# pwrliang/RayJoin

Measured on AMD Instinct MI355X. Metric: LSI+PIP query throughput, USCounty |><| BlockGroup, higher is better.
Workload: dtype int128+f64; 1 GPU; USCounty(base, 7112768 segs) |><| BlockGroup(query, 28793160 segs, 29665680 points), -query=lsi then -query=pip, -mode=lbvh (software LBVH); kernel_schedule=k_lsi and the PIP kernels share the chip (512 + 1536 blocks), schedule_settled_before_timing=True

## Files before the change

### rayjoin_amd/csrc/rj_api.hip

```cpp
#include <hip/hip_runtime.h>
#include <rccl/rccl.h>

#include <cmath>
#include <cstdarg>
#include <cstdio>
#include <cstring>
#include <functional>
#include <new>
#include <string>
#include <thread>
#include <vector>

#include "../../include/rayjoin_amd.h"
#include "rj_crossings.h"
#include "rj_dissolve.h"
#include "rj_eliminate.h"
#include "rj_faces.h"
#include "rj_node.h"
#include "rj_kernels.h"
#include "rj_face_points.h"
#include "rj_nearest.h"
#include "rj_within.h"
#include "rj_neighbours.h"
#include "rj_overlay_dev.h"
#include "rj_overlay_ops.h"
#include "rj_pipeline.h"
#include "rj_polygons.h"
#include "rj_ringmap.h"
#include "rj_rings.h"
#include "rj_simplify.h"
#include "rj_snap.h"

using namespace rj;

namespace {

struct MapState {
  bool present = false;
  uint64_t np = 0, ne = 0, nc = 0;
  int64_t* pts = nullptr;
  Seg* seg = nullptr;
  uint32_t* edge_chain = nullptr;
  uint32_t* ccode = nullptr;
  uint32_t* left = nullptr;
  uint32_t* right = nullptr;
  uint32_t* edge_begin = nullptr;
  int4* qext = nullptr;
  int2* qpts = nullptr;
  bool runs_cut = false;
  uint32_t run_cap = 0;
  uint64_t closed_chains = 0;
  uint32_t *run_len = nullptr, *leaf_first = nullptr, *pack_tmp = nullptr;
  QBox* run_box = nullptr;
  uint64_t packed_leaves = 0;
  uint32_t packed_solo = 0;
  uint64_t nruns = 0, npieces = 0;
  uint32_t *piece_begin = nullptr, *piece_len = nullptr, *run_first = nullptr;
};

struct BvhState {
  bool built = false;
  int leaf_order = 0;
  uint64_t n0 = 0, n0p = 0;
  char* pool = nullptr;
  Seg* sseg = nullptr;
  uint32_t* seid = nullptr;
  int32_t* sface = nullptr;
  QBox* box0 = nullptr;
  int32_t* pmx1 = nullptr;
  uint2* xtab = nullptr;
  uint2* ytab2 = nullptr;
  uint32_t* occ = nullptr;
  uint32_t* sky = nullptr;
  bool use_sky = false;
  uint32_t* strip_ytab = nullptr;
  uint4* strip_info = nullptr;
  uint2* strip_tall = nullptr;
  int strip_shift = 0;
  uint32_t occ_permille = 0;
  bool ysort = false;
  const char* columns_why = "";
  int strip_tab_shift = 0;
  QBox* strip_box = nullptr;
  uint64_t strip_entries = 0, strip_cap = 0;
  bool strips_built = false;
  QBox* lvl[kMaxLevels] = {nullptr};
  uint64_t nlvl[kMaxLevels] = {0};
  uint64_t alloc[kMaxLevels] = {0};
  int top = 0;
};

struct GridState {
  bool built = false;
  int g = 0;
  double scale = 0;
  uint32_t* begin = nullptr;
  uint32_t* eids = nullptr;
  uint64_t total = 0;
};

constexpr int kNumTimers = 12;
constexpr unsigned long long kIncoherentExtent = 1ull << 28;
constexpr uint64_t kExchHead = RJ_EXCHANGE_HEAD_WORDS;
constexpr int kCoTrials = 4;

}

struct rj_handle_s {
  int device = 0;
  hipStream_t own_stream = nullptr;
  hipStream_t aux_stream = nullptr;
  int pip_concurrent = 0;
  int cus = 256;
  bool lsi_inflight = false;
  bool lsi_shared = false;
  int co_trials = 0;
  float co_best[3] = {1e30f, 1e30f, 1e30f};
  int co_choice = -1;
  int co_mode = 0;
  bool co_measure = false;
  bool co_points = false;
  uint64_t co_n = 0;
  uint64_t co_np = 0;
  uint64_t co_np_other = 0;
  float co_ratio = 0.46f;
  int co_wpc = 8;
  int lsi_share_set = 0, pip_share_set = 0;
  int co_L = 0, co_best_L = 0;
  float co_best_imb = 0;
  int lsi_share_blocks() const {
    if (lsi_share_set) return lsi_share_set;
    if (co_L) return co_L;
    const int half = cus / 2 > 0 ? cus / 2 : 1;
    const int b = ((int) ((512.0f + 128.0f * (float) (8 - co_wpc) + 200.0f * (co_ratio - 0.6f)) * (float) cus / 256.0f) + half / 2) / half * half;
    return b < cus ? cus : (b > cus * 4 ? cus * 4 : b);
  }
  int last_pip_share = 0;
  int pip_share_blocks() const { return pip_share_set ? pip_share_set : cus * 5; }
  bool aux_pending = false;
  hipEvent_t ev_order = nullptr;
  hipStream_t stream = nullptr;
  MapState map[2];
  BvhState bvh[2];
  unsigned long long* d_counter = nullptr;
  int flip_lsi = 0, flip_pip[2] = {0, 0};
  int pip_walk = 1;
  int last_walk_points = 1;
  int last_prepared = 0;
  int last_passes = 0;
  int flip_walk[2] = {0, 0};
  uint32_t* rest[3] = {nullptr, nullptr, nullptr};
  uint64_t rest_cap[3] = {0, 0, 0};
  uint32_t* todo[3] = {nullptr, nullptr, nullptr};
  unsigned long long* todo_mask[3] = {nullptr, nullptr, nullptr};
  int exact_own_stream = 0;
  hipStream_t exact_stream = nullptr;
  hipEvent_t ev_walk_done = nullptr, ev_exact_done[2] = {nullptr, nullptr};
  bool exact_recorded[2] = {false, false};
  int exact_buf = 0, exact_last = -1;
  int exact_rot = 0;
  bool exact_pending = false;
  const void *exact_out_closest = nullptr, *exact_out_face = nullptr;
  unsigned long long* h_rest = nullptr;
  unsigned long long* d_rest = nullptr;
  uint64_t walk_n[2] = {0, 0};
  size_t count_word = 0;
  uint32_t* slow_list = nullptr;
  uint64_t slow_cap = 0;
  int flip_slow = 0;
  int last_lsi_segments = 1;
  int lsi_segments = 2;
  int walk_points = 2;
  int timers = 1;
  int points_split = -1;
  int last_points_split = 0;
  unsigned long long* d_stats = nullptr;
  unsigned long long* d_occ_part = nullptr;
  unsigned long long* h_pinned = nullptr;
  uint32_t* h_fault = nullptr;
  uint32_t* d_fault = nullptr;
  int debug_stack_cap = 1 << 30;
  int debug_walk_stack = 0;
  int debug_strip_shift = 0;
  int debug_lazy_columns_min = 0;
  bool lazy_columns_ok = false;
  bool lazy_columns_want = false;
  hipEvent_t ev[kNumTimers][2];
  bool ev_valid[kNumTimers] = {false};
  int stats_on = 0;
  GridState grid[2];
  int query_order = 1;
  bool last_ordered = false;
  bool order_fresh = false;
  struct CohCache { bool valid = false; uint64_t begin = 0, n = 0; bool incoherent = false; } coh[2][2];
  struct OrdCache { uint32_t* perm = nullptr; uint64_t cap = 0, begin = 0, n = 0; bool valid = false; } ordc[2][2];
  struct CallerSet {
    const void* p = nullptr;
    uint64_t n = 0;
    bool valid = false, has_perm = false, fresh_perm = false;
    uint32_t* perm = nullptr;
    uint64_t perm_cap = 0;
    unsigned long long sorted_extent = 0;
    uint64_t queries = 0, stamp = 0;
  };
  static constexpr int kCallerSets = 4;
  CallerSet caller[kCallerSets];
  unsigned long long* h_est = nullptr;
  unsigned long long* d_est = nullptr;
  uint64_t caller_clock = 0;
  int cur_caller = -1;
  const uint32_t* cur_order = nullptr;
  uint64_t ord_cap = 0;
  MortonKey *ord_kin = nullptr, *ord_kout = nullptr;
  uint32_t *ord_vin = nullptr, *ord_vout = nullptr;
  char* ord_temp = nullptr;
  size_t ord_temp_bytes = 0;
  int leaf_order = 1;
  int debug_run_cap = 0;
  int debug_pack_solo = 0;
  int debug_pack_spread = 0;
  int debug_cross_shift = 0, debug_cross_pair_budget = 0, debug_cross_extent_factor = 0, debug_cross_reg_factor = 0;
  CrossingsReport cross_report = {};
  NodeReport node_report;
  SnapReport snap_report;
  int debug_simplify_all_points = 0;
  SimplifyReport simplify_report;
  int debug_faces_shift = 0;
  FacesReport faces_report;
  int debug_elim_point_blocks = 0;
  EliminateReport eliminate_report;
  int debug_dissolve_point_blocks = 0;
  DissolveReport dissolve_report;
  int debug_neighbours_point_blocks = 0;
  NeighboursReport neighbours_report;
  int debug_face_points_blocks = 0;
  FacePointsReport face_points_report;
  int debug_nearest_blocks = 0;
  int debug_nearest_order_nomem = 0;
  StageMs nearest_report;
  struct NearestUnordered { const void* p = nullptr; uint64_t n = 0; bool valid = false; };
  static constexpr int kNearestUnordered = 4;
  NearestUnordered nearest_unordered[kNearestUnordered];
  int nearest_unordered_next = 0;
  int debug_within_blocks = 0;
  StageMs within_report;
  uint32_t stitch_stats[4] = {0, 0, 0, 0};
  char* strip_scratch = nullptr;
  size_t strip_scratch_bytes = 0;
  int pip_columns = -1;
  int last_columns = 0;
  int leaf_ysort = 1;
  int skyline = -1;
  int max_blocks = 1 << 20;
  int chunk_groups = 0;
  int group_lanes = 0;
  uint64_t last_stats[16] = {0};
  char* arena = nullptr;
  size_t arena_bytes = 0;
  ncclComm_t comm = nullptr;
  ncclComm_t comm2 = nullptr;
  hipStream_t comm_stream = nullptr, comm_stream2 = nullptr;
  hipEvent_t ev_comm = nullptr, ev_comm2 = nullptr, ev_comm2_aux = nullptr;
  struct Exch {
    uint32_t* send = nullptr;
    uint32_t* recv = nullptr;
    uint64_t recv_words = 0, slot = 0;
    bool pending = false;
  } ex[2];
  uint64_t ex_capacity = 0, ex_slot = 0;
  int ex_last_begin = -1;
  hipEvent_t ev_count[2] = {nullptr, nullptr};
  bool count_pending[2] = {false, false};
  unsigned long long* h_heads = nullptr;
  uint32_t* ag_send = nullptr;
  uint32_t* ag_recv = nullptr;
  uint64_t ag_send_words = 0, ag_recv_words = 0;
  int nranks = 1, rank = 0;
  unsigned long long* d_counts = nullptr;
  struct PlanRec {
    uint64_t epoch = 1;
    uint64_t sched_epoch = 0;
    struct Lsi { bool ran = false; uint64_t epoch = 0, n = 0; LaunchNote k = {"", 0, 0}; int order = 0, co_mode = 0; bool paired = false, shared = false; } lsi;
    struct Rec { bool ran = false; uint64_t epoch = 0; bool two_kernels = false, count_on_device = false; uint64_t seen = ~0ull; } rec;
    struct Pip {
      bool ran = false, aux = false, caller = false, shared = false;
      uint64_t epoch = 0, n = 0, rest_hint = ~0ull;
      LaunchNote first = {"", 0, 0};
      int passes = 0, order = 0, exact_blocks = 0, locate_blocks = 0;
      int prepared = 0;
      const char* why = "";
    } pip;
  } plan;
  std::string err;
};

namespace {

int fail(rj_handle h, int code, const char* fmt, ...) {
  char buf[512];
  va_list ap;
  va_start(ap, fmt);
  vsnprintf(buf, sizeof(buf), fmt, ap);
  va_end(ap);
  if (h) h->err = buf;
  return code;
}

#define RJ_HIP(h, expr)                                                                        \
  do {                                                                                         \
    hipError_t _e = (expr);                                                                    \
    if (_e != hipSuccess)                                                                      \
      return fail(h, _e == hipErrorOutOfMemory ? RJ_E_NOMEM : RJ_E_HIP, "%s failed: %s (%s:%d)", \
                  #expr, hipGetErrorString(_e), __FILE__, __LINE__);                           \
  } while (0)

#define RJ_CHECK_H(h) \
  if (!(h)) return RJ_E_INVALID

template <typename T>
int dev_alloc(rj_handle h, T** p, uint64_t count) {
  *p = nullptr;
  RJ_HIP(h, hipMalloc((void**) p, (count ? count : 1) * sizeof(T)));
  return RJ_OK;
}

void free_map(MapState& m) {
  (void) hipFree(m.pts); (void) hipFree(m.seg); (void) hipFree(m.edge_chain); (void) hipFree(m.ccode); (void) hipFree(m.left); (void) hipFree(m.right); (void) hipFree(m.edge_begin);
  (void) hipFree(m.qext);
  (void) hipFree(m.piece_begin); (void) hipFree(m.piece_len); (void) hipFree(m.run_first);
  (void) hipFree(m.run_len); (void) hipFree(m.leaf_first); (void) hipFree(m.pack_tmp); (void) hipFree(m.run_box);
  m = MapState();
}

void free_grid(GridState& g) {
  (void) hipFree(g.begin); (void) hipFree(g.eids);
  g = GridState();
}

void free_bvh(BvhState& b) {
  if (b.pool) {
    (void) hipFree(b.pool);
  } else {
    (void) hipFree(b.sseg); (void) hipFree(b.seid); (void) hipFree(b.sface); (void) hipFree(b.box0); (void) hipFree(b.pmx1); (void) hipFree(b.xtab); (void) hipFree(b.ytab2); (void) hipFree(b.occ); (void) hipFree(b.sky);
    for (int l = 0; l < kMaxLevels; l++) (void) hipFree(b.lvl[l]);
  }
  (void) hipFree(b.strip_ytab); (void) hipFree(b.strip_info); (void) hipFree(b.strip_tall); (void) hipFree(b.strip_box);
  b = BvhState();
}

DeviceBvh bvh_view(const BvhState& b) {
  DeviceBvh d;
  d.sseg = b.sseg; d.seid = b.seid; d.sface = b.sface; d.box0 = b.box0; d.pmx1 = b.pmx1; d.xtab = b.xtab; d.ytab2 = b.ysort ? b.ytab2 : nullptr; d.occ = b.occ; d.sky = b.use_sky ? b.sky : nullptr;
  for (int l = 0; l < kMaxLevels; l++) {
    d.lvl[l] = b.lvl[l]; d.nlvl[l] = (uint32_t) b.nlvl[l];
    d.ord[l] = b.lvl[l] ? reinterpret_cast<const uint64_t*>(b.lvl[l] + b.alloc[l]) : nullptr;
  }
  d.top = b.top; d.n0 = b.n0; d.occ_permille = b.occ_permille;
  d.lsi_root = b.top >= 2 && b.nlvl[b.top] <= 4 && b.nlvl[b.top - 1] <= 128 ? b.top - 1 : b.top;
  d.strips.ytab = b.strips_built ? b.strip_ytab : nullptr;
  d.strips.ebox = b.strip_box; d.strips.einfo = b.strip_info; d.strips.tall = b.strip_tall; d.strips.shift = b.strip_shift;
  return d;
}

DeviceMap map_view(const MapState& m) {
  DeviceMap d;
  d.pts = m.pts; d.seg = m.seg; d.edge_chain = m.edge_chain; d.left = m.left; d.right = m.right;
  d.np = m.np; d.ne = m.ne; d.nc = m.nc;
  return d;
}

int set_device(rj_handle h) {
  RJ_HIP(h, hipSetDevice(h->device));
  return RJ_OK;
}

static inline bool timers_off(rj_handle h) { return !h->timers && !(h->pip_concurrent == 2 && h->co_choice < 0); }
void tic(rj_handle h, int t, hipStream_t st = nullptr) { if (timers_off(h)) return; (void) hipEventRecord(h->ev[t][0], st ? st : h->stream); }
void toc(rj_handle h, int t, hipStream_t st = nullptr) { if (timers_off(h)) return; (void) hipEventRecord(h->ev[t][1], st ? st : h->stream); h->ev_valid[t] = true; }
hipError_t join_aux(rj_handle h) {
  if (!h->aux_pending) return hipSuccess;
  h->aux_pending = false;
  hipError_t e = hipStreamSynchronize(h->aux_stream);
  if (h->exact_pending) {
    h->exact_pending = false;
    const hipError_t e2 = hipStreamSynchronize(h->exact_stream);
    if (e == hipSuccess) e = e2;
  }
  return e;
}

static void co_reset(rj_handle h) {
  h->plan.epoch++;
  h->co_trials = 0; h->co_best[0] = h->co_best[1] = h->co_best[2] = 1e30f; h->co_choice = -1; h->co_measure = false; h->co_n = 0; h->co_np = 0; h->co_np_other = 0;
  h->co_ratio = 0.46f;
  h->co_L = h->co_best_L = 0;
  h->co_best_imb = 0;
}
static void co_collect(rj_handle h) {
  if (!h->co_measure) return;
  h->co_measure = false;
  if (h->co_choice >= 0) return;
  if (hipEventQuery(h->ev[RJ_T_LSI_KERNEL][1]) != hipSuccess || hipEventQuery(h->ev[RJ_T_PIP_KERNEL][1]) != hipSuccess) return;
  float a = 0, b = 0;
  if (hipEventElapsedTime(&a, h->ev[RJ_T_LSI_KERNEL][0], h->ev[RJ_T_LSI_KERNEL][1]) != hipSuccess) return;
  if (hipEventElapsedTime(&b, h->ev[RJ_T_LSI_KERNEL][0], h->ev[RJ_T_PIP_KERNEL][1]) != hipSuccess) return;
  float span = a > b ? a : b, c = 0;
  if (h->co_points && hipEventQuery(h->ev[RJ_T_LSI_POINTS][1]) == hipSuccess &&
      hipEventElapsedTime(&c, h->ev[RJ_T_LSI_KERNEL][0], h->ev[RJ_T_LSI_POINTS][1]) == hipSuccess && c > span) span = c;
  if (h->co_mode == 0) {
    float pip = 0, pts = 0;
    if (hipEventElapsedTime(&pip, h->ev[RJ_T_PIP_KERNEL][0], h->ev[RJ_T_PIP_KERNEL][1]) == hipSuccess && pip > 0) {
      if (h->co_points && c > 0) (void) hipEventElapsedTime(&pts, h->ev[RJ_T_LSI_POINTS][0], h->ev[RJ_T_LSI_POINTS][1]);
      h->co_ratio = (a + pts) / pip;
    }
  }
  if (h->co_mode == 1 && h->co_choice < 0 && !h->lsi_share_set) {
    const int used = h->lsi_share_blocks();
    const float lsi_side = a > c ? a : c;
    const float imb = (lsi_side - b) / (span > 0 ? span : 1.0f);
    const float aimb = imb < 0 ? -imb : imb;
    if (h->co_best_L == 0 || span < h->co_best[1] * 0.97f || (span < h->co_best[1] * 0.99f && aimb < h->co_best_imb)) {
      h->co_best_L = used;
      h->co_best_imb = aimb;
    }
    int next = used + (imb > 0 ? 1 : -1) * (h->cus / 2 > 0 ? h->cus / 2 : 1);
    next = next < h->cus ? h->cus : (next > h->cus * 4 ? h->cus * 4 : next);
    h->co_L = next;
  }
  if (span < h->co_best[h->co_mode]) h->co_best[h->co_mode] = span;
  if (++h->co_trials >= kCoTrials && h->co_choice < 0) {
    h->co_choice = 0;
    for (int m = 1; m < 3; m++) if (h->co_best[m] < h->co_best[h->co_choice]) h->co_choice = m;
    if (h->co_choice != 1 && h->co_best[1] <= h->co_best[h->co_choice] * 1.03f) h->co_choice = 1;
    if (h->co_best_L) h->co_L = h->co_best_L;
    h->plan.sched_epoch = h->plan.epoch;
  }
}
static int co_pick(rj_handle h, uint64_t n) {
  co_collect(h);
  if (h->co_n && (n > h->co_n + h->co_n / 4 || n + n / 4 < h->co_n)) co_reset(h);
  h->co_n = n;
  if (h->co_choice >= 0) return h->co_choice;
// ... 10 lines not shown
constexpr size_t kSlowCountWord = 12;
constexpr size_t kRestCountWord = 8;
constexpr size_t kExactRestWord[3] = {10, 11, 14};
constexpr size_t kGridLsiCountWord = 6;

int check_fault(rj_handle h) {
  const uint32_t l = h->h_fault[0], p = h->h_fault[1];
  if (!l && !p) return RJ_OK;
  h->h_fault[0] = h->h_fault[1] = 0;
  return fail(h, RJ_E_INTERNAL, "traversal stack overflow in %s%s%s: results are incomplete", l ? "k_lsi" : "",
              l && p ? " and " : "", p ? "k_pip" : "");
}

int switch_stream(rj_handle h, hipStream_t s) {
  if (s == h->stream) return RJ_OK;
  if (int r = set_device(h)) return r;
  RJ_HIP(h, hipStreamSynchronize(h->stream));
  RJ_HIP(h, join_aux(h));
  h->lsi_shared = h->lsi_inflight = false;
  h->co_measure = false;
  h->stream = s;
  return RJ_OK;
}

int set_stats(rj_handle h, int64_t v) { h->stats_on = v != 0; return RJ_OK; }
int set_own_stream(rj_handle h, int64_t) { return switch_stream(h, h->own_stream); }
int set_pip_concurrent(rj_handle h, int64_t v) {
  if (join_aux(h) != hipSuccess) return fail(h, RJ_E_HIP, "pip_concurrent: stream sync failed");
  h->pip_concurrent = (int) v;
  co_reset(h);
  return RJ_OK;
}
int set_pip_exact_stream(rj_handle h, int64_t v) {
  if ((int) v == h->exact_own_stream) return RJ_OK;
  if (int r = set_device(h)) return r;
  RJ_HIP(h, hipStreamSynchronize(h->stream));
  h->aux_pending = true;
  RJ_HIP(h, join_aux(h));
  RJ_HIP(h, hipStreamSynchronize(h->exact_stream));
  for (size_t wd : kExactRestWord) RJ_HIP(h, hipMemsetAsync(h->d_counter + wd, 0, 8, h->stream));
  RJ_HIP(h, hipStreamSynchronize(h->stream));
  h->exact_rot = 0; h->exact_buf = 0; h->exact_last = -1; h->exact_out_closest = h->exact_out_face = nullptr;
  h->exact_recorded[0] = h->exact_recorded[1] = false;
  h->exact_own_stream = (int) v;
  return RJ_OK;
}

constexpr int64_t kAnyLo = INT64_MIN, kAnyHi = INT64_MAX;
struct Option {
  const char* name;
  bool debug;
  int rj_handle_s::*field;
  int64_t lo, hi;
  const char* hint;
  const char* env;
  int (*set)(rj_handle h, int64_t v);
  int nalso;
  int64_t also[5];
  bool accepts(int64_t v) const {
    if (v >= lo && v <= hi) return true;
    for (int i = 0; i < nalso; i++) if (v == also[i]) return true;
    return false;
  }
};
const Option kOptions[] = {
    {"leaf_order", false, &rj_handle_s::leaf_order, 0, 1, "leaf_order: 0 Hilbert neighbours, 1 chain runs", "RJ_LEAF_ORDER"},
    {"skyline", false, &rj_handle_s::skyline, -1, 1, "skyline: -1 auto (maps of isolated rings), 0 never, 1 always"},
    {"leaf_ysort", false, &rj_handle_s::leaf_ysort, 0, 1, "leaf_ysort: 1 blocks taller than wide get a second order by y (LSI), 0 x order only", "RJ_LEAF_YSORT"},
    {"pip_columns", false, &rj_handle_s::pip_columns, -1, 1, "pip_columns: -1 auto (maps of closed rings or of short chains), 0 never, 1 always",
     "RJ_PIP_COLUMNS"},
    {"lsi_segments", false, &rj_handle_s::lsi_segments, 1, 2, "lsi_segments: 1 or 2", "RJ_LSI_SEGMENTS"},
    {"pip_walk_points", false, &rj_handle_s::walk_points, 1, 2, "pip_walk_points: 1 or 2", "RJ_WALK_POINTS"},
    {"pip_walk", false, &rj_handle_s::pip_walk, 0, 2, "pip_walk: 0 k_pip alone, 1 auto, 2 always two passes"},
    {"lsi_points_split", false, &rj_handle_s::points_split, -1, 1, "lsi_points_split: -1 by the last count, 0 never, 1 always", "RJ_POINTS_SPLIT"},
    {"query_order", false, &rj_handle_s::query_order, 0, 2, "query_order: 0 never, 1 auto, 2 always"},
    {"timers", false, &rj_handle_s::timers, 0, 1, "timers: 0 or 1"},
    {"pip_concurrent", false, &rj_handle_s::pip_concurrent, 0, 2,
     "pip_concurrent: 0 never, 1 LSI and PIP queries come in pairs and share the chip, 2 the same if it measures faster", nullptr, set_pip_concurrent},
    {"pip_exact_stream", false, &rj_handle_s::exact_own_stream, 0, 1, "pip_exact_stream: 0 or 1", nullptr, set_pip_exact_stream},
    {"stats", false, &rj_handle_s::stats_on, kAnyLo, kAnyHi, nullptr, nullptr, set_stats},
    {"own_stream", false, nullptr, kAnyLo, kAnyHi, nullptr, nullptr, set_own_stream},
    {"chunk_groups", true, &rj_handle_s::chunk_groups, 0, 4096},
    {"group_lanes", true, &rj_handle_s::group_lanes, 0, 0, "group_lanes: 0 (auto), 4, 8, 16, 32 or 64", nullptr, nullptr, 5, {4, 8, 16, 32, 64}},
    {"max_blocks", true, &rj_handle_s::max_blocks, 1, 1 << 20},
    {"lsi_share_blocks", true, &rj_handle_s::lsi_share_set, 0, 1 << 20},
    {"pip_share_blocks", true, &rj_handle_s::pip_share_set, 0, 1 << 20},
    {"stack_cap", true, &rj_handle_s::debug_stack_cap, 1, 1 << 30},
    {"walk_stack", true, &rj_handle_s::debug_walk_stack, 0, 1 << 30},
    {"strip_shift", true, &rj_handle_s::debug_strip_shift, 15, 20, "strip_shift: 0 or 15..20 (the sort key holds 16 bits of strip)", nullptr, nullptr, 1, {0}},
    {"lazy_columns_min", true, &rj_handle_s::debug_lazy_columns_min, 0, 1 << 30},
    {"run_cap", true, &rj_handle_s::debug_run_cap, 2, 64, "run_cap: 0 or 2..64", nullptr, nullptr, 1, {0}},
    {"pack_solo", true, &rj_handle_s::debug_pack_solo, 0, 64},
    {"pack_spread", true, &rj_handle_s::debug_pack_spread, 0, 1000000},
    {"cross_shift", true, &rj_handle_s::debug_cross_shift, 15, 47, "cross_shift: 0 (choose) or 15..47", nullptr, nullptr, 1, {0}},
    {"cross_pair_budget", true, &rj_handle_s::debug_cross_pair_budget, 0, 1 << 30},
    {"cross_extent_factor", true, &rj_handle_s::debug_cross_extent_factor, 0, 1 << 20},
    {"cross_reg_factor", true, &rj_handle_s::debug_cross_reg_factor, 0, 1 << 20},
    {"simplify_all_points", true, &rj_handle_s::debug_simplify_all_points, 0, 1},
    {"faces_shift", true, &rj_handle_s::debug_faces_shift, 15, 47, "faces_shift: 0 (choose) or 15..47", nullptr, nullptr, 1, {0}},
    {"elim_point_blocks", true, &rj_handle_s::debug_elim_point_blocks, 0, 1 << 20},
    {"dissolve_point_blocks", true, &rj_handle_s::debug_dissolve_point_blocks, 0, 1 << 20},
    {"neighbours_point_blocks", true, &rj_handle_s::debug_neighbours_point_blocks, 0, 1 << 20},
    {"face_points_blocks", true, &rj_handle_s::debug_face_points_blocks, 0, 1 << 20},
    {"nearest_blocks", true, &rj_handle_s::debug_nearest_blocks, 0, 1 << 20},
    {"nearest_order_nomem", true, &rj_handle_s::debug_nearest_order_nomem, 0, 1},
    {"within_blocks", true, &rj_handle_s::debug_within_blocks, 0, 1 << 20},
};

const Option* find_option(const char* name, bool debug) {
  for (const Option& o : kOptions)
    if (o.debug == debug && !strcmp(name, o.name)) return &o;
  return nullptr;
}

int set_option(rj_handle h, const char* name, int64_t value, bool debug) {
  RJ_CHECK_H(h);
  if (!name) return fail(h, RJ_E_INVALID, "null option name");
  const Option* o = find_option(name, debug);
  if (!o) return fail(h, RJ_E_INVALID, debug ? "unknown debug option '%s'" : "unknown option '%s'", name);
  if (!o->accepts(value))
    return o->hint ? fail(h, RJ_E_INVALID, "%s", o->hint) : fail(h, RJ_E_INVALID, "%s: %lld..%lld", name, (long long) o->lo, (long long) o->hi);
  if (o->set) return o->set(h, value);
  h->*o->field = (int) value;
  return RJ_OK;
}

int read_gcd_pairs(rj_handle h, int, int64_t* v) {
  if (int r = set_device(h)) return r;
  unsigned long long c = 0;
  RJ_HIP(h, hipStreamSynchronize(h->stream));
  RJ_HIP(h, hipMemcpy(&c, h->d_counter + kSlowCountWord + (1 - h->flip_slow), 8, hipMemcpyDeviceToHost));
  *v = h->last_points_split ? (int64_t) c : -1;
  return RJ_OK;
}
int read_comm_ranks(rj_handle h, int, int64_t* v) {
  int c = 0;
  if (h->comm && ncclCommCount(h->comm, &c) != ncclSuccess) return fail(h, RJ_E_HIP, "ncclCommCount failed");
  *v = c;
  return RJ_OK;
}
struct Report {
  const char* name;
  int per;
  int (*get)(rj_handle h, int k, int64_t* v);
};
#define RJ_READ(expr) [](rj_handle h, int k, int64_t* v) { *v = (int64_t) (expr); return (int) RJ_OK; }
const Report kReports[] = {
    {"query_last_ordered", 0, RJ_READ(h->last_ordered ? 1 : 0)},
    {"pip_schedule", 0, RJ_READ(h->pip_concurrent == 2 ? h->co_choice : (h->pip_concurrent == 1 ? 1 : 0))},
    {"pip_schedule_trials", 0, RJ_READ(h->co_trials)},
    {"pip_schedule_us", 3, RJ_READ(h->co_best[k] < 1e29f ? (int64_t) (h->co_best[k] * 1000.0f) : -1)},
    {"lsi_last_segments", 0, RJ_READ(h->last_lsi_segments)},
    {"pip_last_walk_points", 0, RJ_READ(h->last_walk_points)},
    {"pip_last_prepared", 0, RJ_READ(h->last_prepared)},
    {"lsi_points_last_split", 0, RJ_READ(h->last_points_split)},
    {"lsi_points_gcd_pairs", 0, read_gcd_pairs},
    {"pip_last_passes", 0, RJ_READ(h->last_passes)},
    {"pip_last_columns", 0, RJ_READ(h->last_columns)},
    {"pip_rest", 0, RJ_READ(h->h_rest[0])},
    {"pip_rest_aux", 0, RJ_READ(h->h_rest[1])},
    {"leaf_order_used", 2, RJ_READ(h->bvh[k].leaf_order)},
    {"leaf_slots", 2, RJ_READ(h->bvh[k].n0p)},
    {"leaf_runs", 2, RJ_READ(h->map[k].runs_cut ? (int64_t) h->map[k].nruns : -1)},
    {"occ_permille", 2, RJ_READ(h->bvh[k].occ_permille)},
    {"leaf_ysort_used", 2, RJ_READ(h->bvh[k].ysort ? 1 : 0)},
    {"pip_columns_used", 2, RJ_READ(h->bvh[k].strips_built ? 1 : 0)},
    {"pip_column_entries", 2, RJ_READ(h->bvh[k].strip_entries)},
    {"pip_column_shift", 2, RJ_READ(h->bvh[k].strips_built ? h->bvh[k].strip_shift : 0)},
    {"skyline_used", 2, RJ_READ(h->bvh[k].use_sky ? 1 : 0)},
    {"closed_chains", 2, RJ_READ(h->map[k].closed_chains)},
    {"stitch_rounds", 0, RJ_READ(h->stitch_stats[0])},
    {"stitch_loop_ends", 0, RJ_READ(h->stitch_stats[1])},
    {"cross_last_shift", 0, RJ_READ(h->cross_report.shift)},
    {"cross_last_registrations", 0, RJ_READ(h->cross_report.registrations)},
    {"cross_last_largest_cell", 0, RJ_READ(h->cross_report.largest_run)},
    {"cross_last_pair_tests", 0, RJ_READ(h->cross_report.pair_tests)},
    {"cross_last_items", 0, RJ_READ(h->cross_report.n_items)},
    {"cross_last_us", 6, RJ_READ(h->cross_report.ms[k] < 0 ? -1 : (int64_t) (h->cross_report.ms[k] * 1000.0f))},
    {"node_last_us", 6, RJ_READ(h->node_report.ms[k] < 0 ? -1 : (int64_t) (h->node_report.ms[k] * 1000.0f))},
    {"snap_last_us", 6, RJ_READ(h->snap_report.ms[k] < 0 ? -1 : (int64_t) (h->snap_report.ms[k] * 1000.0f))},
    {"simplify_last_us", 6, RJ_READ(h->simplify_report.ms[k] < 0 ? -1 : (int64_t) (h->simplify_report.ms[k] * 1000.0f))},
    {"simplify_last_syncs", 0, RJ_READ(h->simplify_report.n_syncs)},
    {"simplify_last_list_sum", 0, RJ_READ(h->simplify_report.list_sum)},
    {"simplify_last_list_max", 0, RJ_READ(h->simplify_report.list_max)},
    {"simplify_round_list", 10, RJ_READ(h->simplify_report.round_list[k])},
    {"simplify_round_us", 10, RJ_READ((int64_t) (h->simplify_report.round_ms[k] * 1000.0f))},
    {"simplify_late_rounds", 0, RJ_READ(h->simplify_report.late_rounds)},
    {"simplify_late_list", 0, RJ_READ(h->simplify_report.late_list)},
    {"simplify_late_us", 0, RJ_READ((int64_t) (h->simplify_report.late_ms * 1000.0f))},
    {"faces_last_shift", 0, RJ_READ(h->faces_report.shift)},
    {"faces_last_registrations", 0, RJ_READ(h->faces_report.registrations)},
    {"faces_last_ray_tests", 0, RJ_READ(h->faces_report.ray_tests)},
    {"faces_last_cells", 0, RJ_READ(h->faces_report.cells)},
    {"faces_last_us", 6, RJ_READ(h->faces_report.ms[k] < 0 ? -1 : (int64_t) (h->faces_report.ms[k] * 1000.0f))},
    {"elim_last_us", 6, RJ_READ(h->eliminate_report.ms[k] < 0 ? -1 : (int64_t) (h->eliminate_report.ms[k] * 1000.0f))},
    {"dissolve_last_us", 6, RJ_READ(h->dissolve_report.ms[k] < 0 ? -1 : (int64_t) (h->dissolve_report.ms[k] * 1000.0f))},
    {"neighbours_last_us", 6, RJ_READ(h->neighbours_report.ms[k] < 0 ? -1 : (int64_t) (h->neighbours_report.ms[k] * 1000.0f))},
    {"face_points_last_us", 5, RJ_READ(h->face_points_report.ms[k == 4 ? 5 : k] < 0 ? -1 : (int64_t) (h->face_points_report.ms[k == 4 ? 5 : k] * 1000.0f))},
    {"nearest_last_us", 3, RJ_READ(h->nearest_report.ms[k == 2 ? 5 : k] < 0 ? -1 : (int64_t) (h->nearest_report.ms[k == 2 ? 5 : k] * 1000.0f))},
    {"within_last_us", 4, RJ_READ(h->within_report.ms[k == 3 ? 5 : k] < 0 ? -1 : (int64_t) (h->within_report.ms[k == 3 ? 5 : k] * 1000.0f))},
    {"comm_ranks", 0, read_comm_ranks},
    {"lsi_share_blocks", 0, RJ_READ(h->lsi_share_blocks())},
    {"pip_share_blocks", 0, RJ_READ(h->last_pip_share ? h->last_pip_share : h->pip_share_blocks())},
};
#undef RJ_READ

const Report* find_report(const char* name, int* k) {
  for (const Report& r : kReports) {
    const size_t len = strlen(r.name);
    if (strncmp(name, r.name, len)) continue;
    const char* tail = name + len;
    if (!r.per && !tail[0]) { *k = 0; return &r; }
    if (r.per && tail[0] >= '0' && tail[0] < '0' + r.per && !tail[1]) { *k = tail[0] - '0'; return &r; }
  }
  return nullptr;
}

int fail_map_check(rj_handle h, const char* name, uint32_t bad) {
  if (bad == rings::kBadStart) return fail(h, RJ_E_INVALID, "%s: row_index must start at 0", name);
  if (bad == rings::kBadEnd) return fail(h, RJ_E_INVALID, "%s: row_index must end at np", name);
  if (bad == rings::kBadEmptyChain) return fail(h, RJ_E_INVALID, "%s: row_index must ascend (a chain has no point)", name);
  return fail(h, RJ_E_INVALID, "%s: a coordinate lies outside the scaled range [-2^46, 2^46)", name);
}
int write_empty_row(rj_handle h, uint32_t* row_index_dev) {
  if (row_index_dev) {
    RJ_HIP(h, hipMemsetAsync(row_index_dev, 0, 4, h->stream));
    RJ_HIP(h, hipStreamSynchronize(h->stream));
  }
  return RJ_OK;
}
template <class Meta, class Device, class Report, class Counts>
int map_cuts_call(rj_handle h, const char* name, const char* drop_last, Device device, Report rj_handle_s::*report, const int64_t* xy_dev, uint64_t np,
                  const uint32_t* row_index_dev, uint64_t nc, const rj_crossing* cross_dev, uint64_t n_cross, uint32_t flags, uint64_t point_capacity,
                  int64_t* out_xy_dev, uint32_t* out_row_index_dev, uint32_t* edge_origin_dev, Counts* counts) {
  RJ_CHECK_H(h);
  if (!counts) return fail(h, RJ_E_INVALID, "%s: counts is null", name);
  memset(counts, 0, sizeof(*counts));
  if (flags & ~node::kDropLast) return fail(h, RJ_E_INVALID, "%s: unknown flags 0x%x", name, flags);
  if ((np && !xy_dev) || (nc && !row_index_dev) || (n_cross && !cross_dev)) return fail(h, RJ_E_INVALID, "%s: null input array", name);
  if (np >= (1ull << 32) || nc > np || np - nc >= 0xFFFFFFFFull) return fail(h, RJ_E_INVALID, "%s: nc <= np < 2^32 and np - nc < 2^32 - 1", name);
  if (nc == 0 && np != 0) return fail(h, RJ_E_INVALID, "%s: points without chains", name);
  if (n_cross >= (1ull << 31)) return fail(h, RJ_E_INVALID, "%s: n_cross < 2^31", name);
  if (nc == 0 && n_cross) return fail(h, RJ_E_INVALID, "%s: a record names an edge that the map does not have", name);
  if (point_capacity && (!out_xy_dev || !out_row_index_dev)) return fail(h, RJ_E_INVALID, "%s: null output", name);
  if (int r = set_device(h)) return r;
  h->*report = Report{};
  if (nc == 0) return write_empty_row(h, out_row_index_dev);
  Meta m;
  RJ_HIP(h, device(h->stream, xy_dev, np, row_index_dev, nc, cross_dev, n_cross, flags, point_capacity, out_xy_dev, out_row_index_dev, edge_origin_dev, &m,
                   &(h->*report)));
  if (m.bad && m.bad <= rings::kBadStart) return fail_map_check(h, name, m.bad);
  if (m.bad == node::kBadOpenChain)
    return fail(h, RJ_E_INVALID, "%s: %s needs chains of two points or more whose first point equals the last", name, drop_last);
  if (m.bad == node::kBadRecord) return fail(h, RJ_E_INVALID, "%s: a record needs eid[0] < eid[1] < ne and a kind in 1..4", name);
  if (m.bad == node::kBadZeroEdge) return fail(h, RJ_E_INVALID, "%s: a record names an edge of zero length", name);
  if (m.bad) return fail(h, RJ_E_INVALID, "%s: the records must strictly ascend by (eid[0], eid[1])", name);
  memcpy(counts, &m.counts, sizeof(*counts));
  if (np + counts->n_cuts >= (1ull << 32))
    return fail(h, RJ_E_INVALID, "%s: %llu points and %llu cuts: np + n_cuts < 2^32", name, (unsigned long long) np, (unsigned long long) counts->n_cuts);
  if (counts->n_points > point_capacity)
    return fail(h, RJ_E_OVERFLOW, "%s: %llu points; capacity %llu", name, (unsigned long long) counts->n_points, (unsigned long long) point_capacity);
  return RJ_OK;
}

}

extern "C" {

const char* rj_version(void) { return "rayjoin_amd 0.1.0 (gfx950)"; }

int rj_create(int device_id, rj_handle* out) {
  if (!out) return RJ_E_INVALID;
  *out = nullptr;
  int ndev = 0;
  if (hipGetDeviceCount(&ndev) != hipSuccess || device_id < 0 || device_id >= ndev) return RJ_E_HIP;
  rj_handle h = new (std::nothrow) rj_handle_s();
  if (!h) return RJ_E_NOMEM;
  h->device = device_id;
  for (const Option& o : kOptions)
    if (const char* e = o.env ? getenv(o.env) : nullptr)
      if (o.accepts(atoi(e))) h->*o.field = atoi(e);
  {
    hipDeviceProp_t prop;
    if (hipGetDeviceProperties(&prop, device_id) == hipSuccess && prop.multiProcessorCount > 0) h->cus = prop.multiProcessorCount;
  }
  if (hipSetDevice(device_id) != hipSuccess) { delete h; return RJ_E_HIP; }
  if (hipStreamCreateWithFlags(&h->own_stream, hipStreamNonBlocking) != hipSuccess) { delete h; return RJ_E_HIP; }
  h->stream = h->own_stream;
  if (hipStreamCreateWithFlags(&h->aux_stream, hipStreamNonBlocking) != hipSuccess) { (void) hipStreamDestroy(h->own_stream); delete h; return RJ_E_HIP; }
  int prio_least = 0, prio_greatest = 0;
  (void) hipDeviceGetStreamPriorityRange(&prio_least, &prio_greatest);
  if (hipStreamCreateWithPriority(&h->exact_stream, hipStreamNonBlocking, prio_greatest) != hipSuccess) {
    (void) hipStreamDestroy(h->own_stream); (void) hipStreamDestroy(h->aux_stream); delete h; return RJ_E_HIP;
  }
  bool ok = hipMalloc((void**) &h->d_counter, kCounterBytes) == hipSuccess &&
            hipMalloc((void**) &h->d_stats, 128) == hipSuccess &&
            hipMalloc((void**) &h->d_occ_part, 128) == hipSuccess &&
            hipHostMalloc((void**) &h->h_pinned, 256) == hipSuccess &&
            hipHostMalloc((void**) &h->h_fault, 64, hipHostMallocMapped) == hipSuccess &&
            hipHostGetDevicePointer((void**) &h->d_fault, h->h_fault, 0) == hipSuccess &&
            hipHostMalloc((void**) &h->h_rest, 64, hipHostMallocMapped) == hipSuccess &&
            hipHostGetDevicePointer((void**) &h->d_rest, h->h_rest, 0) == hipSuccess &&
            hipHostMalloc((void**) &h->h_est, 64, hipHostMallocMapped) == hipSuccess &&
            hipHostGetDevicePointer((void**) &h->d_est, h->h_est, 0) == hipSuccess;
  if (ok) {
    h->h_fault[0] = h->h_fault[1] = h->h_fault[kFaultNearestStack] = h->h_fault[kFaultWithinStack] = 0;
    h->h_rest[0] = h->h_rest[1] = ~0ull;
    h->h_rest[2] = ~0ull;
    for (int k = 0; k < rj_handle_s::kCallerSets; k++) h->h_est[k] = 0;
    ok = hipMemset(h->d_counter, 0, kCounterBytes) == hipSuccess;
    for (size_t blk : {kSchedLsi, kSchedLsi + kSchedBlockWords, kSchedPipMain, kSchedPipMain + kSchedBlockWords, kSchedPipAux,
                       kSchedPipAux + kSchedBlockWords, kSchedWalkMain, kSchedWalkMain + kSchedBlockWords, kSchedWalkAux,
                       kSchedWalkAux + kSchedBlockWords})
      ok = ok && hipMemcpy((char*) (h->d_counter + blk) + kSchedFaultPtrWord * 4, &h->d_fault, sizeof(h->d_fault), hipMemcpyHostToDevice) == hipSuccess;
  }
  for (int t = 0; ok && t < kNumTimers; t++)
    ok = hipEventCreate(&h->ev[t][0]) == hipSuccess && hipEventCreate(&h->ev[t][1]) == hipSuccess;
  ok = ok && hipEventCreateWithFlags(&h->ev_count[0], hipEventDisableTiming) == hipSuccess &&
       hipEventCreateWithFlags(&h->ev_count[1], hipEventDisableTiming) == hipSuccess;
  ok = ok && hipEventCreateWithFlags(&h->ev_order, hipEventDisableTiming) == hipSuccess;
  ok = ok && hipEventCreateWithFlags(&h->ev_walk_done, hipEventDisableTiming) == hipSuccess &&
       hipEventCreateWithFlags(&h->ev_exact_done[0], hipEventDisableTiming) == hipSuccess &&
       hipEventCreateWithFlags(&h->ev_exact_done[1], hipEventDisableTiming) == hipSuccess;
  ok = ok && warm_query_kernels(h->stream) == hipSuccess && warm_grid_kernels(h->stream) == hipSuccess &&
       warm_stitch_kernels(h->stream) == hipSuccess && warm_strip_kernels(h->stream) == hipSuccess &&
       warm_overlay_kernels(h->stream) == hipSuccess && warm_crossings_kernels(h->stream) == hipSuccess &&
       hipStreamSynchronize(h->stream) == hipSuccess;
  if (!ok) { delete h; return RJ_E_HIP; }
  *out = h;
  return RJ_OK;
}

int rj_destroy(rj_handle h) {
  RJ_CHECK_H(h);
  (void) hipSetDevice(h->device);
  (void) hipStreamSynchronize(h->stream);
  (void) hipStreamSynchronize(h->aux_stream);
  (void) hipStreamSynchronize(h->exact_stream);
  for (int i = 0; i < 2; i++) { free_map(h->map[i]); free_bvh(h->bvh[i]); free_grid(h->grid[i]); }
  for (int k = 0; k < 2; k++) for (int i = 0; i < 2; i++) (void) hipFree(h->ordc[k][i].perm);
  (void) hipFree(h->d_counter); (void) hipFree(h->d_stats); (void) hipFree(h->d_occ_part); (void) hipHostFree(h->h_pinned); (void) hipHostFree(h->h_fault);
  (void) hipFree(h->slow_list);
  (void) hipHostFree(h->h_est);
  for (int k = 0; k < rj_handle_s::kCallerSets; k++) (void) hipFree(h->caller[k].perm);
  (void) hipHostFree(h->h_rest); for (int k = 0; k < 3; k++) { (void) hipFree(h->rest[k]); (void) hipFree(h->todo[k]); (void) hipFree(h->todo_mask[k]); }
  (void) hipFree(h->ord_kin); (void) hipFree(h->ord_kout); (void) hipFree(h->ord_vin); (void) hipFree(h->ord_vout); (void) hipFree(h->ord_temp);
  for (int t = 0; t < kNumTimers; t++) { (void) hipEventDestroy(h->ev[t][0]); (void) hipEventDestroy(h->ev[t][1]); }
  for (int k = 0; k < 2; k++) if (h->ev_count[k]) (void) hipEventDestroy(h->ev_count[k]);
  if (h->ev_order) (void) hipEventDestroy(h->ev_order);
  if (h->ev_walk_done) (void) hipEventDestroy(h->ev_walk_done);
  for (int k = 0; k < 2; k++) if (h->ev_exact_done[k]) (void) hipEventDestroy(h->ev_exact_done[k]);
  (void) hipFree(h->arena);
  (void) hipFree(h->strip_scratch);
  if (h->comm) (void) rj_comm_destroy(h);
  (void) hipStreamDestroy(h->own_stream);
  (void) hipStreamDestroy(h->aux_stream);
  (void) hipStreamDestroy(h->exact_stream);
  delete h;
  return RJ_OK;
}

int rj_set_stream(rj_handle h, void* s) {
  RJ_CHECK_H(h);
  return switch_stream(h, (hipStream_t) s);
}

int rj_sync(rj_handle h) {
  RJ_CHECK_H(h);
  if (int r = set_device(h)) return r;
  RJ_HIP(h, hipStreamSynchronize(h->stream));
  h->lsi_shared = h->lsi_inflight = false;
  RJ_HIP(h, join_aux(h));
  return check_fault(h);
}

const char* rj_last_error_string(rj_handle h) { return h ? h->err.c_str() : "null handle"; }

int rj_invalidate(rj_handle h) {
  RJ_CHECK_H(h);
  if (int r = set_device(h)) return r;
  RJ_HIP(h, hipStreamSynchronize(h->stream));
  RJ_HIP(h, join_aux(h));
  for (int k = 0; k < rj_handle_s::kCallerSets; k++) {
    h->caller[k].valid = h->caller[k].has_perm = false;
    h->h_est[k] = 0;
  }
  for (auto& u : h->nearest_unordered) u.valid = false;
  return RJ_OK;
}

int rj_get_option(rj_handle h, const char* name, int64_t* value) {
  RJ_CHECK_H(h);
  if (!name || !value) return fail(h, RJ_E_INVALID, "rj_get_option: null argument");
  const Option* o = find_option(name, false);
  if (o && o->field) { *value = h->*o->field; return RJ_OK; }
  int k = 0;
  if (const Report* r = find_report(name, &k)) return r->get(h, k, value);
  return fail(h, RJ_E_INVALID, "unknown option '%s'", name);
}

int rj_get_plan(rj_handle h, char* buf, size_t cap, size_t* need) {
  RJ_CHECK_H(h);
  const rj_handle_s::PlanRec& P = h->plan;
  char t[1024];
  std::string o = "{";
  auto add = [&](const char* fmt, ...) {
    va_list ap;
    va_start(ap, fmt);
    vsnprintf(t, sizeof(t), fmt, ap);
    va_end(ap);
    o += t;
  };
  static const char* const kOrder[3] = {"as given", "through a cached Morton permutation", "through a Morton permutation sorted in this call (runs alone)"};
  static const char* const kSched[3] = {"turns", "shared", "full grids"};
  add("\"epoch\": %llu", (unsigned long long) P.epoch);
  add(", \"index\": [");
  for (int m = 0; m < 2; m++) {
    const BvhState& b = h->bvh[m];
    add("%s{\"map\": %d, \"built\": %s, \"levels\": %d, \"slots\": %llu, \"leaves\": \"%s\", \"skyline\": %s, \"columns\": %s, \"column_shift\": %d, "
        "\"steep_blocks_sorted_by_y\": %s, \"occupancy_permille\": %u, \"mean_chain_edges\": %.1f, \"slots_per_segment\": %.3f, \"columns_why\": \"",
        m ? ", " : "", m, b.built ? "true" : "false", b.top, (unsigned long long) b.n0p, b.leaf_order == 1 ? "polyline runs" : "Hilbert neighbours",
        b.use_sky ? "true" : "false", b.strips_built ? "true" : "false", b.strips_built ? b.strip_shift : 0, b.ysort ? "true" : "false", b.occ_permille,
        h->map[m].nc ? (double) h->map[m].ne / (double) h->map[m].nc : 0.0, b.n0 ? (double) b.n0p / (double) b.n0 : 0.0);
    for (const char* c = b.built ? b.columns_why : ""; *c; c++) { if (*c == '"') o += '\\'; o += *c; }
    o += "\"}";
  }
  add("]");
  add(", \"schedule\": {\"pip_concurrent\": %d, \"trials\": %d, \"of\": %d", h->pip_concurrent, h->co_trials, kCoTrials);
  if (h->pip_concurrent == 2) {
    add(", \"choice\": \"%s\", \"settled\": %s, \"settled_in_epoch\": %llu, \"in_force\": %s, \"for_query_size\": %llu", h->co_choice >= 0 ? kSched[h->co_choice] : "undecided",
        h->co_choice >= 0 ? "true" : "false", (unsigned long long) P.sched_epoch, h->co_choice >= 0 && P.sched_epoch == P.epoch ? "true" : "false",
        (unsigned long long) h->co_n);
    add(", \"best_span_us\": {");
    for (int m = 0; m < 3; m++) add("%s\"%s\": %d", m ? ", " : "", kSched[m], h->co_best[m] < 1e29f ? (int) (h->co_best[m] * 1000.0f) : -1);
    add("}, \"turns_ratio_lsi_over_pip\": %.3f", (double) h->co_ratio);
  } else {
    add(", \"choice\": \"%s\", \"settled\": true", h->pip_concurrent == 1 ? "shared" : "turns");
  }
  add(", \"shared_grids\": {\"lsi_blocks\": %d, \"pip_blocks\": %d, \"fixed_by_debug_option\": %s}}", h->lsi_share_blocks(),
      h->last_pip_share ? h->last_pip_share : h->pip_share_blocks(), h->lsi_share_set || h->pip_share_set ? "true" : "false");
  if (P.lsi.ran) {
    add(", \"lsi\": {\"epoch\": %llu, \"current\": %s, \"segments\": %llu, \"kernel\": \"%s\", \"blocks\": %d, \"segments_per_lane\": %d, \"order\": \"%s\", "
        "\"paired_with_pip\": %s, \"schedule\": \"%s\", \"on_shared_grid\": %s}",
        (unsigned long long) P.lsi.epoch, P.lsi.epoch == P.epoch ? "true" : "false", (unsigned long long) P.lsi.n, P.lsi.k.kernel, P.lsi.k.grid, P.lsi.k.per_lane,
        kOrder[P.lsi.order], P.lsi.paired ? "true" : "false", P.lsi.paired ? kSched[P.lsi.co_mode] : "alone (a synchronous or unpaired query: full grid)",
        P.lsi.shared ? "true" : "false");
  } else {
    add(", \"lsi\": null");
  }
  if (P.rec.ran) {
    add(", \"records\": {\"epoch\": %llu, \"kernels\": \"%s\", \"count\": \"%s\", \"pairs_expected\": %lld, \"rule\": \"%s\"}", (unsigned long long) P.rec.epoch,
        P.rec.two_kernels ? "k_lsi_points + k_lsi_points_gcd over what it declines" : "k_lsi_points_gcd alone",
        P.rec.count_on_device ? "read on the device" : "given by the caller", P.rec.seen == ~0ull ? -1ll : (long long) P.rec.seen,
        h->points_split >= 0 ? "fixed by the lsi_points_split option" : "two kernels from 393216 pairs on (the count of the last query; unknown yet: two)");
  } else {
    add(", \"records\": null");
  }
  if (P.pip.ran) {
    add(", \"pip\": {\"epoch\": %llu, \"current\": %s, \"points\": %llu, \"points_from\": \"%s\", \"stream\": \"%s\", \"on_shared_grid\": %s, \"order\": \"%s\", "
        "\"passes\": %d, \"first_pass\": {\"kernel\": \"%s\", \"blocks\": %d, \"points_per_lane\": %d}, \"prepared_points\": %d",
        (unsigned long long) P.pip.epoch, P.pip.epoch == P.epoch ? "true" : "false", (unsigned long long) P.pip.n, P.pip.caller ? "a caller-owned array" : "the query map's vertices",
        P.pip.aux ? "second (beside the LSI query)" : "main", P.pip.shared ? "true" : "false", kOrder[P.pip.order], P.pip.passes, P.pip.first.kernel, P.pip.first.grid,
        P.pip.first.per_lane, P.pip.prepared);
    if (P.pip.passes == 3)
      add(", \"second_pass\": {\"kernel\": \"k_pip_exact\", \"blocks\": %d, \"locate_blocks\": %d}, \"left_over_by_last_query_of_this_size\": %lld", P.pip.exact_blocks,
          P.pip.locate_blocks, P.pip.rest_hint == ~0ull ? -1ll : (long long) P.pip.rest_hint);
    add(", \"why\": \"");
    for (const char* c = P.pip.why; *c; c++) { if (*c == '"' || *c == '\\') o += '\\'; o += *c; }
    add("\"}");
  } else {
    add(", \"pip\": null");
  }
  o += "}";
  if (need) *need = o.size();
  if (buf && cap) {
    const size_t k = o.size() < cap - 1 ? o.size() : cap - 1;
    memcpy(buf, o.data(), k);
    buf[k] = 0;
  }
  return RJ_OK;
}

int rj_set_option(rj_handle h, const char* name, int64_t value) { return set_option(h, name, value, false); }

int rj_set_debug_option(rj_handle h, const char* name, int64_t value) { return set_option(h, name, value, true); }

int rj_get_debug_option(rj_handle h, const char* name, int64_t* value) {
  RJ_CHECK_H(h);
  if (!name || !value) return fail(h, RJ_E_INVALID, "rj_get_debug_option: null argument");
  const Option* o = find_option(name, true);
  if (!o) return fail(h, RJ_E_INVALID, "unknown debug option '%s'", name);
  *value = h->*o->field;
  return RJ_OK;
}

static int begin_upload(rj_handle h, int map_id) {
  if (map_id < 0 || map_id > 1) return fail(h, RJ_E_INVALID, "map_id must be 0 or 1");
  RJ_HIP(h, join_aux(h));
  co_reset(h);
  h->h_rest[0] = h->h_rest[1] = ~0ull;
  h->walk_n[0] = h->walk_n[1] = 0;
  return RJ_OK;
}

static int install_map(rj_handle h, int map_id, uint64_t np, uint64_t nc, const std::function<hipError_t(MapState&)>& fill) {
  if (int r = set_device(h)) return r;
  MapState& m = h->map[map_id];
  free_map(m);
  free_bvh(h->bvh[map_id]);
  free_grid(h->grid[map_id]);
  h->coh[0][map_id].valid = h->coh[1][map_id].valid = false;
  h->ordc[0][map_id].valid = h->ordc[1][map_id].valid = false;
  for (auto& u : h->nearest_unordered) u.valid = false;
  m.np = np; m.nc = nc; m.ne = np - nc;
  int rc = RJ_OK;
  if (!rc) rc = dev_alloc(h, &m.pts, 2 * np + 2);
  if (!rc) rc = dev_alloc(h, &m.seg, m.ne);
  if (!rc) rc = dev_alloc(h, &m.edge_chain, m.ne);
  if (!rc) rc = dev_alloc(h, &m.ccode, m.ne);
  if (!rc) rc = dev_alloc(h, &m.left, nc);
  if (!rc) rc = dev_alloc(h, &m.right, nc);
  if (!rc) rc = dev_alloc(h, &m.edge_begin, nc + 1);
  hipError_t e = hipSuccess;
  if (!rc) {
    e = fill(m);
    if (e == hipSuccess) e = launch_build_segs(h->stream, m.pts, m.edge_begin, (uint32_t) nc, m.ne, m.seg, m.edge_chain, m.ccode);
    if (e == hipSuccess && np) {
      const uint64_t nblocks = (np + 63) / 64;
      if (hipMalloc((void**) &m.qext, 16 * nblocks + 8 * np) != hipSuccess) {
        (void) hipGetLastError();
        m.qext = nullptr;
      } else {
        m.qpts = reinterpret_cast<int2*>(m.qext + nblocks);
        e = launch_prepare_points(h->stream, m.pts, np, m.qpts, m.qext);
      }
    }
    const hipError_t es = hipStreamSynchronize(h->stream);
    if (e == hipSuccess) e = es;
  }
  if (rc || e != hipSuccess) free_map(m);
  if (rc) return rc;
  RJ_HIP(h, e);
  m.present = true;
  return RJ_OK;
}

int rj_upload_map(rj_handle h, int map_id, const int64_t* xy, uint64_t np, const uint32_t* row_index,
                  const int64_t* left, const int64_t* right, uint64_t nc) {
  RJ_CHECK_H(h);
  if (int r = begin_upload(h, map_id)) return r;
  if ((np && !xy) || (nc && (!row_index || !left || !right))) return fail(h, RJ_E_INVALID, "null input array");
  if (np >= (1ull << 32) || nc > np) return fail(h, RJ_E_INVALID, "index_t is 32-bit: np < 2^32, nc <= np");
  if (nc && (row_index[0] != 0 || row_index[nc] != np)) return fail(h, RJ_E_INVALID, "row_index must start at 0 and end at np");
  for (uint64_t c = 0; c < nc; c++)
    if (row_index[c + 1] < row_index[c] + 2)
      return fail(h, RJ_E_INVALID, "chain %llu has fewer than 2 points (planar_graph.h:71)", (unsigned long long) c);
  if (nc == 0 && np != 0) return fail(h, RJ_E_INVALID, "points without chains");
  for (uint64_t i = 0; i < 2 * np; i++)
    if (xy[i] < -((int64_t) 1 << 46) || xy[i] >= ((int64_t) 1 << 46))
      return fail(h, RJ_E_INVALID, "coordinate %llu outside the scaled range [-2^46, 2^46)", (unsigned long long) i);
  std::vector<uint32_t> eb(nc + 1), l32(nc), r32(nc);
  for (uint64_t c = 0; c <= nc; c++) eb[c] = nc ? (uint32_t) (row_index[c] - c) : 0;
  for (uint64_t c = 0; c < nc; c++) { l32[c] = (uint32_t) left[c]; r32[c] = (uint32_t) right[c]; }
  return install_map(h, map_id, np, nc, [&](MapState& m) {
    hipError_t e = hipSuccess;
    if (np) e = hipMemcpyAsync(m.pts, xy, 16 * np, hipMemcpyHostToDevice, h->stream);
    if (e == hipSuccess && nc) e = hipMemcpyAsync(m.edge_begin, eb.data(), 4 * (nc + 1), hipMemcpyHostToDevice, h->stream);
    if (e == hipSuccess && nc) e = hipMemcpyAsync(m.left, l32.data(), 4 * nc, hipMemcpyHostToDevice, h->stream);
    if (e == hipSuccess && nc) e = hipMemcpyAsync(m.right, r32.data(), 4 * nc, hipMemcpyHostToDevice, h->stream);
    return e;
  });
}

int rj_upload_map_dev(rj_handle h, int map_id, const int64_t* xy_dev, uint64_t np, const uint32_t* row_index_dev,
                      const int32_t* left_dev, const int32_t* right_dev, uint64_t nc) {
  RJ_CHECK_H(h);
  if (int r = begin_upload(h, map_id)) return r;
  if ((np && !xy_dev) || (nc && (!row_index_dev || !left_dev || !right_dev))) return fail(h, RJ_E_INVALID, "null input array");
  if (np >= (1ull << 32) || nc > np) return fail(h, RJ_E_INVALID, "index_t is 32-bit: np < 2^32, nc <= np");
  if (nc == 0 && np != 0) return fail(h, RJ_E_INVALID, "points without chains");
  if (int r = set_device(h)) return r;
  uint32_t* eb = nullptr;
  if (nc) {
    uint32_t status = 0;
    if (int r = dev_alloc(h, &eb, nc + 2)) return r;
    const hipError_t e = map_check_device(h->stream, xy_dev, np, row_index_dev, nc, eb, eb + nc + 1, &status);
    if (e != hipSuccess || status) (void) hipFree(eb);
    RJ_HIP(h, e);
    if (status == kMapBadStart) return fail(h, RJ_E_INVALID, "row_index must start at 0");
    if (status == kMapBadEnd) return fail(h, RJ_E_INVALID, "row_index must end at np");
    if (status == kMapBadShortChain) return fail(h, RJ_E_INVALID, "a chain has fewer than 2 points (planar_graph.h:71)");
    if (status) return fail(h, RJ_E_INVALID, "a coordinate lies outside the scaled range [-2^46, 2^46)");
  }
  const int rc = install_map(h, map_id, np, nc, [&](MapState& m) {
    hipError_t e = hipSuccess;
    if (np) e = hipMemcpyAsync(m.pts, xy_dev, 16 * np, hipMemcpyDeviceToDevice, h->stream);
    if (e == hipSuccess && nc) e = hipMemcpyAsync(m.edge_begin, eb, 4 * (nc + 1), hipMemcpyDeviceToDevice, h->stream);
    if (e == hipSuccess && nc) e = hipMemcpyAsync(m.left, left_dev, 4 * nc, hipMemcpyDeviceToDevice, h->stream);
    if (e == hipSuccess && nc) e = hipMemcpyAsync(m.right, right_dev, 4 * nc, hipMemcpyDeviceToDevice, h->stream);
    return e;
  });
  (void) hipFree(eb);
  return rc;
}

int rj_scale_points(const double bb[4], const double* xy, uint64_t n, int64_t* out_xy, int fused) {
  if (!bb || (n && (!xy || !out_xy))) return RJ_E_INVALID;
  const int64_t imax = INT64_MAX >> 17, imin = INT64_MIN >> 17;
  const double range = (double) (imax - imin);
  const double max_x = bb[2] + 1, min_x = bb[0] - 1, max_y = bb[3] + 1, min_y = bb[1] - 1;
  const double rx = range / (max_x - min_x), ry = range / (max_y - min_y);
  const double dx = 0.5 * ((imax + imin) - (max_x + min_x) * rx), dy = 0.5 * ((imax + imin) - (max_y + min_y) * ry);
  for (uint64_t i = 0; i < n; i++) {
    const double x = xy[2 * i], y = xy[2 * i + 1];
    double sx, sy;
    if (fused) {
      sx = std::fma(x, rx, dx);
      sy = std::fma(y, ry, dy);
    } else {
      const double tx = x * rx, ty = y * ry;
      sx = tx + dx;
      sy = ty + dy;
    }
    out_xy[2 * i] = (int64_t) sx;
    out_xy[2 * i + 1] = (int64_t) sy;
  }
  return RJ_OK;
}

int rj_map_num_edges(rj_handle h, int map_id, uint64_t* ne) {
  RJ_CHECK_H(h);
  if (map_id < 0 || map_id > 1 || !ne || !h->map[map_id].present) return fail(h, RJ_E_INVALID, "map not uploaded");
  *ne = h->map[map_id].ne;
  return RJ_OK;
}

int rj_map_num_points(rj_handle h, int map_id, uint64_t* np) {
  RJ_CHECK_H(h);
  if (map_id < 0 || map_id > 1 || !np || !h->map[map_id].present) return fail(h, RJ_E_INVALID, "map not uploaded");
  *np = h->map[map_id].np;
  return RJ_OK;
}

int rj_map_points_dev(rj_handle h, int map_id, const int64_t** pts_dev) {
  RJ_CHECK_H(h);
  if (map_id < 0 || map_id > 1 || !pts_dev || !h->map[map_id].present) return fail(h, RJ_E_INVALID, "map not uploaded");
  *pts_dev = h->map[map_id].pts;
  return RJ_OK;
}

int rj_map_prepared_dev(rj_handle h, int map_id, const int32_t** qpts_dev, const int32_t** qext_dev) {
  RJ_CHECK_H(h);
  if (map_id < 0 || map_id > 1 || !h->map[map_id].present) return fail(h, RJ_E_INVALID, "map not uploaded");
  if (qpts_dev) *qpts_dev = reinterpret_cast<const int32_t*>(h->map[map_id].qpts);
// ... 174 lines not shown
  uint64_t nruns = (h->leaf_order == 1 && m.ne && m.runs_cut) ? m.nruns : 0;
  uint64_t nleaves_runs = 0;
  if (nruns) {
    MapState& mm = h->map[base_map_id];
    if (int r = ensure_sort_scratch(h, nruns)) return r;
    k_in = h->ord_kin; k_out = h->ord_kout; v_in = h->ord_vin; v_out = h->ord_vout;
    const uint64_t nchunks = pack_runs_chunks(nruns);
    if (!mm.run_len) {
      int rc = dev_alloc(h, &mm.run_len, nruns);
      if (!rc) rc = dev_alloc(h, &mm.leaf_first, nruns + 1);
      if (!rc) rc = dev_alloc(h, &mm.run_box, nruns);
      if (!rc) rc = dev_alloc(h, &mm.pack_tmp, 2 * (nchunks + 1));
      if (rc) return rc;
    }
    const bool short_rings = mm.nc && mm.ne / mm.nc < 16 && 2 * mm.closed_chains >= mm.nc;
    const uint32_t solo_above = h->debug_pack_solo ? (uint32_t) h->debug_pack_solo : (short_rings ? 24u : (mm.run_cap ? mm.run_cap : 64u) * 3 / 4);
    const uint32_t spread = h->debug_pack_spread ? (uint32_t) h->debug_pack_spread : 8;
    hipError_t e = hipSuccess;
    tic(h, RJ_T_BUILD_KEYS);
    e = launch_run_keys(h->stream, m.seg, m.piece_begin, m.piece_len, m.run_first, nruns, k_in, v_in, mm.run_len, mm.run_box, solo_above);
    toc(h, RJ_T_BUILD_KEYS);
    tic(h, RJ_T_BUILD_SORT);
    size_t tb = h->ord_temp_bytes;
    if (e == hipSuccess) e = sort_morton_pairs(h->stream, h->ord_temp, tb, k_in, k_out, v_in, v_out, nruns);
    if (e == hipSuccess) e = launch_pack_runs(h->stream, v_out, mm.run_len, mm.run_box, nruns, solo_above, spread, mm.pack_tmp, mm.pack_tmp + nchunks + 1, mm.leaf_first, h->d_rest + 3);
    toc(h, RJ_T_BUILD_SORT);
    RJ_HIP(h, e);
    if (!mm.packed_leaves || mm.packed_solo != solo_above + 1000 * spread) {
      RJ_HIP(h, hipStreamSynchronize(h->stream));
      mm.packed_leaves = h->h_rest[3];
      mm.packed_solo = solo_above + 1000 * spread;
    }
    nleaves_runs = mm.packed_leaves;
    if (nleaves_runs * 64 > m.ne * 5 / 2) nruns = 0;
  }
  const uint64_t n0p_new = nruns ? nleaves_runs * 64 : pad64(m.ne ? m.ne : 1);
  if (n0p_new >= (1ull << 32)) return fail(h, RJ_E_INVALID, "rj_build_lbvh: %llu leaf slots do not fit 32-bit slot ids", (unsigned long long) n0p_new);
  const bool reuse = b.sseg && b.n0p == n0p_new;
  if (!reuse) free_bvh(b);
  b.built = false;
  b.leaf_order = nruns ? 1 : 0;
  b.n0 = m.ne;
  b.n0p = n0p_new;
  b.nlvl[0] = b.n0;
  b.alloc[0] = b.n0p;
  int top = 0;
  uint64_t n = b.n0p / 64;
  for (int l = 1; l < kMaxLevels; l++) {
    b.nlvl[l] = n;
    b.alloc[l] = pad64(n);
    top = l;
    if (n <= 64) break;
    n = (n + 63) / 64;
  }
  if (b.nlvl[top] > 64) return fail(h, RJ_E_INVALID, "too many segments for %d levels", kMaxLevels);
  b.top = top;
  if (!reuse) {
    size_t used = 0;
    auto take = [&](size_t bytes) { const size_t at = used; used = (used + bytes + 255) & ~(size_t) 255; return at; };
    const size_t o_sseg = take(sizeof(Seg) * b.n0p), o_seid = take(4 * b.n0p), o_sface = take(4 * b.n0p), o_box0 = take(sizeof(QBox) * b.n0p),
                 o_pmx1 = take(4 * b.n0p), o_xtab = take(sizeof(uint2) * b.n0p), o_ytab2 = take(sizeof(uint2) * b.n0p), o_occ = take(4 * ((size_t) kOccDim * kOccRowWords + 1)),
                 o_sky = take(4 * ((size_t) kSkyBuckets + 1));
    size_t o_lvl[kMaxLevels] = {0};
    for (int l = 1; l <= top; l++) o_lvl[l] = take(sizeof(QBox) * (b.alloc[l] + b.alloc[l] / 2));
    if (used <= ((size_t) 5 << 29)) {
      const hipError_t pe = hipMalloc((void**) &b.pool, used ? used : 1);
      if (pe != hipSuccess) {
        free_bvh(b);
        return fail(h, pe == hipErrorOutOfMemory ? RJ_E_NOMEM : RJ_E_HIP, "rj_build_lbvh: hipMalloc of %zu bytes for the index failed: %s", used, hipGetErrorString(pe));
      }
      b.sseg = (Seg*) (b.pool + o_sseg); b.seid = (uint32_t*) (b.pool + o_seid); b.sface = (int32_t*) (b.pool + o_sface);
      b.box0 = (QBox*) (b.pool + o_box0); b.pmx1 = (int32_t*) (b.pool + o_pmx1); b.xtab = (uint2*) (b.pool + o_xtab); b.ytab2 = (uint2*) (b.pool + o_ytab2);
      b.occ = (uint32_t*) (b.pool + o_occ); b.sky = (uint32_t*) (b.pool + o_sky);
      for (int l = 1; l <= top; l++) b.lvl[l] = (QBox*) (b.pool + o_lvl[l]);
    } else {
      int r = 0;
      if (!r) r = dev_alloc(h, &b.sseg, b.n0p);
      if (!r) r = dev_alloc(h, &b.seid, b.n0p);
      if (!r) r = dev_alloc(h, &b.sface, b.n0p);
      if (!r) r = dev_alloc(h, &b.box0, b.n0p);
      if (!r) r = dev_alloc(h, &b.pmx1, b.n0p);
      if (!r) r = dev_alloc(h, &b.xtab, b.n0p);
      if (!r) r = dev_alloc(h, &b.ytab2, b.n0p);
      if (!r) r = dev_alloc(h, &b.occ, (uint64_t) kOccDim * kOccRowWords + 1);
      if (!r) r = dev_alloc(h, &b.sky, (uint64_t) kSkyBuckets + 1);
      for (int l = 1; l <= top && !r; l++) r = dev_alloc(h, &b.lvl[l], b.alloc[l] + b.alloc[l] / 2);
      if (r) { free_bvh(b); return r; }
    }
  }
  if (!nruns && m.ne) {
    if (int r = ensure_sort_scratch(h, m.ne)) return r;
    k_in = h->ord_kin; k_out = h->ord_kout; v_in = h->ord_vin; v_out = h->ord_vout;
  }
  hipError_t e = hipSuccess;
  do {
    if (!nruns) {
      tic(h, RJ_T_BUILD_KEYS);
      if ((e = launch_morton(h->stream, m.seg, m.ne, k_in, v_in)) != hipSuccess) break;
      toc(h, RJ_T_BUILD_KEYS);
      tic(h, RJ_T_BUILD_SORT);
      if (m.ne) {
        size_t tb = h->ord_temp_bytes;
        if ((e = sort_morton_pairs(h->stream, h->ord_temp, tb, k_in, k_out, v_in, v_out, m.ne)) != hipSuccess) break;
      }
      toc(h, RJ_T_BUILD_SORT);
    }
    tic(h, RJ_T_BUILD_LEAVES);
    if ((e = hipMemsetAsync(b.occ, 0, ((size_t) kOccDim * kOccRowWords + 1) * 4, h->stream)) != hipSuccess) break;
    b.use_sky = false;
    b.ysort = h->leaf_ysort != 0 && !(m.runs_cut && m.nc && 2 * m.closed_chains >= m.nc);
    if ((e = launch_build_leaves(h->stream, m.seg, v_out, m.edge_chain, m.left, m.right, m.ne, nruns ? m.piece_begin : nullptr,
                                 m.piece_len, m.run_first, m.run_len, m.leaf_first, b.n0p / 64, b.alloc[1],
                                 b.sseg, b.seid, b.sface, b.box0, b.pmx1, b.xtab, b.lvl[1], b.occ, b.ysort ? b.ytab2 : nullptr)) != hipSuccess) break;
    toc(h, RJ_T_BUILD_LEAVES);
    tic(h, RJ_T_BUILD_LEVELS);
    const QBox* child = b.lvl[1];
    uint64_t child_alloc = b.alloc[1];
    for (int l = 2; l <= top; l++) {
      if ((e = launch_reduce_level(h->stream, child, child_alloc, b.lvl[l], b.alloc[l])) != hipSuccess) break;
      child = b.lvl[l];
      child_alloc = b.alloc[l];
    }
    if (e != hipSuccess) break;
    for (int l = 1; l <= top; l++)
      if ((e = launch_sibling_order(h->stream, b.lvl[l], b.alloc[l], (uint64_t*) (b.lvl[l] + b.alloc[l]))) != hipSuccess) break;
    if (e != hipSuccess) break;
    toc(h, RJ_T_BUILD_LEVELS);
  } while (0);
  RJ_HIP(h, e);
  b.strips_built = false;
  const bool rings = m.runs_cut && m.nc && 2 * m.closed_chains >= m.nc;
  const bool short_chains = m.runs_cut && m.nc && m.ne / m.nc < 16;
  const bool want_sky = h->skyline == 1 || (h->skyline < 0 && rings);
  b.columns_why = h->pip_columns == 0 ? "off (\"pip_columns\" 0)" : "the map's chains are long open polylines: the tree walk is the faster first pass";
  if (h->pip_columns == 1 || (h->pip_columns < 0 && (rings || short_chains))) {
    if (int r = build_strips(h, b, want_sky)) return r;
    b.columns_why = !b.strips_built ? "wanted, not built (a segment spans too many strips, or no memory for it): the tree serves the map"
                    : h->pip_columns == 1 ? "forced (\"pip_columns\" 1)"
                    : rings ? "most chains are closed rings (the tree is at its worst for upward rays there)"
                            : "short chains (mean chain length below 16 edges: fat leaves, measured rule of round 6)";
  }
  if (want_sky && !b.use_sky) {
    RJ_HIP(h, hipMemsetAsync(b.sky, 0, ((size_t) kSkyBuckets + 1) * 4, h->stream));
    RJ_HIP(h, launch_build_sky(h->stream, b.box0, b.seid, b.n0p, b.sky));
    b.use_sky = true;
  }
  RJ_HIP(h, launch_occ_count(h->stream, b.occ, h->d_occ_part, h->d_rest + 4));
  toc(h, RJ_T_BUILD);
  RJ_HIP(h, hipStreamSynchronize(h->stream));
  b.occ_permille = (uint32_t) (h->h_rest[4] * 1000ull / ((unsigned long long) kOccDim * kOccDim));
  b.built = true;
  co_reset(h);
  h->h_rest[0] = h->h_rest[1] = ~0ull;
  h->walk_n[0] = h->walk_n[1] = 0;
  return RJ_OK;
}

static int sort_query_points(rj_handle h, const int64_t* pts, uint64_t n) {
  if (int r = ensure_sort_scratch(h, n)) return r;
  tic(h, RJ_T_ORDER);
  RJ_HIP(h, launch_query_keys(h->stream, true, pts, nullptr, 0, n, h->ord_kin, h->ord_vin));
  size_t tb = h->ord_temp_bytes;
  RJ_HIP(h, sort_morton_pairs(h->stream, h->ord_temp, tb, h->ord_kin, h->ord_kout, h->ord_vin, h->ord_vout, n));
  toc(h, RJ_T_ORDER);
  return RJ_OK;
}
static int order_caller_points(rj_handle h, const int64_t* pts, uint64_t n, const uint32_t** order_out) {
  rj_handle_s::CallerSet* e = nullptr;
  int slot = -1;
  for (int k = 0; k < rj_handle_s::kCallerSets; k++)
    if (h->caller[k].valid && h->caller[k].p == pts && h->caller[k].n == n) { e = &h->caller[k]; slot = k; }
  bool incoherent = false;
  if (!e) {
    slot = 0;
    for (int k = 0; k < rj_handle_s::kCallerSets; k++) {
      if (!h->caller[k].valid) { slot = k; break; }
      if (h->caller[k].stamp < h->caller[slot].stamp) slot = k;
    }
    e = &h->caller[slot];
    RJ_HIP(h, hipStreamSynchronize(h->stream));
    RJ_HIP(h, join_aux(h));
    uint32_t* keep = e->perm;
    const uint64_t keep_cap = e->perm_cap;
    *e = rj_handle_s::CallerSet();
    e->perm = keep; e->perm_cap = keep_cap;
    e->p = pts; e->n = n; e->valid = true;
    h->h_est[slot] = 0;
    RJ_HIP(h, launch_group_extent_tail(h->stream, pts, nullptr, n, h->d_est + slot));
    RJ_HIP(h, hipStreamSynchronize(h->stream));
    incoherent = h->h_est[slot] > kIncoherentExtent + 1;
  } else {
    const unsigned long long v = h->h_est[slot];
    if (v) {
      if (e->has_perm) {
        if (e->fresh_perm) { e->sorted_extent = v - 1; e->fresh_perm = false; }
        incoherent = v - 1 > kIncoherentExtent && v - 1 > 2 * e->sorted_extent;
      } else {
        incoherent = v - 1 > kIncoherentExtent;
      }
    }
  }
  e->stamp = ++h->caller_clock;
  e->queries++;
  if (incoherent && h->lazy_columns_ok) {
    h->lazy_columns_want = true;
    h->cur_caller = slot;
    return RJ_OK;
  }
  if (incoherent) {
    if (e->perm_cap < n) {
      RJ_HIP(h, hipStreamSynchronize(h->stream));
      RJ_HIP(h, join_aux(h));
      (void) hipFree(e->perm);
      e->perm = nullptr; e->perm_cap = 0; e->has_perm = false;
      RJ_HIP(h, hipMalloc((void**) &e->perm, n * sizeof(uint32_t)));
      e->perm_cap = n;
    }
    if (int r = sort_query_points(h, pts, n)) return r;
    h->order_fresh = true;
    RJ_HIP(h, hipMemcpyAsync(e->perm, h->ord_vout, n * sizeof(uint32_t), hipMemcpyDeviceToDevice, h->stream));
    e->has_perm = true;
    e->fresh_perm = true;
    h->h_est[slot] = 0;
    e->queries = 1;
  }
  if (e->has_perm) {
    *order_out = e->perm;
    h->last_ordered = true;
  }
  h->cur_caller = slot;
  h->cur_order = *order_out;
  return RJ_OK;
}

static int maybe_order_queries(rj_handle h, bool points, const int64_t* pts, const Seg* segs, uint64_t begin,
                               uint64_t n, const uint32_t** order_out, int owner_map ,
                               uint64_t key_begin) {
  *order_out = nullptr;
  h->last_ordered = false;
  h->order_fresh = false;
  h->cur_caller = -1;
  h->cur_order = nullptr;
  if (h->query_order == 0 || n <= 64) return RJ_OK;
  if (points && owner_map < 0 && h->query_order == 1) return order_caller_points(h, pts, n, order_out);
  if (h->query_order == 1) {
    rj_handle_s::CohCache* cc = owner_map >= 0 ? &h->coh[points ? 1 : 0][owner_map] : nullptr;
    bool incoherent;
    if (cc && cc->valid && cc->begin == key_begin && cc->n == n) {
      incoherent = cc->incoherent;
    } else {
      RJ_HIP(h, hipMemsetAsync(h->d_counter + 4, 0, 16, h->stream));
      RJ_HIP(h, launch_group_extent(h->stream, points, pts, segs, begin, n, h->d_counter + 4));
      RJ_HIP(h, hipMemcpyAsync(h->h_pinned + 20, h->d_counter + 4, 16, hipMemcpyDeviceToHost, h->stream));
      RJ_HIP(h, hipStreamSynchronize(h->stream));
      const unsigned long long sum = h->h_pinned[20], groups = h->h_pinned[21];
      incoherent = groups != 0 && sum / groups > kIncoherentExtent;
      if (cc) { cc->valid = true; cc->begin = key_begin; cc->n = n; cc->incoherent = incoherent; }
    }
    if (!incoherent) return RJ_OK;
    if (h->lazy_columns_ok) { h->lazy_columns_want = true; return RJ_OK; }
  }
  rj_handle_s::OrdCache* oc = owner_map >= 0 ? &h->ordc[points ? 1 : 0][owner_map] : nullptr;
  if (oc && oc->valid && oc->begin == key_begin && oc->n == n) {
    *order_out = oc->perm;
    h->last_ordered = true;
    return RJ_OK;
  }
  if (int r = ensure_sort_scratch(h, n)) return r;
  h->order_fresh = true;
  tic(h, RJ_T_ORDER);
  RJ_HIP(h, launch_query_keys(h->stream, points, pts, segs, begin, n, h->ord_kin, h->ord_vin));
  size_t tb = h->ord_temp_bytes;
  RJ_HIP(h, sort_morton_pairs(h->stream, h->ord_temp, tb, h->ord_kin, h->ord_kout, h->ord_vin, h->ord_vout, n));
  toc(h, RJ_T_ORDER);
  *order_out = h->ord_vout;
  h->last_ordered = true;
  if (oc) {
    oc->valid = false;
    if (oc->cap < n) {
      (void) hipFree(oc->perm);
      oc->perm = nullptr; oc->cap = 0;
      if (hipMalloc((void**) &oc->perm, n * sizeof(uint32_t)) != hipSuccess) { oc->perm = nullptr; return RJ_OK; }
      oc->cap = n;
    }
    RJ_HIP(h, hipMemcpyAsync(oc->perm, h->ord_vout, n * sizeof(uint32_t), hipMemcpyDeviceToDevice, h->stream));
    oc->begin = key_begin; oc->n = n; oc->valid = true;
    *order_out = oc->perm;
  }
  return RJ_OK;
}

static int lsi_launch(rj_handle h, int base_map_id, int query_map_id, uint64_t qb, uint64_t qe,
                      uint64_t capacity, uint32_t* pairs_dev, bool async_call = false) {
  if (base_map_id < 0 || base_map_id > 1 || query_map_id != 1 - base_map_id)
    return fail(h, RJ_E_INVALID, "rj_lsi_query: base/query map ids must be {0,1} and differ");
  if (!h->map[query_map_id].present) return fail(h, RJ_E_INVALID, "rj_lsi_query: query map not uploaded");
  if (!h->bvh[base_map_id].built) return fail(h, RJ_E_INVALID, "rj_lsi_query: call rj_build_lbvh(base map) first");
  if (qb > qe || qe > h->map[query_map_id].ne) return fail(h, RJ_E_INVALID, "rj_lsi_query: bad query eid range");
  if (capacity && !pairs_dev) return fail(h, RJ_E_INVALID, "rj_lsi_query: null output");
  if (int r = set_device(h)) return r;
  if (h->stats_on) RJ_HIP(h, hipMemsetAsync(h->d_stats, 0, 128, h->stream));
  const uint32_t* order = nullptr;
  if (int r = maybe_order_queries(h, false, nullptr, h->map[query_map_id].seg, qb, qe - qb, &order, query_map_id, qb)) return r;
  LsiArgs a;
  a.bvh = bvh_view(h->bvh[base_map_id]);
  a.qseg = h->map[query_map_id].seg;
  a.qcode = h->map[query_map_id].ccode;
// ... 62 lines not shown
  RJ_CHECK_H(h);
  if (slot < 0 || slot > 1) return fail(h, RJ_E_INVALID, "rj_lsi_count_async: slot is 0 or 1");
  if (int r = set_device(h)) return r;
  RJ_HIP(h, hipMemcpyAsync(h->h_pinned + 28 + slot, h->d_counter + h->count_word, 8, hipMemcpyDeviceToHost, h->stream));
  RJ_HIP(h, hipEventRecord(h->ev_count[slot], h->stream));
  h->count_pending[slot] = true;
  return RJ_OK;
}

int rj_lsi_count_wait(rj_handle h, int slot, uint64_t capacity, uint64_t* n_found) {
  RJ_CHECK_H(h);
  if (slot < 0 || slot > 1 || !h->count_pending[slot]) return fail(h, RJ_E_INVALID, "rj_lsi_count_wait: no count in flight in slot %d", slot);
  if (int r = set_device(h)) return r;
  RJ_HIP(h, hipEventSynchronize(h->ev_count[slot]));
  h->count_pending[slot] = false;
  const uint64_t n = h->h_pinned[28 + slot];
  h->h_rest[2] = n;
  if (n_found) *n_found = n;
  if (int r = check_fault(h)) return r;
  if (n > capacity)
    return fail(h, RJ_E_OVERFLOW, "intersection queue overflow: %llu found, capacity %llu", (unsigned long long) n, (unsigned long long) capacity);
  return RJ_OK;
}

int rj_lsi_count_to(rj_handle h, uint64_t* n_found_dev) {
  RJ_CHECK_H(h);
  if (!n_found_dev) return fail(h, RJ_E_INVALID, "rj_lsi_count_to: null destination");
  if (int r = set_device(h)) return r;
  RJ_HIP(h, hipMemcpyAsync(n_found_dev, h->d_counter + h->count_word, 8, hipMemcpyDeviceToDevice, h->stream));
  return RJ_OK;
}

int rj_lsi_query(rj_handle h, int base_map_id, int query_map_id, uint64_t qb, uint64_t qe,
                 uint64_t capacity, uint32_t* pairs_dev, uint64_t* n_found) {
  RJ_CHECK_H(h);
  if (int r = lsi_launch(h, base_map_id, query_map_id, qb, qe, capacity, pairs_dev)) return r;
  return rj_lsi_query_finish(h, capacity, n_found);
}

constexpr uint64_t kPointsSplitAbove = 384 * 1024;
static hipError_t lsi_points_on_stream(rj_handle h, const uint32_t* pairs_dev, uint64_t n, const unsigned long long* n_dev, XsectRec* out) {
  const uint64_t seen = n_dev ? (uint64_t) h->h_rest[2] : n;
  const bool split = n < (1ull << 32) && (h->points_split >= 0 ? h->points_split == 1 : (seen == ~0ull || seen >= kPointsSplitAbove));
  if (split && h->slow_cap < n) {
    hipError_t e = hipStreamSynchronize(h->stream);
    if (e != hipSuccess) return e;
    (void) hipFree(h->slow_list);
    h->slow_list = nullptr; h->slow_cap = 0;
    if (hipMalloc((void**) &h->slow_list, n * 4) == hipSuccess) {
      h->slow_cap = n;
      (void) hipMemsetAsync(h->slow_list, 0, n * 4, h->stream);
    } else {
      (void) hipGetLastError();
    }
  }
  uint32_t* list = split && h->slow_cap >= n ? h->slow_list : nullptr;
  const int f = h->flip_slow;
  hipError_t e = launch_lsi_points(h->stream, h->map[0].seg, h->map[1].seg, pairs_dev, n, n_dev, out, list,
                                   h->d_counter + kSlowCountWord + f, h->d_counter + kSlowCountWord + (1 - f), h->d_rest + 2);
  if (list) h->flip_slow = 1 - f;
  h->last_points_split = list ? 1 : 0;
  h->plan.rec.ran = true; h->plan.rec.epoch = h->plan.epoch; h->plan.rec.two_kernels = list != nullptr;
  h->plan.rec.count_on_device = n_dev != nullptr; h->plan.rec.seen = seen;
  return e;
}

int rj_lsi_points(rj_handle h, const uint32_t* pairs_dev, uint64_t n, rj_xsect* out_dev) {
  RJ_CHECK_H(h);
  if (!h->map[0].present || !h->map[1].present) return fail(h, RJ_E_INVALID, "rj_lsi_points: both maps must be uploaded");
  if (n && (!pairs_dev || !out_dev)) return fail(h, RJ_E_INVALID, "rj_lsi_points: null buffer");
  if (int r = set_device(h)) return r;
  h->co_measure = false;
  tic(h, RJ_T_LSI_POINTS);
  RJ_HIP(h, lsi_points_on_stream(h, pairs_dev, n, nullptr, (XsectRec*) out_dev));
  toc(h, RJ_T_LSI_POINTS);
  RJ_HIP(h, hipStreamSynchronize(h->stream));
  return RJ_OK;
}

int rj_lsi_points_async(rj_handle h, const uint32_t* pairs_dev, uint64_t capacity, rj_xsect* out_dev) {
  RJ_CHECK_H(h);
  if (!h->map[0].present || !h->map[1].present) return fail(h, RJ_E_INVALID, "rj_lsi_points_async: both maps must be uploaded");
  if (capacity && (!pairs_dev || !out_dev)) return fail(h, RJ_E_INVALID, "rj_lsi_points_async: null buffer");
  if (int r = set_device(h)) return r;
  if (h->lsi_inflight) h->co_points = true;
  tic(h, RJ_T_LSI_POINTS);
  RJ_HIP(h, lsi_points_on_stream(h, pairs_dev, capacity, h->d_counter + h->count_word, (XsectRec*) out_dev));
  toc(h, RJ_T_LSI_POINTS);
  return RJ_OK;
}

int rj_sort_pairs(rj_handle h, uint32_t* pairs_dev, uint64_t n) {
  RJ_CHECK_H(h);
  if (n == 0) return RJ_OK;
  if (!pairs_dev) return fail(h, RJ_E_INVALID, "rj_sort_pairs: null buffer");
  if (int r = set_device(h)) return r;
  uint64_t* keys = (uint64_t*) pairs_dev;
  uint64_t* tmp = nullptr;
  void* temp = nullptr;
  size_t temp_bytes = 0;
  if (int r = dev_alloc(h, &tmp, n)) return r;
  tic(h, RJ_T_SORT);
  hipError_t e = launch_swap_halves(h->stream, keys, n);
  if (e == hipSuccess) e = sort_keys_u64(h->stream, nullptr, temp_bytes, keys, tmp, n);
  if (e == hipSuccess) e = hipMalloc(&temp, temp_bytes ? temp_bytes : 1);
  if (e == hipSuccess) e = sort_keys_u64(h->stream, temp, temp_bytes, keys, tmp, n);
  if (e == hipSuccess) e = hipMemcpyAsync(keys, tmp, 8 * n, hipMemcpyDeviceToDevice, h->stream);
  if (e == hipSuccess) e = launch_swap_halves(h->stream, keys, n);
  toc(h, RJ_T_SORT);
  if (e == hipSuccess) e = hipStreamSynchronize(h->stream);
  (void) hipFree(tmp); (void) hipFree(temp);
  RJ_HIP(h, e);
  return RJ_OK;
}

int rj_pip_query_async(rj_handle h, int base_map_id, int query_map_id, const int64_t* pts_dev,
                       uint64_t pt_begin, uint64_t n, uint32_t* closest_eid_dev, int32_t* face_id_dev) {
  RJ_CHECK_H(h);
  if (base_map_id < 0 || base_map_id > 1 || query_map_id != 1 - base_map_id)
    return fail(h, RJ_E_INVALID, "rj_pip_query: base/query map ids must be {0,1} and differ");
  if (!h->bvh[base_map_id].built) return fail(h, RJ_E_INVALID, "rj_pip_query: call rj_build_lbvh(base map) first");
  if (n && !closest_eid_dev) return fail(h, RJ_E_INVALID, "rj_pip_query: null output");
  const int64_t* pts = pts_dev;
  uint64_t coh_begin = 0;
  if (!pts) {
    coh_begin = pt_begin;
    const MapState& q = h->map[query_map_id];
    if (!q.present || pt_begin + n > q.np) return fail(h, RJ_E_INVALID, "rj_pip_query: bad point range of the query map");
    pts = q.pts + 2 * pt_begin;
  }
  if (int r = set_device(h)) return r;
  if (h->stats_on) RJ_HIP(h, hipMemsetAsync(h->d_stats, 0, 128, h->stream));
  const uint32_t* order = nullptr;
  bool by_columns = h->bvh[base_map_id].strips_built && h->pip_walk != 0 && (!h->stats_on || h->pip_walk == 2);
  if (by_columns && h->query_order != 2) { h->last_ordered = false; h->order_fresh = false; h->cur_caller = -1; h->cur_order = nullptr; }
  else {
    const uint64_t lazy_min = h->debug_lazy_columns_min ? (uint64_t) h->debug_lazy_columns_min : (1ull << 22);
    h->lazy_columns_ok = !by_columns && !h->bvh[base_map_id].strips_built && h->pip_columns < 0 && h->query_order == 1 && h->pip_walk != 0 &&
                         !h->stats_on && n >= lazy_min;
    h->lazy_columns_want = false;
    if (int r = maybe_order_queries(h, true, pts, nullptr, 0, n, &order, pts_dev ? -1 : query_map_id, coh_begin)) { h->lazy_columns_ok = false; return r; }
    h->lazy_columns_ok = false;
    if (h->lazy_columns_want) {
      BvhState& bb = h->bvh[base_map_id];
      RJ_HIP(h, hipStreamSynchronize(h->stream));
      RJ_HIP(h, join_aux(h));
      if (int r = build_strips(h, bb, false)) return r;
      if (bb.strips_built) {
        bb.columns_why = "built at the first PIP query over a spatially incoherent point set (uniform random points: every point on its own)";
        by_columns = true;
        co_reset(h);
        h->plan.epoch++;
        h->h_rest[0] = h->h_rest[1] = ~0ull;
        h->walk_n[0] = h->walk_n[1] = 0;
        h->last_ordered = false; h->order_fresh = false; h->cur_caller = -1; h->cur_order = nullptr;
      } else if (int r = maybe_order_queries(h, true, pts, nullptr, 0, n, &order, pts_dev ? -1 : query_map_id, coh_begin)) {
        return r;
      }
    }
  }
  const bool aux = !(order && h->order_fresh) && !h->stats_on && (h->pip_concurrent == 1 || (h->pip_concurrent == 2 && h->lsi_inflight));
  if (aux && h->pip_concurrent == 2 && h->co_mode == 0) {
    RJ_HIP(h, hipEventRecord(h->ev_order, h->stream));
    RJ_HIP(h, hipStreamWaitEvent(h->aux_stream, h->ev_order, 0));
  }
  const int max_blocks = aux && h->lsi_shared && h->pip_share_blocks() < h->max_blocks ? h->pip_share_blocks() : h->max_blocks;
  const int walk_share_of_this_pair = h->lsi_share_blocks();
  h->co_measure = h->pip_concurrent == 2 && h->lsi_inflight && !(order && h->order_fresh) && !h->stats_on && n > 0;
  if (h->co_measure) {
    if (h->co_np && (n > h->co_np + h->co_np / 4 || n + n / 4 < h->co_np)) {
      h->co_measure = false;
      if (h->co_np_other && !(n > h->co_np_other + h->co_np_other / 4 || n + n / 4 < h->co_np_other)) {
        const int keep_mode = h->co_mode;
        co_reset(h);
        h->co_mode = keep_mode;
        h->co_np = n;
        h->co_np_other = 0;
      } else {
        h->co_np_other = n;
      }
    } else {
      h->co_np = n;
      h->co_np_other = 0;
    }
  }
  hipStream_t st = aux ? h->aux_stream : h->stream;
  const int pflip = h->flip_pip[aux ? 1 : 0];
  unsigned long long* sched = h->d_counter + (aux ? kSchedPipAux : kSchedPipMain) + pflip * kSchedBlockWords;
  PipArgs a;
  a.bvh = bvh_view(h->bvh[base_map_id]);
  a.base = map_view(h->map[base_map_id]);
  a.pts = pts; a.n = n;
  a.order = order;
  a.query_map_id = query_map_id;
  a.closest = closest_eid_dev; a.face = face_id_dev;
  a.work_counter = (unsigned int*) sched;
  a.next_work_counter = (unsigned int*) (h->d_counter + (aux ? kSchedPipAux : kSchedPipMain) + (1 - pflip) * kSchedBlockWords);
  a.chunk_groups = (uint32_t) h->chunk_groups;
  a.group_lanes = (uint32_t) h->group_lanes;
  a.stack_cap = h->debug_stack_cap;
  a.walk_stack = h->debug_walk_stack;
  a.stats = h->stats_on ? h->d_stats : nullptr;
  a.rest = nullptr; a.rest_count = nullptr; a.next_rest_count = nullptr; a.n_dev = nullptr;
  a.todo = nullptr; a.todo_mask = nullptr;
  a.qpts = nullptr; a.qext = nullptr;
  const int walk_full = h->cus * pip_walk_blocks_per_cu(h->bvh[base_map_id].top);
  int walk_blocks = h->max_blocks;
  if (aux && h->lsi_shared) {
    const int share = h->pip_share_set ? h->pip_share_set : walk_full - (walk_share_of_this_pair <= 2 * h->cus ? 2 : 1) * h->cus;
    walk_blocks = share < h->max_blocks ? share : h->max_blocks;
  }
  if (aux && h->lsi_shared) h->last_pip_share = max_blocks;
  const int si = aux ? 1 : 0;
  bool walk = h->pip_walk != 0 && (!h->stats_on || h->pip_walk == 2) && n > 0 && n < (1ull << 32);
  uint64_t seen = ~0ull;
  for (int k : {si, 1 - si})
    if (seen == ~0ull && h->walk_n[k] == n && h->h_rest[k] != ~0ull) {
      seen = h->h_rest[k];
    }
  const char* why = !h->pip_walk ? "\"pip_walk\" 0: the exact kernel alone" : (walk ? "" : "instrumented (\"stats\"), no points, or more than 2^32 of them: the exact kernel alone");
  if (walk && h->pip_walk == 1 && seen != ~0ull && (seen * 10 > n * 3 || seen > 16384)) {
    walk = false;
    why = "the last two-pass query of this size left too many points to the exact kernel (> 30 %, or > 16384): first pass dropped";
  }
  const bool own = aux && walk && h->exact_own_stream;
  const int li = own ? 1 + h->exact_buf : si;
  if (walk && (h->rest_cap[si] < n || h->rest_cap[li] < n)) {
    RJ_HIP(h, hipStreamSynchronize(h->stream));
    RJ_HIP(h, join_aux(h));
    for (int k = 0; k < (h->exact_own_stream ? 3 : 2); k++) {
      if (h->rest_cap[k] >= n) continue;
      (void) hipFree(h->rest[k]); (void) hipFree(h->todo[k]); (void) hipFree(h->todo_mask[k]);
      h->rest[k] = nullptr; h->rest_cap[k] = 0; h->todo[k] = nullptr; h->todo_mask[k] = nullptr;
      if (int r = dev_alloc(h, &h->rest[k], n)) return r;
      if (int r = dev_alloc(h, &h->todo[k], n * (uint64_t) pip_walk_list_slots())) return r;
      if (int r = dev_alloc(h, &h->todo_mask[k], n / 4 + 1)) return r;
      h->rest_cap[k] = n;
      RJ_HIP(h, hipMemsetAsync(h->todo[k], 0xFF, n * (uint64_t) pip_walk_list_slots() * 4, h->stream));
      RJ_HIP(h, hipMemsetAsync(h->todo_mask[k], 0, (n / 4 + 1) * 8, h->stream));
      RJ_HIP(h, hipMemsetAsync(h->rest[k], 0, n * 4, h->stream));
    }
    RJ_HIP(h, hipStreamSynchronize(h->stream));
  }
  h->last_passes = walk ? 3 : 1;
  h->last_walk_points = 1;
  h->last_prepared = 0;
  tic(h, RJ_T_PIP_KERNEL, st);
  if (n && walk) {
    const int wflip = h->flip_walk[si];
    PipArgs w = a;
    w.work_counter = (unsigned int*) (h->d_counter + (aux ? kSchedWalkAux : kSchedWalkMain) + wflip * kSchedBlockWords);
    w.next_work_counter = (unsigned int*) (h->d_counter + (aux ? kSchedWalkAux : kSchedWalkMain) + (1 - wflip) * kSchedBlockWords);
    w.rest = h->rest[li];
    w.rest_count = h->d_counter + kRestCountWord + 2 * si + wflip;
    w.next_rest_count = h->d_counter + kRestCountWord + 2 * si + (1 - wflip);
    if (own) {
      w.rest_count = h->d_counter + kExactRestWord[h->exact_rot];
      w.next_rest_count = h->d_counter + kExactRestWord[(h->exact_rot + 1) % 3];
      h->exact_rot = (h->exact_rot + 1) % 3;
      if (h->exact_recorded[h->exact_buf]) RJ_HIP(h, hipStreamWaitEvent(st, h->ev_exact_done[h->exact_buf], 0));
      if (h->exact_last >= 0 && h->exact_recorded[h->exact_last] &&
          (h->exact_out_closest == (const void*) closest_eid_dev || (face_id_dev && h->exact_out_face == (const void*) face_id_dev)))
        RJ_HIP(h, hipStreamWaitEvent(st, h->ev_exact_done[h->exact_last], 0));
    }
    w.todo = h->todo[li]; w.todo_mask = h->todo_mask[li];
    if (!w.group_lanes) w.group_lanes = pip_walk_group_lanes(n, w.bvh.top, h->cus);
    const bool two = h->walk_points >= 2 && w.group_lanes == 64 && !h->chunk_groups && pip_walk2_blocks_per_cu(w.bvh.top) >= 6 &&
                     n >= (uint64_t) 2 * 256 * 4 * h->cus * pip_walk2_blocks_per_cu(w.bvh.top);
    tic(h, RJ_T_PIP_WALK, st);
    const bool columns = w.bvh.strips.ytab != nullptr;
    h->last_columns = columns ? 1 : 0;
    if (columns) {
      w.group_lanes = 64;
      RJ_HIP(h, launch_pip_strip(st, w, walk_blocks, h->cus));
    } else if (two) {
      if (aux && h->lsi_shared && !h->pip_share_set)
        walk_blocks = h->cus * pip_walk2_blocks_beside(w.bvh.top, walk_share_of_this_pair / h->cus < 1 ? 1 : walk_share_of_this_pair / h->cus);
      const MapState& q = h->map[query_map_id];
      if (!pts_dev && !order && !h->stats_on && q.qpts) {
        w.qpts = q.qpts + pt_begin;
        h->last_prepared = 1;
        if (pt_begin % 64 == 0) { w.qext = q.qext + pt_begin / 64; h->last_prepared = 2; }
      }
      RJ_HIP(h, launch_pip_walk2(st, w, walk_blocks, h->cus, h->stats_on));
      h->last_walk_points = 2;
    } else {
      RJ_HIP(h, launch_pip_walk(st, w, h->stats_on, walk_blocks));
    }
    if (aux && h->lsi_shared) h->last_pip_share = walk_blocks;
    h->plan.pip.first = columns ? last_strip_launch() : last_launch();
    toc(h, RJ_T_PIP_WALK, st);
    h->flip_walk[si] = 1 - wflip;
    const uint64_t left = seen != ~0ull ? seen : 8192;
    PipRestArgs r;
    r.order = h->rest[li];
    r.n_dev = w.rest_count;
    r.rest_count = h->d_rest + si;
    r.work_counter = a.work_counter;
    r.next_work_counter = a.next_work_counter;
    r.group_lanes = left < 8192 ? 1 : (left * 100 < n ? 4 : (left * 10 < n ? 8 : 16));
    r.chunk_groups = 1;
    int rest_blocks = h->cus * 4;
    if (seen != ~0ull) {
      const uint64_t want = seen / (r.group_lanes * 4 * 2) + 1;
      const uint64_t lo = (uint64_t) h->cus / 4, hi = (uint64_t) h->cus * 4;
      rest_blocks = (int) (want < lo ? lo : (want > hi ? hi : want));
    }
    r.blocks = (uint32_t) rest_blocks;
    h->walk_n[si] = n;
    if (own) {
      RJ_HIP(h, hipEventRecord(h->ev_walk_done, st));
      RJ_HIP(h, hipStreamWaitEvent(h->exact_stream, h->ev_walk_done, 0));
      RJ_HIP(h, launch_pip_exact(h->exact_stream, w, h->cus * 8, r));
      RJ_HIP(h, hipEventRecord(h->ev_exact_done[h->exact_buf], h->exact_stream));
      h->exact_recorded[h->exact_buf] = true;
      h->exact_last = h->exact_buf;
      h->exact_out_closest = closest_eid_dev; h->exact_out_face = face_id_dev;
      h->exact_buf ^= 1;
      h->exact_pending = true;
    } else {
      RJ_HIP(h, launch_pip_exact(st, w, h->cus * 8, r));
    }
    h->flip_pip[si] = 1 - pflip;
    h->plan.pip.exact_blocks = h->cus * 8; h->plan.pip.locate_blocks = rest_blocks;
    if (columns) why = "the base map has a column index (closed rings or short chains: index[].columns_why): the first pass reads the point's strip";
    else if (!two && h->walk_points >= 2) why = "one point per lane: a query set too small for full groups on every resident wave (or a debug knob set)";
  } else if (n) {
    if (aux && h->exact_pending && h->exact_last >= 0) RJ_HIP(h, hipStreamWaitEvent(st, h->ev_exact_done[h->exact_last], 0));
    RJ_HIP(h, launch_pip(st, a, h->stats_on, max_blocks));
    h->flip_pip[aux ? 1 : 0] = 1 - pflip;
    h->plan.pip.first = last_launch();
    h->plan.pip.exact_blocks = h->plan.pip.locate_blocks = 0;
  }
  {
    rj_handle_s::PlanRec::Pip& pp = h->plan.pip;
    pp.ran = n > 0; pp.epoch = h->plan.epoch; pp.n = n; pp.aux = aux; pp.caller = pts_dev != nullptr;
    pp.shared = aux && h->lsi_shared; pp.passes = h->last_passes; pp.rest_hint = seen; pp.why = why;
    pp.order = order ? (h->order_fresh ? 2 : 1) : 0;
    pp.prepared = h->last_prepared;
  }
  toc(h, RJ_T_PIP_KERNEL, own ? h->exact_stream : st);
  if (h->cur_caller >= 0 && n) {
    const rj_handle_s::CallerSet& e = h->caller[h->cur_caller];
    if (e.queries <= 2 || e.queries % 4 == 0) RJ_HIP(h, launch_group_extent_tail(st, pts, h->cur_order, n, h->d_est + h->cur_caller));
  }
  if (aux) h->aux_pending = true;
  return RJ_OK;
}

int rj_pip_query(rj_handle h, int base_map_id, int query_map_id, const int64_t* pts_dev,
                 uint64_t pt_begin, uint64_t n, uint32_t* closest_eid_dev, int32_t* face_id_dev) {
  RJ_CHECK_H(h);
  if (int r = rj_pip_query_async(h, base_map_id, query_map_id, pts_dev, pt_begin, n, closest_eid_dev, face_id_dev)) return r;
  if (h->stats_on) RJ_HIP(h, hipMemcpyAsync(h->h_pinned + 1, h->d_stats, 128, hipMemcpyDeviceToHost, h->stream));
  RJ_HIP(h, hipStreamSynchronize(h->stream));
  RJ_HIP(h, join_aux(h));
  if (h->stats_on) for (int i = 0; i < 16; i++) h->last_stats[i] = h->h_pinned[1 + i];
  return check_fault(h);
}

static int order_distance_points(rj_handle h, const int64_t* pts, bool callers, int query_map_id, uint64_t coh_begin, uint64_t n, const uint32_t** order_out) {
  const uint32_t* order = nullptr;
  h->lazy_columns_ok = false;
  bool given_order = false;
  for (const auto& u : h->nearest_unordered) given_order = given_order || (u.valid && u.p == pts && u.n == n);
  if (!given_order) {
    const std::string err_before = h->err;
    const int r = h->debug_nearest_order_nomem ? RJ_E_NOMEM : maybe_order_queries(h, true, pts, nullptr, 0, n, &order, callers ? -1 : query_map_id, coh_begin);
    if (r == RJ_E_NOMEM) {
      (void) hipGetLastError();
      h->err = err_before;
      rj_handle_s::NearestUnordered& u = h->nearest_unordered[h->nearest_unordered_next];
      h->nearest_unordered_next = (h->nearest_unordered_next + 1) % rj_handle_s::kNearestUnordered;
      u.p = pts; u.n = n; u.valid = true;
      given_order = true;
    } else if (r != RJ_OK) {
      return r;
    }
  }
  if (given_order) {
    order = nullptr;
    h->last_ordered = false; h->order_fresh = false; h->cur_caller = -1; h->cur_order = nullptr;
  }
  *order_out = order;
  return RJ_OK;
}
static int estimate_distance_points(rj_handle h, const int64_t* pts, uint64_t n) {
  if (h->cur_caller >= 0) {
    const rj_handle_s::CallerSet& e = h->caller[h->cur_caller];
    if (e.queries <= 2 || e.queries % 4 == 0) RJ_HIP(h, launch_group_extent_tail(h->stream, pts, h->cur_order, n, h->d_est + h->cur_caller));
  }
  return RJ_OK;
}

int rj_nearest_query(rj_handle h, int base_map_id, int query_map_id, const int64_t* pts_dev, uint64_t pt_begin, uint64_t n, int64_t max_dist,
                     uint32_t* eid_dev, rj_near* rec_dev, double* dist_dev) {
  static_assert(sizeof(rj_near) == 40 && sizeof(nearest::Near) == 40, "layouts");
  static_assert(RJ_MISS_EID == nearest::kMissEid, "the miss value");
  RJ_CHECK_H(h);
  h->nearest_report = StageMs{};
  if (base_map_id < 0 || base_map_id > 1 || query_map_id != 1 - base_map_id)
    return fail(h, RJ_E_INVALID, "rj_nearest_query: base/query map ids must be {0,1} and differ");
  if (!h->bvh[base_map_id].built) return fail(h, RJ_E_INVALID, "rj_nearest_query: call rj_build_lbvh(base map) first");
  if (n && !eid_dev) return fail(h, RJ_E_INVALID, "rj_nearest_query: null output");
  if (max_dist > nearest::kMaxDist) return fail(h, RJ_E_INVALID, "rj_nearest_query: max_dist must not exceed 2^48 (negative: unlimited)");
  const int64_t* pts = pts_dev;
  uint64_t coh_begin = 0;
  if (!pts) {
    coh_begin = pt_begin;
    const MapState& q = h->map[query_map_id];
    if (!q.present || pt_begin + n > q.np || pt_begin + n < pt_begin) return fail(h, RJ_E_INVALID, "rj_nearest_query: bad point range of the query map");
    pts = q.pts + 2 * pt_begin;
  }
  if (n >= (1ull << 32)) return fail(h, RJ_E_INVALID, "rj_nearest_query: n < 2^32");
  if (n == 0) return RJ_OK;
  if (int r = set_device(h)) return r;
  StageEvents ev;
  RJ_HIP(h, ev.create());
  RJ_HIP(h, ev.mark(0, h->stream));
  const uint32_t* order = nullptr;
  if (int r = order_distance_points(h, pts, pts_dev != nullptr, query_map_id, coh_begin, n, &order)) return r;
  if (h->stats_on) RJ_HIP(h, hipMemsetAsync(h->d_stats, 0, 128, h->stream));
  NearestArgs a;
  a.bvh = bvh_view(h->bvh[base_map_id]);
  a.pts = pts; a.n = n; a.order = order;
  a.max_dist = max_dist;
  a.eid = eid_dev; a.rec = reinterpret_cast<nearest::Near*>(rec_dev); a.dist = dist_dev;
  a.fault = h->d_fault;
  a.stats = h->stats_on ? h->d_stats : nullptr;
  a.stack_cap = h->debug_stack_cap;
  RJ_HIP(h, ev.mark(1, h->stream));
  RJ_HIP(h, launch_nearest(h->stream, a, h->stats_on != 0, h->debug_nearest_blocks, h->cus));
  RJ_HIP(h, ev.mark(2, h->stream));
  if (int r = estimate_distance_points(h, pts, n)) return r;
  if (h->stats_on) RJ_HIP(h, hipMemcpyAsync(h->h_pinned + 1, h->d_stats, 128, hipMemcpyDeviceToHost, h->stream));
  RJ_HIP(h, hipStreamSynchronize(h->stream));
  ev.times(2, h->nearest_report.ms);
  if (h->stats_on) for (int i = 0; i < 16; i++) h->last_stats[i] = h->h_pinned[1 + i];
  if (h->h_fault[kFaultNearestStack]) {
    h->h_fault[kFaultNearestStack] = 0;
    return fail(h, RJ_E_INTERNAL, "traversal stack overflow in k_nearest: results are incomplete");
  }
  return RJ_OK;
}

int rj_within_query(rj_handle h, int base_map_id, int query_map_id, const int64_t* pts_dev, uint64_t pt_begin, uint64_t n, int64_t max_dist,
                    uint64_t pair_capacity, uint64_t* offsets_dev, uint32_t* eid_dev, rj_near* rec_dev, double* dist_dev, rj_within_counts* counts) {
  static_assert(sizeof(rj_within_counts) == sizeof(within::Counts), "layouts");
  RJ_CHECK_H(h);
  h->within_report = StageMs{};
  if (base_map_id < 0 || base_map_id > 1 || query_map_id != 1 - base_map_id)
    return fail(h, RJ_E_INVALID, "rj_within_query: base/query map ids must be {0,1} and differ");
  if (!h->bvh[base_map_id].built) return fail(h, RJ_E_INVALID, "rj_within_query: call rj_build_lbvh(base map) first");
  if (!counts) return fail(h, RJ_E_INVALID, "rj_within_query: counts is null");
  if (pair_capacity && !eid_dev) return fail(h, RJ_E_INVALID, "rj_within_query: pair_capacity without eid_dev");
  if (max_dist < 0 || max_dist > nearest::kMaxDist) return fail(h, RJ_E_INVALID, "rj_within_query: max_dist must lie in [0, 2^48]");
  const int64_t* pts = pts_dev;
  uint64_t coh_begin = 0;
  if (!pts) {
    coh_begin = pt_begin;
    const MapState& q = h->map[query_map_id];
    if (!q.present || pt_begin + n > q.np || pt_begin + n < pt_begin) return fail(h, RJ_E_INVALID, "rj_within_query: bad point range of the query map");
    pts = q.pts + 2 * pt_begin;
  }
  if (n >= within::kMaxPoints || pair_capacity >= within::kMaxPoints) return fail(h, RJ_E_INVALID, "rj_within_query: n < 2^32 and pair_capacity < 2^32");
  if (int r = set_device(h)) return r;
  memset(counts, 0, sizeof(*counts));
  if (n == 0) {
    if (offsets_dev) {
      RJ_HIP(h, hipMemsetAsync(offsets_dev, 0, sizeof(uint64_t), h->stream));
      RJ_HIP(h, hipStreamSynchronize(h->stream));
    }
    return RJ_OK;
  }
  StageEvents ev;
  RJ_HIP(h, ev.create());
  RJ_HIP(h, ev.mark(0, h->stream));
  const uint32_t* order = nullptr;
  if (int r = order_distance_points(h, pts, pts_dev != nullptr, query_map_id, coh_begin, n, &order)) return r;
  if (int r = estimate_distance_points(h, pts, n)) return r;
  if (h->stats_on) RJ_HIP(h, hipMemsetAsync(h->d_stats, 0, 128, h->stream));
  WithinArgs a;
  a.bvh = bvh_view(h->bvh[base_map_id]);
  a.seg = h->map[base_map_id].seg;
  a.pts = pts; a.n = n; a.order = order;
  a.max_dist = max_dist;
  a.capacity = pair_capacity;
  a.offsets = offsets_dev;
  a.eid = eid_dev; a.rec = reinterpret_cast<nearest::Near*>(rec_dev); a.dist = dist_dev;
  a.fault = h->d_fault;
  a.stats = h->stats_on ? h->d_stats : nullptr;
  a.stack_cap = h->debug_stack_cap;
// ... 1014 lines not shown
```

### rayjoin_amd/csrc/rj_kernels.h

```cpp
#pragma once
#include "../../include/rayjoin_amd.h"
#include "rj_device.h"

namespace rj {

struct XsectRec {
  int64_t x_num, x_den, y_num, y_den;
  uint32_t eid0, eid1;
  int32_t mid, pad;
};
static_assert(sizeof(XsectRec) == 48, "Intersection record must be 48 bytes");
static_assert(sizeof(Seg) == 32 && sizeof(QBox) == 16, "layout");

struct PipRestArgs {
  const uint32_t* order;
  const unsigned long long* n_dev;
  unsigned long long* rest_count;
  unsigned int* work_counter;
  unsigned int* next_work_counter;
  uint32_t group_lanes, chunk_groups;
  uint32_t blocks;
};

struct LsiArgs {
  DeviceBvh bvh;
  const Seg* qseg;
  const uint32_t* qcode;
  const uint32_t* order;
  uint64_t qbeg, qend;
  int base_is_map0;
  uint32_t* out;
  uint64_t cap;
  unsigned long long* counter;
  unsigned int* work_counter;
  unsigned long long* next_counter;
  unsigned int* next_work_counter;
  uint32_t chunk_groups;
  uint32_t group_lanes;
  int stack_cap;
  unsigned long long* stats;
};

struct PipArgs {
  DeviceBvh bvh;
  DeviceMap base;
  const int64_t* pts;
  const uint32_t* order;
  uint64_t n;
  int query_map_id;
  uint32_t* closest;
  int32_t* face;
  unsigned int* work_counter;
  unsigned int* next_work_counter;
  uint32_t chunk_groups;
  uint32_t group_lanes;
  int stack_cap;
  int walk_stack;
  unsigned long long* stats;
  uint32_t* todo;
  unsigned long long* todo_mask;
  uint32_t* rest;
  unsigned long long* rest_count;
  unsigned long long* next_rest_count;
  const unsigned long long* n_dev;
  const int2* qpts;
  const int4* qext;
};

struct GridLsiArgs {
  int g;
  double scale;
  const uint32_t *begin0, *eids0, *begin1, *eids1;
  const Seg *seg0, *seg1;
  uint32_t* out;
  uint64_t cap;
  unsigned long long* counter;
};
struct GridPipArgs {
  int g;
  double scale;
  const uint32_t *begin, *eids;
  DeviceMap base;
  const int64_t* pts;
  uint64_t n;
  int query_map_id;
  uint32_t* closest;
  int32_t* face;
};
hipError_t launch_grid_count(hipStream_t st, const Seg* seg, uint64_t ne, int g, double scale, uint32_t* counts,
                             unsigned long long* total);
hipError_t launch_grid_emit(hipStream_t st, const Seg* seg, uint64_t ne, int g, double scale, uint64_t* keys,
                            unsigned long long* cursor);
hipError_t launch_grid_unpack(hipStream_t st, const uint64_t* keys, uint64_t n, uint32_t* eids);
hipError_t scan_cell_counts(hipStream_t st, void* temp, size_t& temp_bytes, const uint32_t* counts, uint32_t* begin, uint64_t n);
hipError_t launch_lsi_grid(hipStream_t st, const GridLsiArgs& a);
hipError_t launch_pip_grid(hipStream_t st, const GridPipArgs& a);

hipError_t launch_build_segs(hipStream_t st, const int64_t* pts, const uint32_t* edge_begin,
                             uint32_t nc, uint64_t ne, Seg* seg, uint32_t* edge_chain, uint32_t* ccode);
hipError_t launch_prepare_points(hipStream_t st, const int64_t* pts, uint64_t np, int2* qpts, int4* qext);
hipError_t launch_morton(hipStream_t st, const Seg* seg, uint64_t ne, MortonKey* keys, uint32_t* vals);
hipError_t sort_morton_pairs(hipStream_t st, void* temp, size_t& temp_bytes, const MortonKey* kin, MortonKey* kout,
                             const uint32_t* vin, uint32_t* vout, uint64_t n);
hipError_t sort_pairs_u64_u32(hipStream_t st, void* temp, size_t& temp_bytes, const uint64_t* kin,
                              uint64_t* kout, const uint32_t* vin, uint32_t* vout, uint64_t n, unsigned begin_bit = 0,
                              unsigned end_bit = 64);
hipError_t sort_keys_u64(hipStream_t st, void* temp, size_t& temp_bytes, const uint64_t* kin,
                         uint64_t* kout, uint64_t n);
hipError_t launch_xsect_keys(hipStream_t st, const XsectRec* rec, uint64_t n, int im, uint64_t* keys, uint32_t* vals);
hipError_t launch_xsect_gather(hipStream_t st, const XsectRec* in, const uint32_t* order, uint64_t n, XsectRec* out);
hipError_t launch_xsect_order_runs(hipStream_t st, XsectRec* rec, uint64_t n, int im, const Seg* seg_im, int64_t* midpts);
hipError_t launch_xsect_set_mid(hipStream_t st, XsectRec* rec, uint64_t n, int im, const int32_t* face);
hipError_t launch_swap_halves(hipStream_t st, uint64_t* v, uint64_t n);
hipError_t warm_query_kernels(hipStream_t st);
hipError_t warm_grid_kernels(hipStream_t st);
hipError_t warm_stitch_kernels(hipStream_t st);
hipError_t warm_strip_kernels(hipStream_t st);
hipError_t warm_overlay_kernels(hipStream_t st);
hipError_t launch_strip_width(hipStream_t st, const QBox* box0, const uint32_t* seid, uint64_t n0p, unsigned long long* out2);
hipError_t launch_strip_count(hipStream_t st, const QBox* box0, const uint32_t* seid, uint64_t n0p, int shift, uint32_t* cnt, uint32_t* offs,
                              void* temp, size_t& temp_bytes, uint32_t* flag);
hipError_t launch_strip_fill(hipStream_t st, const QBox* box0, const uint32_t* seid, const int32_t* sface, const uint32_t* cnt,
                             const uint32_t* offs, uint64_t n0p, int shift, uint64_t entries, uint32_t* key, uint32_t* eslot, uint32_t* key_tmp,
                             uint32_t* slot_tmp, uint32_t* tall, uint32_t* ytab, QBox* ebox, uint4* einfo, uint2* tall_end, uint32_t* sky, void* temp,
                             size_t& temp_bytes);
hipError_t launch_pip_strip(hipStream_t st, const PipArgs& a, int max_blocks, int cus);
void stitch_output_bounds(uint64_t nc, uint64_t ne, uint32_t cap, uint64_t* max_pieces, uint64_t* max_runs);
hipError_t stitch_runs_device(hipStream_t st, const int64_t* pts, const uint32_t* edge_begin, uint64_t nc, uint64_t ne, uint32_t cap,
                              uint32_t* piece_begin, uint32_t* piece_len, uint32_t* run_first, uint64_t* nruns, uint64_t* npieces,
                              uint32_t* stats ,
                              char** scratch, size_t* scratch_bytes );
hipError_t launch_run_keys(hipStream_t st, const Seg* seg, const uint32_t* piece_begin, const uint32_t* piece_len, const uint32_t* run_first,
                           uint64_t nruns, MortonKey* keys, uint32_t* vals, uint32_t* run_len, QBox* run_box, uint32_t box_upto);
uint64_t pack_runs_chunks(uint64_t nruns);
hipError_t launch_pack_runs(hipStream_t st, const uint32_t* order, const uint32_t* run_len, const QBox* run_box, uint64_t nruns,
                            uint32_t solo_above, uint32_t spread, uint32_t* chunk_leaves, uint32_t* chunk_base, uint32_t* leaf_first,
                            unsigned long long* total_out);
hipError_t launch_build_leaves(hipStream_t st, const Seg* seg, const uint32_t* order, const uint32_t* edge_chain,
                               const uint32_t* left, const uint32_t* right, uint64_t ne, const uint32_t* piece_begin,
                               const uint32_t* piece_len, const uint32_t* run_first, const uint32_t* run_len, const uint32_t* leaf_first, uint64_t nblocks,
                               uint64_t n_parent_alloc, Seg* sseg, uint32_t* seid, int32_t* sface, QBox* box0,
                               int32_t* pmx1, uint2* xtab, QBox* lvl1, uint32_t* occ, uint2* ytab2 = nullptr);
hipError_t launch_occ_count(hipStream_t st, const uint32_t* occ, unsigned long long* part16, unsigned long long* out_mapped);
hipError_t launch_build_sky(hipStream_t st, const QBox* box0, const uint32_t* seid, uint64_t n0p, uint32_t* sky);
hipError_t launch_sibling_order(hipStream_t st, const QBox* box, uint64_t n_alloc, uint64_t* higher);
hipError_t launch_reduce_level(hipStream_t st, const QBox* child, uint64_t n_child_alloc, QBox* parent,
                               uint64_t n_parent_alloc);
struct LaunchNote { const char* kernel; int grid; int per_lane; };
LaunchNote last_launch();
LaunchNote last_strip_launch();
hipError_t launch_lsi(hipStream_t st, const LsiArgs& a, bool stats, int max_blocks, int segs_per_lane = 1, int* segs_used = nullptr);
hipError_t launch_group_extent(hipStream_t st, bool points, const int64_t* pts, const Seg* segs, uint64_t begin,
                               uint64_t n, unsigned long long* out2);
hipError_t launch_group_extent_tail(hipStream_t st, const int64_t* pts, const uint32_t* order, uint64_t n, unsigned long long* out_mapped);
hipError_t launch_query_keys(hipStream_t st, bool points, const int64_t* pts, const Seg* segs, uint64_t begin,
                             uint64_t n, MortonKey* keys, uint32_t* vals);
hipError_t launch_lsi_points(hipStream_t st, const Seg* seg0, const Seg* seg1, const uint32_t* pairs,
                             uint64_t n, const unsigned long long* n_dev, XsectRec* out, uint32_t* slow_list,
                             unsigned long long* slow_count, unsigned long long* next_slow_count,
                             unsigned long long* count_hint);
hipError_t launch_pip(hipStream_t st, const PipArgs& a, bool stats, int max_blocks);
hipError_t launch_pip_walk(hipStream_t st, const PipArgs& a, bool stats, int max_blocks);
hipError_t launch_pip_walk2(hipStream_t st, const PipArgs& a, int max_blocks, int cus, bool stats = false);
int pip_walk2_blocks_per_cu(int top);
int pip_walk2_blocks_beside(int top, int lsi_blocks_per_cu);
hipError_t launch_pip_exact(hipStream_t st, const PipArgs& a, int blocks, const PipRestArgs& r);
int pip_walk_list_slots();
uint32_t pip_walk_group_lanes(uint64_t n, int top, int cus);
int pip_walk_blocks_per_cu(int top);

struct OverlayFacesMap {
  const int64_t* pts;
  const uint32_t *edge_chain, *edge_begin, *left, *right;
  uint64_t ne, nc;
};
struct OverlayOp {
  uint32_t how, by;
};
hipError_t overlay_faces_device(hipStream_t st, const OverlayFacesMap maps[2], const rj_xsect* const xsects[2], uint64_t n,
                                const int32_t* const vertex_face[2], uint64_t capacity, rj_overlay_face* out, uint64_t* n_rows,
                                char** scratch, size_t* scratch_bytes, const OverlayOp* op = nullptr);

}
```

### rayjoin_amd/csrc/rj_kernels.hip

```cpp
#include "rj_kernels.h"

#include <cstring>
#include <rocprim/device/device_radix_sort.hpp>

namespace rj {

__device__ __forceinline__ uint32_t cell_code(const Seg& s) {
  const int cx0 = quant(s.x1 < s.x2 ? s.x1 : s.x2) >> kOccShift, cx1 = quant(s.x1 < s.x2 ? s.x2 : s.x1) >> kOccShift;
  const int cy0 = quant(s.y1 < s.y2 ? s.y1 : s.y2) >> kOccShift, cy1 = quant(s.y1 < s.y2 ? s.y2 : s.y1) >> kOccShift;
  const int dx = cx1 - cx0 > 1 ? 2 : cx1 - cx0, dy = cy1 - cy0 > 1 ? 2 : cy1 - cy0;
  return (uint32_t) cx0 | ((uint32_t) cy0 << 12) | ((uint32_t) dx << 24) | ((uint32_t) dy << 26);
}
__global__ __launch_bounds__(256) void k_build_segs(const int64_t* __restrict__ pts,
                                                    const uint32_t* __restrict__ edge_begin,
                                                    uint32_t nc, uint64_t ne, Seg* __restrict__ seg,
                                                    uint32_t* __restrict__ edge_chain, uint32_t* __restrict__ ccode) {
  for (uint64_t e = blockIdx.x * (uint64_t) blockDim.x + threadIdx.x; e < ne;
       e += (uint64_t) gridDim.x * blockDim.x) {
    uint32_t lo = 0, hi = nc;
    while (hi - lo > 1) {
      uint32_t mid = lo + ((hi - lo) >> 1);
      if (edge_begin[mid] <= e) lo = mid; else hi = mid;
    }
    uint64_t p = e + lo;
// ... 1540 lines not shown
    }
    if (STATS) tk_head += clock64() - tkg;
    while (sp > 0) {
      --sp;
      uint4 ent;
      asm volatile("ds_read_b128 %0, %1\n\ts_waitcnt lgkmcnt(0)" : "=v"(ent) : "v"(stack_lds + (uint32_t) sp * 16u) : "memory");
      const int32_t ey0 = (int32_t) ent.y, ex0 = (int32_t) ent.z, ex1 = (int32_t) ent.w;
      const bool want = ((uint32_t) (qx - ex0) <= (uint32_t) (ex1 - ex0)) & (qbest >= ey0);
      if (!__ballot(want)) {
        if (STATS) st_stale++;
        continue;
      }
      const uint32_t e = __builtin_amdgcn_readfirstlane(ent.x);
      const long long tk0 = STATS ? clock64() : 0;
      const int lvl = (int) (e >> 28);
      const uint32_t idx = e & 0x0FFFFFFFu;
      if (lvl > 1) {
        const QBox b = T.lvl[lvl - 1][(uint64_t) idx * 64 + lane];
        const uint64_t higher = sibling_order(T, lvl - 1)[(uint64_t) idx * 64 + lane];
        uint64_t m = refine_if_many(b, __ballot(b.x0 <= gx1 && gx0 <= b.x1 && b.y1 >= gy0 - 1 && b.y0 <= gbest));
        if (sp + __popcll(m) > stack_cap) { ovf = true; break; }
        if ((m >> lane) & 1)
          stack[sp + __popcll(m & higher)] =
              make_uint4(((uint32_t) (lvl - 1) << 28) | (idx * 64 + lane), (uint32_t) b.y0, (uint32_t) b.x0, (uint32_t) b.x1);
        sp += __popcll(m);
        wave_lds_fence();
        if (STATS) {
          sp_max = sp > sp_max ? sp : sp_max;
          st_nodes++;
          tk_node += clock64() - tk0;
        }
      } else {
        const uint32_t slot0 = idx * 64;
        const QBox bb = T.box0[(uint64_t) slot0 + lane];
        const uint2 tab = T.xtab[(uint64_t) slot0 + lane];
        const uint32_t sx0s = __builtin_amdgcn_readfirstlane((uint32_t) ex0);
        const int sh = leaf_bucket_shift(__builtin_amdgcn_readfirstlane((uint32_t) ex1) - sx0s);
        const uint32_t bk = want ? ((uint32_t) qx - sx0s) >> sh : 0u;
        const uint32_t bsh = (bk & 3u) * 8u;
        const uint32_t hi = ((uint32_t) __shfl((int) tab.x, (int) (bk >> 2), 64) >> bsh) & 0xFFu;
        const uint32_t lo = ((uint32_t) __shfl((int) tab.y, (int) (bk >> 2), 64) >> bsh) & 0xFFu;
        int j = (int) hi - 1, jlo = (int) lo;
        {
          const int32_t top_x0 = __builtin_amdgcn_ds_bpermute(j << 2, bb.x0);
          const int32_t low_x1 = __builtin_amdgcn_ds_bpermute(jlo << 2, bb.x1);
          j -= top_x0 > qx ? 1 : 0;
          jlo += low_x1 < qx ? 1 : 0;
        }
        j = want ? j : -1;
        jlo = want ? jlo : 0;
        const int32_t qbest_before = qbest;
        if (STATS) {
          st_leaf++;
          st_leaf_lanes += (unsigned long long) __popcll(__ballot(want));
        }
        while (__ballot(j >= jlo)) {
          const int jj = j & 63;
          const int ja = j << 2;
          const int32_t sx0 = __builtin_amdgcn_ds_bpermute(ja, bb.x0), sx1 = __builtin_amdgcn_ds_bpermute(ja, bb.x1);
          const int32_t sy0 = __builtin_amdgcn_ds_bpermute(ja, bb.y0), sy1 = __builtin_amdgcn_ds_bpermute(ja, bb.y1);
          if (STATS) st_box++;
          if ((sx0 <= qx) & (qx <= sx1) & (sy1 >= qym1) & (qbest >= sy0) & (j >= jlo)) {
            const bool certain = sx0 < qx && qx < sx1 && sy0 > qy;
            const bool replace = certain && sy1 < sure_y0;
            const bool first = cand_at == cand_base;
            const bool over = !replace && cand_at == cand_base + kWalkList * 64;
            cand[(replace || over) ? cand_base : cand_at] = slot0 + (uint32_t) jj;
            sure_y0 = (replace || (first && certain)) ? sy0 : INT32_MIN;
            cand_at += replace ? 0u : 64u;
            const int32_t top = certain ? sy1 + 1 : 0x7FFFFFFF;
            qbest = over ? -1 : (top < qbest ? top : qbest);
          }
          j--;
        }
        if (__ballot(qbest != qbest_before)) {
          const int32_t gbest_before = gbest;
          gbest = wave_max(qbest);
          if (gbest < gbest_before && sp > 1) {
            int kept = 0;
            for (int base = 0; base < sp; base += 64) {
              const int i = base + lane;
              const bool have = i < sp;
              uint4 en = make_uint4(0, 0, 0, 0);
              if (have) en = stack[i];
              const bool alive = have && (int32_t) en.y <= gbest;
              const uint64_t am = __ballot(alive);
              wave_lds_fence();
              if (alive) stack[kept + rank_below(am)] = en;
              kept += __popcll(am);
            }
            if (STATS) st_stale += (unsigned long long) (sp - kept);
            sp = kept;
            wave_lds_fence();
          }
        }
        if (STATS) tk_leaf += clock64() - tk0;
      }
    }
    const long long tkt = STATS ? clock64() : 0;
    const bool done = valid && !ovf && (cand_at == cand_base || sure_y0 != INT32_MIN);
    {
      const bool hit = done && cand_at != cand_base;
      const uint32_t slot = hit ? cand[lane] : 0u;
      const uint32_t e = T.seid[slot];
      const int32_t f = A.face ? T.sface[slot] : 0;
      if (done) {
        __builtin_nontemporal_store(hit ? e : 0xFFFFFFFFu, A.closest + ip);
        if (A.face) __builtin_nontemporal_store(hit ? f : 0, A.face + ip);
      }
    }
    const uint32_t fill = (cand_at - cand_base) >> 6;
    const bool listed = valid && !done && !ovf && fill <= (uint32_t) kWalkList;
    const bool rest = valid && !done && !listed;
    const uint64_t lm = __ballot(listed);
    if (listed) {
      const uint64_t rec = (uint64_t) g32 * GL + rank_below(lm);
#pragma unroll
      for (int k = 0; k < kWalkList; k++) A.todo[rec * kWalkList + k] = (uint32_t) k < fill ? cand[lane + 64 * k] : 0xFFFFFFFFu;
    }
    if (lane == 0) A.todo_mask[g32] = lm;
    const uint64_t rm = __ballot(rest);
    if (rm) {
      unsigned long long base = 0;
      if (lane == 0) base = atomicAdd(A.rest_count, (unsigned long long) __popcll(rm));
      base = ((unsigned long long) __builtin_amdgcn_readfirstlane((uint32_t) (base >> 32)) << 32) | __builtin_amdgcn_readfirstlane((uint32_t) base);
      if (rest) A.rest[base + rank_below(rm)] = ip;
    }
    wave_lds_fence();
    if (STATS) {
      if (lane == 0 && A.stats) atomicMax(&A.stats[8], (unsigned long long) sp_max);
      st_rest += (unsigned long long) __popcll(rm);
      tk_tail += clock64() - tkt;
    }
  }
  if (STATS && lane == 0 && A.stats) {
    const long long tk_total = clock64() - tk_begin;
    atomicAdd(&A.stats[0], st_leaf);
    atomicAdd(&A.stats[1], st_rest);
    atomicAdd(&A.stats[2], st_nodes);
    atomicAdd(&A.stats[3], st_box);
    atomicAdd(&A.stats[4], (unsigned long long) tk_total);
    atomicAdd(&A.stats[5], (unsigned long long) tk_node);
    atomicAdd(&A.stats[6], (unsigned long long) tk_leaf);
    atomicMax(&A.stats[9], (unsigned long long) tk_total);
    atomicAdd(&A.stats[10], (unsigned long long) tk_sched);
    atomicAdd(&A.stats[11], (unsigned long long) tk_head);
    atomicAdd(&A.stats[12], (unsigned long long) tk_tail);
    atomicAdd(&A.stats[13], st_stale);
    atomicAdd(&A.stats[15], st_leaf_lanes);
  }
}


__host__ __device__ __forceinline__ size_t walk2_wave_lds(int top, int P = 2) { return (size_t) 16 * walk_stack_entries(top) + (size_t) kWalkList * 256 * P; }

constexpr int kWalkCycleStamps = 7777;
template <bool STATS, int P, bool PREP = false>
__device__ __forceinline__ void pip_walk_many(const PipArgs& A) {
  extern __shared__ uint4 walk_smem[];
  const int lane = lane_id();
  const int wib = threadIdx.x >> 6;
  const DeviceBvh& T = A.bvh;
  const uint32_t* const sky = (T.sky && T.sky[kSkyBuckets] == 0u) ? T.sky : nullptr;
  const int stack_entries = walk_stack_entries(T.top);
  const int stack_cap = A.walk_stack > 0 && A.walk_stack < stack_entries ? A.walk_stack : stack_entries;
  uint4* const stack = walk_smem + (size_t) wib * (walk2_wave_lds(T.top, P) / 16);
  uint32_t* const cand = reinterpret_cast<uint32_t*>(stack + stack_entries);
  const uint32_t stack_lds = (uint32_t) (uintptr_t) stack;
  constexpr uint32_t GP = 64u * P;
  const uint64_t ngroups = (A.n + GP - 1) / GP;
  const uint32_t nchunks = (uint32_t) ((ngroups + A.chunk_groups - 1) / A.chunk_groups);
  int part = blockIdx.x & 7, tried = 0;
  __shared__ unsigned long long ranges[4];
  if (threadIdx.x < 4) ranges[threadIdx.x] = 0;
  if (blockIdx.x == 0 && threadIdx.x < 8) A.next_work_counter[threadIdx.x * 32] = 0;
  if (blockIdx.x == 0 && threadIdx.x == 8) *A.next_rest_count = 0;
  __syncthreads();
  unsigned long long st_pops = 0, st_stale = 0, st_nodes = 0, st_leaf = 0, st_setvisits = 0, st_steps = 0, st_pushed = 0, st_sweeps = 0, st_swept = 0,
                     st_groups = 0, st_want = 0, st_hits = 0, st_rest = 0;
  const bool cyc = STATS && A.stack_cap == kWalkCycleStamps;
  long long ck_sched = 0, ck_load = 0, ck_head = 0, ck_pop = 0, ck_node_wait = 0, ck_node = 0, ck_leaf_wait = 0, ck_leaf = 0, ck_bound = 0, ck_tail = 0;
  const long long ck_begin = STATS ? clock64() : 0;
#define RJ_CK(var, since) do { if (STATS && cyc) { const long long _n = clock64(); var += _n - since; since = _n; } } while (0)
  for (;;) {
    uint32_t g32 = 0;
    long long ck = STATS && cyc ? clock64() : 0;
    if (!next_group<4>(ranges, wib, A.work_counter, nchunks, A.chunk_groups, ngroups, part, tried, lane, g32)) break;
    RJ_CK(ck_sched, ck);
    typedef long long ll2_t __attribute__((ext_vector_type(2)));
    int32_t qx[P], qy[P], qbest[P], sure_y0[P];
    uint32_t cand_base[P], cand_at[P];
    bool valid[P];
    typedef int i2_t __attribute__((ext_vector_type(2)));
    typedef int i4_t __attribute__((ext_vector_type(4)));
    typedef const __attribute__((address_space(4))) i4_t* ext_ptr_t;
    constexpr bool prep = PREP;
    const uint32_t gu = __builtin_amdgcn_readfirstlane(g32);
    const bool full = prep && gu < (uint32_t) (A.n / GP);
    const bool ext = full && A.qext != nullptr;
    uint32_t ipl[P];
    if (full) {
#pragma unroll
      for (int p = 0; p < P; p++) { valid[p] = true; ipl[p] = 0; }
    } else {
#pragma unroll
      for (int p = 0; p < P; p++) {
        const uint64_t ipos = (uint64_t) g32 * GP + (uint64_t) p * 64 + lane;
        valid[p] = ipos < A.n;
        const uint64_t ipc = valid[p] ? ipos : A.n - 1;
        ipl[p] = !prep && A.order ? A.order[ipc] : (uint32_t) ipc;
      }
    }
    i4_t ext0 = {0, 0, 0, 0}, ext1 = {0, 0, 0, 0};
    if (ext) {
      const ext_ptr_t E = (ext_ptr_t) (uintptr_t) A.qext + (uint64_t) gu * P;
      ext0 = E[0];
      ext1 = E[1];
    }
    ll2_t ptl[P];
    i2_t qpl[P];
    if (full) {
      const i2_t* const q = reinterpret_cast<const i2_t*>(A.qpts) + (uint64_t) gu * GP + lane;
#pragma unroll
      for (int p = 0; p < P; p++) qpl[p] = __builtin_nontemporal_load(q + 64 * p);
    } else if (prep) {
#pragma unroll
      for (int p = 0; p < P; p++) qpl[p] = __builtin_nontemporal_load(reinterpret_cast<const i2_t*>(A.qpts) + ipl[p]);
    } else {
#pragma unroll
      for (int p = 0; p < P; p++) ptl[p] = __builtin_nontemporal_load(reinterpret_cast<const ll2_t*>(A.pts) + ipl[p]);
    }
    const QBox root_box = T.lvl[T.top][lane];
    const uint64_t root_higher = sibling_order(T, T.top)[lane];
    if (STATS && cyc) { asm volatile("s_waitcnt vmcnt(0)" ::: "memory"); RJ_CK(ck_load, ck); }
#pragma unroll
    for (int p = 0; p < P; p++) {
      if (full) {
        qx[p] = qpl[p].x;
        qy[p] = qpl[p].y;
        qbest[p] = 0x7FFFFFFF;
      } else if (prep) {
        qx[p] = valid[p] ? qpl[p].x : 0;
        qy[p] = valid[p] ? qpl[p].y : 0;
        qbest[p] = valid[p] ? 0x7FFFFFFF : -1;
      } else {
        qx[p] = valid[p] ? quant(ptl[p].x) : 0;
        qy[p] = valid[p] ? quant(ptl[p].y) : 0;
        qbest[p] = valid[p] ? 0x7FFFFFFF : -1;
      }
      cand_base[p] = (uint32_t) lane + (uint32_t) p * (kWalkList * 64);
      cand_at[p] = cand_base[p];
      sure_y0[p] = INT32_MIN;
    }
    if (sky) {
#pragma unroll
      for (int p = 0; p < P; p++)
        if (sky[(uint32_t) qx[p] >> kSkyShift] <= (uint32_t) qy[p]) qbest[p] = -1;
    }
    int32_t gx0, gx1, gy0;
    bool ext_ok = ext;
    if (ext && sky) {
      bool gone = qbest[0] < 0;
#pragma unroll
      for (int p = 1; p < P; p++) gone = gone || qbest[p] < 0;
      ext_ok = !__ballot(gone);
    }
    if (ext_ok) {
      gx0 = ext0.x < ext1.x ? ext0.x : ext1.x;
      gx1 = ext0.y > ext1.y ? ext0.y : ext1.y;
      gy0 = ext0.z < ext1.z ? ext0.z : ext1.z;
    } else {
      const bool l0 = qbest[0] >= 0, l1 = qbest[1] >= 0;
      const int32_t a0 = l0 ? qx[0] : kEmptyMin, a1 = l1 ? qx[1] : kEmptyMin;
      const int32_t b0 = l0 ? qx[0] : kEmptyMax, b1 = l1 ? qx[1] : kEmptyMax;
      const int32_t c0 = l0 ? qy[0] : kEmptyMin, c1 = l1 ? qy[1] : kEmptyMin;
      gx0 = a0 < a1 ? a0 : a1; gx1 = b0 > b1 ? b0 : b1; gy0 = c0 < c1 ? c0 : c1;
#pragma unroll
      for (int p = 2; p < P; p++) {
        const bool lp = qbest[p] >= 0;
        const int32_t ap = lp ? qx[p] : kEmptyMin, bp = lp ? qx[p] : kEmptyMax, cp = lp ? qy[p] : kEmptyMin;
        gx0 = gx0 < ap ? gx0 : ap; gx1 = gx1 > bp ? gx1 : bp; gy0 = gy0 < cp ? gy0 : cp;
      }
      wave_min_max_min(gx0, gx1, gy0);
    }
    int32_t gbest = 0x7FFFFFFF;
    bool gbest_stale = false;

    auto refine_if_many = [&](const QBox& b, uint64_t um) -> uint64_t {
      if (__popcll(um) <= kPipRefineAbove) return um;
      uint64_t keep = 0;
      while (um) {
        const int c = __builtin_ctzll(um);
        um &= um - 1;
        const int32_t cx0 = bcast(b.x0, c), cy0 = bcast(b.y0, c);
        const int32_t cx1 = bcast(b.x1, c), cy1 = bcast(b.y1, c);
        bool any = ray_can_hit(qx[0], qy[0] > 0 ? qy[0] - 1 : 0, qbest[0], cx0, cy0, cx1, cy1) || ray_can_hit(qx[1], qy[1] > 0 ? qy[1] - 1 : 0, qbest[1], cx0, cy0, cx1, cy1);
#pragma unroll
        for (int p = 2; p < P; p++) any = any || ray_can_hit(qx[p], qy[p] > 0 ? qy[p] - 1 : 0, qbest[p], cx0, cy0, cx1, cy1);
        if (__ballot(any)) keep |= 1ull << c;
      }
      return keep;
    };
    int sp = 0;
    bool ovf = false;
    {
      const QBox b = root_box;
      const uint64_t higher = root_higher;
      uint64_t m = refine_if_many(b, __ballot(b.x0 <= gx1 && gx0 <= b.x1 && b.y1 >= gy0 - 1));
      if (__popcll(m) > stack_cap) { m = 0; ovf = true; }
      if ((m >> lane) & 1)
        stack[__popcll(m & higher)] = make_uint4(((uint32_t) T.top << 28) | (uint32_t) lane, (uint32_t) b.y0, (uint32_t) b.x0, (uint32_t) b.x1);
      sp = __popcll(m);
      wave_lds_fence();
      if (STATS) { st_groups++; st_pushed += (unsigned long long) sp; }
    }
    RJ_CK(ck_head, ck);
    while (sp > 0) {
      --sp;
      uint4 ent;
      if (STATS) st_pops++;
      asm volatile("ds_read_b128 %0, %1\n\ts_waitcnt lgkmcnt(0)" : "=v"(ent) : "v"(stack_lds + (uint32_t) sp * 16u) : "memory");
      const int32_t ey0 = (int32_t) ent.y, ex0 = (int32_t) ent.z, ex1 = (int32_t) ent.w;
      const uint32_t ew = (uint32_t) (ex1 - ex0);
      bool want[P];
      bool want_any = false;
#pragma unroll
      for (int p = 0; p < P; p++) {
        want[p] = ((uint32_t) (qx[p] - ex0) <= ew) & (qbest[p] >= ey0);
        want_any = want_any || want[p];
      }
      if (!__ballot(want_any)) {
        if (STATS) st_stale++;
        RJ_CK(ck_pop, ck);
        continue;
      }
      RJ_CK(ck_pop, ck);
      const uint32_t e = __builtin_amdgcn_readfirstlane(ent.x);
      const int lvl = (int) (e >> 28);
      const uint32_t idx = e & 0x0FFFFFFFu;
      if (lvl > 1) {
        uint32_t lane_here = (uint32_t) lane;
        asm volatile("" : "+v"(lane_here));
        const QBox b = T.lvl[lvl - 1][(uint64_t) idx * 64 + lane_here];
        const uint64_t higher = sibling_order(T, lvl - 1)[(uint64_t) idx * 64 + lane_here];
        if (STATS && cyc) { asm volatile("s_waitcnt vmcnt(0)" ::: "memory"); RJ_CK(ck_node_wait, ck); }
        if (gbest_stale) {
          gbest_stale = false;
          int32_t lane_best = qbest[0] > qbest[1] ? qbest[0] : qbest[1];
#pragma unroll
          for (int p = 2; p < P; p++) lane_best = lane_best > qbest[p] ? lane_best : qbest[p];
          gbest = wave_max(lane_best);
        }
        uint64_t m = refine_if_many(b, __ballot(b.x0 <= gx1 && gx0 <= b.x1 && b.y1 >= gy0 - 1 && b.y0 <= gbest));
        if (sp + __popcll(m) > stack_cap) { ovf = true; break; }
        if ((m >> lane) & 1)
          stack[sp + __popcll(m & higher)] =
              make_uint4(((uint32_t) (lvl - 1) << 28) | (idx * 64 + lane), (uint32_t) b.y0, (uint32_t) b.x0, (uint32_t) b.x1);
        sp += __popcll(m);
        wave_lds_fence();
        if (STATS) { st_nodes++; st_pushed += (unsigned long long) __popcll(m); }
        RJ_CK(ck_node, ck);
      } else {
        if (STATS) st_leaf++;
        const uint32_t slot0 = idx * 64;
        uint32_t lane_here = (uint32_t) lane;
        asm volatile("" : "+v"(lane_here));
        const QBox bb = T.box0[(uint64_t) slot0 + lane_here];
        const uint2 tab = T.xtab[(uint64_t) slot0 + lane_here];
        if (STATS && cyc) { asm volatile("s_waitcnt vmcnt(0)" ::: "memory"); RJ_CK(ck_leaf_wait, ck); }
        const uint32_t sx0s = __builtin_amdgcn_readfirstlane((uint32_t) ex0);
        const int sh = leaf_bucket_shift(__builtin_amdgcn_readfirstlane((uint32_t) ex1) - sx0s);
        bool changed = false;
#pragma unroll
        for (int p = 0; p < P; p++) {
          if (!__ballot(want[p])) continue;
          if (STATS) { st_setvisits++; st_want += (unsigned long long) __popcll(__ballot(want[p])); }
          const uint32_t bk = ((uint32_t) qx[p] - sx0s) >> sh;
          const uint32_t bsh = (bk & 3u) * 8u;
          const uint32_t hi = ((uint32_t) __shfl((int) tab.x, (int) (bk >> 2), 64) >> bsh) & 0xFFu;
          const uint32_t lo = ((uint32_t) __shfl((int) tab.y, (int) (bk >> 2), 64) >> bsh) & 0xFFu;
          int j = (int) hi - 1, jlo = (int) lo;
          {
            const int32_t top_x0 = __builtin_amdgcn_ds_bpermute(j << 2, bb.x0);
            const int32_t low_x1 = __builtin_amdgcn_ds_bpermute(jlo << 2, bb.x1);
            j -= top_x0 > qx[p] ? 1 : 0;
            jlo += low_x1 < qx[p] ? 1 : 0;
          }
          j = want[p] ? j : -1;
          const int32_t qbest_before = qbest[p];
          auto scan_step = [&]() {
                  if (STATS) st_steps++;
            const int jj = j & 63;
            const int ja = j << 2;
            const int32_t sx0 = __builtin_amdgcn_ds_bpermute(ja, bb.x0), sx1 = __builtin_amdgcn_ds_bpermute(ja, bb.x1);
            const int32_t sy0 = __builtin_amdgcn_ds_bpermute(ja, bb.y0), sy1 = __builtin_amdgcn_ds_bpermute(ja, bb.y1);
            if ((sx0 <= qx[p]) & (qx[p] <= sx1) & (sy1 >= qy[p] - 1) & (qbest[p] >= sy0) & (j >= jlo)) {
              const bool certain = sx0 < qx[p] && qx[p] < sx1 && sy0 > qy[p];
              const bool replace = certain && sy1 < sure_y0[p];
              const bool first = cand_at[p] == cand_base[p];
              const bool over = !replace && cand_at[p] == cand_base[p] + kWalkList * 64;
              if (STATS && lane == __builtin_ctzll(__ballot(true))) st_hits++;
              cand[(replace || over) ? cand_base[p] : cand_at[p]] = slot0 + (uint32_t) jj;
              sure_y0[p] = (replace || (first && certain)) ? sy0 : INT32_MIN;
              cand_at[p] += replace ? 0u : 64u;
              const int32_t top = certain ? sy1 + 1 : 0x7FFFFFFF;
              qbest[p] = over ? -1 : (top < qbest[p] ? top : qbest[p]);
            }
            j--;
          };
          if (__ballot(j >= jlo)) {
            scan_step();
            while (__ballot(j >= jlo)) scan_step();
          }
          changed = changed || qbest[p] != qbest_before;
        }
        RJ_CK(ck_leaf, ck);
        if (__ballot(changed)) gbest_stale = true;
        if (gbest_stale && sp > 1) {
          gbest_stale = false;
          const int32_t gbest_before = gbest;
          int32_t lane_best = qbest[0] > qbest[1] ? qbest[0] : qbest[1];
#pragma unroll
          for (int p = 2; p < P; p++) lane_best = lane_best > qbest[p] ? lane_best : qbest[p];
          gbest = wave_max(lane_best);
          if (gbest < gbest_before && sp > 1) {
            int kept = 0;
            if (STATS) st_sweeps++;
            for (int base = 0; base < sp; base += 64) {
              const int i = base + lane;
              const bool have = i < sp;
              uint4 en = make_uint4(0, 0, 0, 0);
              if (have) en = stack[i];
              const bool alive = have && (int32_t) en.y <= gbest;
              const uint64_t am = __ballot(alive);
              wave_lds_fence();
              if (alive) stack[kept + rank_below(am)] = en;
              kept += __popcll(am);
            }
            if (STATS) st_swept += (unsigned long long) (sp - kept);
            sp = kept;
            wave_lds_fence();
          }
        }
        RJ_CK(ck_bound, ck);
      }
    }
    RJ_CK(ck_bound, ck);
    uint32_t out_e[P], ipv[P];
    int32_t out_f[P];
    bool donev[P];
#pragma unroll
    for (int p = 0; p < P; p++) {
      const uint64_t ipos = (uint64_t) g32 * GP + (uint64_t) p * 64 + lane;
      ipv[p] = !PREP && A.order ? A.order[valid[p] ? ipos : A.n - 1] : (uint32_t) ipos;
      donev[p] = valid[p] && !ovf && (cand_at[p] == cand_base[p] || sure_y0[p] != INT32_MIN);
      const bool hit = donev[p] && cand_at[p] != cand_base[p];
      const uint32_t slot = hit ? cand[cand_base[p]] : 0u;
      const uint32_t e = T.seid[slot];
      const int32_t f = A.face ? T.sface[slot] : 0;
      out_e[p] = hit ? e : 0xFFFFFFFFu;
      out_f[p] = hit ? f : 0;
    }
#pragma unroll
    for (int p = 0; p < P; p++) {
      const uint32_t fill = (cand_at[p] - cand_base[p]) >> 6;
      const bool listed = valid[p] && !donev[p] && !ovf && fill <= (uint32_t) kWalkList;
      const bool rest = valid[p] && !donev[p] && !listed;
      const uint64_t lm = __ballot(listed);
      const uint64_t g64 = (uint64_t) g32 * P + p;
      if (listed) {
        const uint64_t rec = g64 * 64 + rank_below(lm);
#pragma unroll
        for (int k = 0; k < kWalkList; k++) A.todo[rec * kWalkList + k] = (uint32_t) k < fill ? cand[cand_base[p] + 64 * k] : 0xFFFFFFFFu;
      }
      if (lane == 0 && g64 * 64 < A.n) A.todo_mask[g64] = lm;
      const uint64_t rm = __ballot(rest);
      if (rm) {
        unsigned long long base = 0;
        if (lane == 0) base = atomicAdd(A.rest_count, (unsigned long long) __popcll(rm));
        base = ((unsigned long long) __builtin_amdgcn_readfirstlane((uint32_t) (base >> 32)) << 32) | __builtin_amdgcn_readfirstlane((uint32_t) base);
        if (rest) A.rest[base + rank_below(rm)] = ipv[p];
      }
      if (STATS) st_rest += (unsigned long long) __popcll(rm);
    }
#pragma unroll
    for (int p = 0; p < P; p++) {
      if (donev[p]) {
        __builtin_nontemporal_store(out_e[p], A.closest + ipv[p]);
        if (A.face) __builtin_nontemporal_store(out_f[p], A.face + ipv[p]);
      }
    }
    wave_lds_fence();
    if (STATS && cyc) { asm volatile("s_waitcnt vmcnt(0)" ::: "memory"); RJ_CK(ck_tail, ck); }
  }
#undef RJ_CK
  if (STATS && A.stats && cyc) {
    if (lane == 0) {
      const long long total = clock64() - ck_begin;
      atomicAdd(&A.stats[0], (unsigned long long) total);
      atomicAdd(&A.stats[1], (unsigned long long) ck_sched);
      atomicAdd(&A.stats[2], (unsigned long long) ck_load);
      atomicAdd(&A.stats[3], (unsigned long long) ck_head);
      atomicAdd(&A.stats[4], st_groups);
      atomicAdd(&A.stats[5], (unsigned long long) ck_pop);
      atomicAdd(&A.stats[6], (unsigned long long) ck_node_wait);
      atomicAdd(&A.stats[7], (unsigned long long) ck_node);
      atomicAdd(&A.stats[8], (unsigned long long) ck_leaf_wait);
      atomicAdd(&A.stats[9], (unsigned long long) ck_leaf);
      atomicAdd(&A.stats[10], (unsigned long long) ck_bound);
      atomicAdd(&A.stats[11], (unsigned long long) ck_tail);
      atomicAdd(&A.stats[12], 1ull);
    }
    return;
  }
  if (STATS && A.stats) {
    const unsigned long long hits = st_hits;
    if (hits) atomicAdd(&A.stats[6], hits);
    if (lane == 0) {
      atomicAdd(&A.stats[0], st_leaf);
      atomicAdd(&A.stats[1], st_rest);
      atomicAdd(&A.stats[2], st_nodes);
      atomicAdd(&A.stats[3], st_steps);
      atomicAdd(&A.stats[4], st_groups);
      atomicAdd(&A.stats[5], st_setvisits);
      atomicAdd(&A.stats[7], st_sweeps);
      atomicAdd(&A.stats[8], st_swept);
      atomicAdd(&A.stats[10], st_pops);
      atomicAdd(&A.stats[11], st_pushed);
      atomicAdd(&A.stats[13], st_stale);
      atomicAdd(&A.stats[15], st_want);
    }
  }
}


__global__ __launch_bounds__(256, 8) __attribute__((amdgpu_num_sgpr(96))) __attribute__((amdgpu_num_vgpr(28))) void k_pip_walk2(PipArgs A) { pip_walk_many<false, 2>(A); }
__global__ __launch_bounds__(256, 4) __attribute__((amdgpu_num_sgpr(96))) void k_pip_walk2_stats(PipArgs A) { pip_walk_many<true, 2>(A); }
__global__ __launch_bounds__(256, 8) __attribute__((amdgpu_num_sgpr(96))) __attribute__((amdgpu_num_vgpr(28))) void k_pip_walk2_prepared(PipArgs A) { pip_walk_many<false, 2, true>(A); }


#ifndef RJ_EXACT_WAVES
#define RJ_EXACT_WAVES 5
#endif
static_assert(kPipWaves == 4, "k_pip_exact's first blocks run pip_locate: same block size");
__global__ __launch_bounds__(256, RJ_EXACT_WAVES) void k_pip_exact(PipArgs A, PipRestArgs R) {
  if (blockIdx.x < R.blocks) {
    pip_locate<false>(A, blockIdx.x, R, nullptr);
    return;
  }
  __shared__ uint32_t queue[4][128];
  __shared__ uint32_t qrec[4][128];
  const DeviceBvh& T = A.bvh;
  const int lane = lane_id();
  const int wib = threadIdx.x >> 6;
  const uint32_t gl_shift = 31 - __builtin_clz(A.group_lanes);
  const uint64_t wave = ((blockIdx.x - R.blocks) * (uint64_t) blockDim.x + threadIdx.x) >> 6;
  const uint64_t nwaves = ((uint64_t) (gridDim.x - R.blocks) * blockDim.x) >> 6;
  auto evaluate = [&](uint32_t i, uint32_t rec) {
    const uint64_t ip = A.order ? A.order[i] : i;
    uint32_t slot[kWalkList];
#pragma unroll
    for (int r = 0; r < kWalkList; r++) slot[r] = A.todo[(uint64_t) rec * kWalkList + r];
    typedef long long ll2_t __attribute__((ext_vector_type(2)));
    const ll2_t pxy = reinterpret_cast<const ll2_t*>(A.pts)[ip];
    const int64_t px = pxy.x, py = pxy.y;
    double best_yy = __builtin_inf();
    uint32_t best_slot = 0xFFFFFFFFu;
    Seg best_seg = {0, 0, 0, 0};
    int64_t best_lo = INT64_MAX, best_hi = INT64_MAX;
    bool best_exact = false;
    Seg cur = {0, 0, 0, 0}, nxt = {0, 0, 0, 0};
    if (slot[0] != 0xFFFFFFFFu) cur = T.sseg[slot[0]];
    if (slot[1] != 0xFFFFFFFFu) nxt = T.sseg[slot[1]];
#pragma unroll
    for (int r = 0; r < kWalkList; r++) {
      if (slot[r] == 0xFFFFFFFFu) break;
      const Seg e = cur;
      cur = nxt;
      if (r + 2 < kWalkList && slot[r + 2] != 0xFFFFFFFFu) nxt = T.sseg[slot[r + 2]];
      const int64_t x_min = e.x1 < e.x2 ? e.x1 : e.x2, x_max = e.x1 < e.x2 ? e.x2 : e.x1;
      if (px < x_min || px > x_max || px == (A.query_map_id == 0 ? x_min : x_max)) continue;
      const int64_t ylo = e.y1 < e.y2 ? e.y1 : e.y2, yhi = e.y1 < e.y2 ? e.y2 : e.y1;
      if (yhi <= py - 1) continue;
      if (ylo >= py + 1 && ylo > best_hi) continue;
      if (ylo >= py + 1 && yhi < best_lo) {
        best_slot = slot[r]; best_seg = e; best_lo = ylo; best_hi = yhi; best_exact = false;
        continue;
      }
      if (best_slot != 0xFFFFFFFFu && !best_exact) {
        double byy;
        (void) pip_eval_y(best_seg, px, py, A.query_map_id, &byy);
        best_yy = byy; best_exact = true;
      }
      double yy;
      if (pip_eval_y(e, px, py, A.query_map_id, &yy)) {
        bool better = yy < best_yy;
        if (yy == best_yy && best_slot != 0xFFFFFFFFu)
          better = pip_better(yy, pip_slope(e), T.seid[slot[r]], best_yy, pip_slope(best_seg), T.seid[best_slot], A.query_map_id);
        if (better) {
          best_yy = yy; best_slot = slot[r]; best_seg = e; best_lo = ylo; best_hi = yhi; best_exact = true;
        }
      }
    }
    const bool hit = best_slot != 0xFFFFFFFFu;
    A.closest[ip] = hit ? T.seid[best_slot] : 0xFFFFFFFFu;
    if (A.face) A.face[ip] = hit ? T.sface[best_slot] : 0;
  };
  int nq = 0;
  const uint64_t ngroups = (A.n + A.group_lanes - 1) >> gl_shift;
  for (uint64_t g0 = wave * 16; g0 < ngroups; g0 += nwaves * 16) {
    unsigned long long mine = 0;
    if (lane < 16 && g0 + lane < ngroups) mine = A.todo_mask[g0 + lane];
    uint64_t any = __ballot(mine != 0);
    while (any) {
      const int k = __builtin_ctzll(any);
      any &= any - 1;
      const uint64_t m = ((uint64_t) (uint32_t) __builtin_amdgcn_readlane((int) (mine >> 32), k) << 32) |
                         (uint32_t) __builtin_amdgcn_readlane((int) mine, k);
      if ((m >> lane) & 1) {
        const uint32_t r = rank_below(m);
        queue[wib][nq + r] = (uint32_t) (((g0 + k) << gl_shift) + lane);
        qrec[wib][nq + r] = (uint32_t) ((g0 + k) << gl_shift) + r;
      }
      nq += __popcll(m);
      wave_lds_fence();
      if (nq >= 64) {
        evaluate(queue[wib][nq - 64 + lane], qrec[wib][nq - 64 + lane]);
        nq -= 64;
        wave_lds_fence();
      }
    }
  }
  if (lane < nq) evaluate(queue[wib][lane], qrec[wib][lane]);
}

__global__ void k_noop() {}
hipError_t warm_query_kernels(hipStream_t st) {
  hipLaunchKernelGGL(k_noop, dim3(1), dim3(1), 0, st);
  return hipGetLastError();
}

static thread_local LaunchNote g_note = {"", 0, 0};
LaunchNote last_launch() { return g_note; }
static inline void note(const char* kernel, int grid, int per_lane) { g_note.kernel = kernel; g_note.grid = grid; g_note.per_lane = per_lane; }

static inline int grid_for(uint64_t work_items, int per_block, int max_blocks) {
  uint64_t b = (work_items + per_block - 1) / per_block;
  if (b < 1) b = 1;
  if (b > (uint64_t) max_blocks) b = max_blocks;
  return (int) b;
}

hipError_t launch_build_segs(hipStream_t st, const int64_t* pts, const uint32_t* edge_begin,
                             uint32_t nc, uint64_t ne, Seg* seg, uint32_t* edge_chain, uint32_t* ccode) {
  if (ne == 0) return hipSuccess;
  hipLaunchKernelGGL(k_build_segs, dim3(grid_for(ne, 256, 8192)), dim3(256), 0, st, pts, edge_begin,
                     nc, ne, seg, edge_chain, ccode);
  return hipGetLastError();
}

hipError_t launch_prepare_points(hipStream_t st, const int64_t* pts, uint64_t np, int2* qpts, int4* qext) {
  if (np == 0) return hipSuccess;
  hipLaunchKernelGGL(k_prepare_points, dim3(grid_for(np, 256, 8192)), dim3(256), 0, st, pts, np, qpts, qext);
  return hipGetLastError();
}

hipError_t launch_morton(hipStream_t st, const Seg* seg, uint64_t ne, MortonKey* keys, uint32_t* vals) {
  if (ne == 0) return hipSuccess;
  hipLaunchKernelGGL(k_morton, dim3(grid_for(ne, 256, 8192)), dim3(256), 0, st, seg, ne, keys, vals);
  return hipGetLastError();
}

hipError_t sort_pairs_u64_u32(hipStream_t st, void* temp, size_t& temp_bytes, const uint64_t* kin,
                              uint64_t* kout, const uint32_t* vin, uint32_t* vout, uint64_t n, unsigned begin_bit,
                              unsigned end_bit) {
  return rocprim::radix_sort_pairs(temp, temp_bytes, kin, kout, vin, vout, (size_t) n, begin_bit, end_bit, st);
}

hipError_t sort_morton_pairs(hipStream_t st, void* temp, size_t& temp_bytes, const MortonKey* kin, MortonKey* kout,
                             const uint32_t* vin, uint32_t* vout, uint64_t n) {
  return rocprim::radix_sort_pairs(temp, temp_bytes, kin, kout, vin, vout, (size_t) n, 0, 64 - kMortonDropBits, st);
}

hipError_t sort_keys_u64(hipStream_t st, void* temp, size_t& temp_bytes, const uint64_t* kin,
                         uint64_t* kout, uint64_t n) {
  return rocprim::radix_sort_keys(temp, temp_bytes, kin, kout, (size_t) n, 0, 64, st);
}

hipError_t launch_xsect_keys(hipStream_t st, const XsectRec* rec, uint64_t n, int im, uint64_t* keys, uint32_t* vals) {
  if (n) hipLaunchKernelGGL(k_xsect_keys, dim3(grid_for(n, 256, 4096)), dim3(256), 0, st, rec, n, im, keys, vals);
  return hipGetLastError();
// ... 61 lines not shown
hipError_t launch_build_sky(hipStream_t st, const QBox* box0, const uint32_t* seid, uint64_t n0p, uint32_t* sky) {
  hipLaunchKernelGGL(k_build_sky, dim3(grid_for(n0p, 256, 8192)), dim3(256), 0, st, box0, seid, n0p, sky);
  return hipGetLastError();
}

hipError_t launch_sibling_order(hipStream_t st, const QBox* box, uint64_t n_alloc, uint64_t* higher) {
  hipLaunchKernelGGL(k_sibling_order, dim3(grid_for(n_alloc / 64, 4, 8192)), dim3(256), 0, st, box, n_alloc, higher);
  return hipGetLastError();
}

hipError_t launch_reduce_level(hipStream_t st, const QBox* child, uint64_t n_child_alloc, QBox* parent,
                               uint64_t n_parent_alloc) {
  hipLaunchKernelGGL(k_reduce_level, dim3(grid_for(n_parent_alloc, 4, 8192)), dim3(256), 0, st, child,
                     n_child_alloc, parent, n_parent_alloc);
  return hipGetLastError();
}

static int resident_blocks(const void* kernel, int max_blocks, int block_threads = 256) {
  int dev = 0, cus = 256, per_cu = 4;
  hipDeviceProp_t prop;
  if (hipGetDevice(&dev) == hipSuccess && hipGetDeviceProperties(&prop, dev) == hipSuccess) cus = prop.multiProcessorCount;
  if (hipOccupancyMaxActiveBlocksPerMultiprocessor(&per_cu, kernel, block_threads, 0) != hipSuccess || per_cu < 1) per_cu = 4;
  int b = cus * per_cu;
  return b < max_blocks ? b : max_blocks;
}

static uint32_t pick_group_lanes(uint64_t nqueries, int resident_blocks_, int block_waves = 4) {
  const uint64_t waves = (uint64_t) resident_blocks_ * block_waves;
  uint32_t gl = 64;
  while (gl > 4 && (nqueries + gl - 1) / gl < 2 * waves) gl >>= 1;
  return gl;
}

static uint32_t pick_chunk_groups(uint32_t requested, uint32_t optimum) { return requested ? requested : optimum; }

hipError_t launch_lsi(hipStream_t st, const LsiArgs& a_in, bool stats, int max_blocks, int segs_per_lane, int* segs_used) {
  LsiArgs a = a_in;
  if (segs_used) *segs_used = 1;
  const bool ys = a.bvh.ytab2 != nullptr;
  const void* k = stats ? (const void*) k_lsi<true> : (const void*) k_lsi<false>;
  static int res[2] = {0, 0};
  if (!res[stats]) res[stats] = resident_blocks(k, 1 << 20);
  const bool auto_lanes = !a.group_lanes;
  if (!a.group_lanes) a.group_lanes = pick_group_lanes(a.qend - a.qbeg, res[stats]);
  if (segs_per_lane == 2 && !stats && auto_lanes && a.group_lanes == 64 && !a.chunk_groups &&
      pick_group_lanes((a.qend - a.qbeg) / 2, res[0]) == 64) {
    static int res2 = 0;
    if (!res2) res2 = resident_blocks((const void*) k_lsi2, 1 << 20);
    const uint64_t ngroups = (a.qend - a.qbeg + 127) / 128;
    a.chunk_groups = 4;
    const uint64_t nchunks = (ngroups + a.chunk_groups - 1) / a.chunk_groups;
    int grid = grid_for(nchunks, 4, res2 < max_blocks ? res2 : max_blocks);
    const uint64_t per_wave = a.bvh.occ_permille >= kOccDensePermille ? 5 : 10;
    const uint64_t by_work = ngroups / (4 * per_wave);
    const int floor_blocks = 512 < grid ? 512 : grid;
    if (by_work < (uint64_t) grid) grid = by_work > (uint64_t) floor_blocks ? (int) by_work : floor_blocks;
    if (ys) { note("k_lsi2", grid, 2); hipLaunchKernelGGL(k_lsi2, dim3(grid), dim3(256), 0, st, a); }
    else { note("k_lsi2x", grid, 2); hipLaunchKernelGGL(k_lsi2x, dim3(grid), dim3(256), 0, st, a); }
    if (segs_used) *segs_used = 2;
    return hipGetLastError();
  }
  uint64_t ngroups = (a.qend - a.qbeg + a.group_lanes - 1) / a.group_lanes;
  a.chunk_groups = pick_chunk_groups(a.chunk_groups, 8);
  uint64_t nchunks = (ngroups + a.chunk_groups - 1) / a.chunk_groups;
  int grid = grid_for(nchunks, 4, res[stats] < max_blocks ? res[stats] : max_blocks);
  const uint64_t by_work = ngroups / (4 * 20);
  const int floor_blocks = 512 < grid ? 512 : grid;
  if (by_work < (uint64_t) grid) grid = by_work > (uint64_t) floor_blocks ? (int) by_work : floor_blocks;
  if (stats)
    { note("k_lsi (instrumented)", grid, 1); if (ys) hipLaunchKernelGGL(k_lsi<true>, dim3(grid), dim3(256), 0, st, a); else hipLaunchKernelGGL(k_lsix<true>, dim3(grid), dim3(256), 0, st, a); }
  else if (ys)
    { note("k_lsi", grid, 1); hipLaunchKernelGGL(k_lsi<false>, dim3(grid), dim3(256), 0, st, a); }
  else
    { note("k_lsix", grid, 1); hipLaunchKernelGGL(k_lsix<false>, dim3(grid), dim3(256), 0, st, a); }
  return hipGetLastError();
}

hipError_t launch_group_extent(hipStream_t st, bool points, const int64_t* pts, const Seg* segs, uint64_t begin,
                               uint64_t n, unsigned long long* out2) {
  const uint64_t ngroups = (n + 63) / 64;
  const uint64_t stride = ngroups > 8192 ? ngroups / 8192 : 1;
  const int grid = grid_for((ngroups + stride - 1) / stride, 4, 512);
  if (points)
    hipLaunchKernelGGL(k_group_extent<true>, dim3(grid), dim3(256), 0, st, pts, segs, begin, n, stride, out2);
  else
    hipLaunchKernelGGL(k_group_extent<false>, dim3(grid), dim3(256), 0, st, pts, segs, begin, n, stride, out2);
  return hipGetLastError();
}

hipError_t launch_group_extent_tail(hipStream_t st, const int64_t* pts, const uint32_t* order, uint64_t n, unsigned long long* out_mapped) {
  hipLaunchKernelGGL(k_group_extent_tail, dim3(1), dim3(1024), 0, st, pts, order, n, out_mapped);
  return hipGetLastError();
}

hipError_t launch_query_keys(hipStream_t st, bool points, const int64_t* pts, const Seg* segs, uint64_t begin,
                             uint64_t n, MortonKey* keys, uint32_t* vals) {
  if (n == 0) return hipSuccess;
  if (points)
    hipLaunchKernelGGL(k_query_keys<true>, dim3(grid_for(n, 256, 8192)), dim3(256), 0, st, pts, segs, begin, n, keys, vals);
  else
    hipLaunchKernelGGL(k_query_keys<false>, dim3(grid_for(n, 256, 8192)), dim3(256), 0, st, pts, segs, begin, n, keys, vals);
  return hipGetLastError();
}

hipError_t launch_lsi_points(hipStream_t st, const Seg* seg0, const Seg* seg1, const uint32_t* pairs,
                             uint64_t n, const unsigned long long* n_dev, XsectRec* out, uint32_t* slow_list,
                             unsigned long long* slow_count, unsigned long long* next_slow_count, unsigned long long* count_hint) {
  if (n == 0) return hipSuccess;
  const uint64_t expect = n_dev ? (n < (1u << 20) ? n : (1u << 20)) : n;
  if (!slow_list || n >= (1ull << 32)) {
    hipLaunchKernelGGL(k_lsi_points_gcd, dim3(grid_for(expect, 256, 4096)), dim3(256), 0, st, seg0, seg1, pairs, n, n_dev,
                       (const uint32_t*) nullptr, (const unsigned long long*) nullptr, count_hint, out);
    return hipGetLastError();
  }
  hipLaunchKernelGGL(k_lsi_points, dim3(grid_for(expect, 256, 2048)), dim3(256), 0, st, seg0, seg1, pairs, n, n_dev, slow_list,
                     slow_count, next_slow_count, count_hint, out);
  hipLaunchKernelGGL(k_lsi_points_gcd, dim3(grid_for(expect / 16 + 1, 256, 1024)), dim3(256), 0, st, seg0, seg1, pairs, n, n_dev,
                     (const uint32_t*) slow_list, (const unsigned long long*) slow_count, (unsigned long long*) nullptr, out);
  return hipGetLastError();
}

int pip_walk_list_slots() { return kWalkList; }

int pip_walk_blocks_per_cu(int top) {
  const size_t block = 4 * walk_wave_lds(top) + 64;
  const size_t by_lds = (size_t) 160 * 1024 / block;
  return (int) (by_lds < 8 ? by_lds : 8);
}

uint32_t pip_walk_group_lanes(uint64_t n, int top, int cus) { return pick_group_lanes(n, cus * pip_walk_blocks_per_cu(top), 4); }

hipError_t launch_pip_walk(hipStream_t st, const PipArgs& a_in, bool stats, int max_blocks) {
  PipArgs a = a_in;
  const size_t lds = 4 * walk_wave_lds(a.bvh.top);
  static int cus = 0;
  if (!cus) {
    int dev = 0;
    hipDeviceProp_t prop;
    cus = hipGetDevice(&dev) == hipSuccess && hipGetDeviceProperties(&prop, dev) == hipSuccess ? prop.multiProcessorCount : 256;
  }
  const int res = cus * pip_walk_blocks_per_cu(a.bvh.top);
  if (!a.group_lanes) a.group_lanes = pick_group_lanes(a.n, res, 4);
  const uint64_t ngroups = (a.n + a.group_lanes - 1) / a.group_lanes;
  a.chunk_groups = pick_chunk_groups(a.chunk_groups, 6);
  const uint64_t nchunks = (ngroups + a.chunk_groups - 1) / a.chunk_groups;
  const int grid = grid_for(nchunks, 4, res < max_blocks ? res : max_blocks);
  if (stats)
    { note("k_pip_walk (instrumented)", grid, 1); hipLaunchKernelGGL(k_pip_walk<true>, dim3(grid), dim3(256), lds, st, a); }
  else
    { note("k_pip_walk", grid, 1); hipLaunchKernelGGL(k_pip_walk<false>, dim3(grid), dim3(256), lds, st, a); }
  return hipGetLastError();
}

int pip_walk2_blocks_per_cu(int top) {
  const size_t block = 4 * walk2_wave_lds(top) + 64;
  const size_t by_lds = (size_t) 160 * 1024 / block;
  return (int) (by_lds < 8 ? by_lds : 8);
}

int pip_walk2_blocks_beside(int top, int lsi_blocks_per_cu) {
  const size_t block = 4 * walk2_wave_lds(top) + 64;
  const size_t left = (size_t) 160 * 1024 > (size_t) lsi_blocks_per_cu * 17920 ? (size_t) 160 * 1024 - (size_t) lsi_blocks_per_cu * 17920 : 0;
  int n = (int) (left / block);
  if (n > 8 - lsi_blocks_per_cu) n = 8 - lsi_blocks_per_cu;
  static int walk_regs = 0, lsi_regs = 0;
  if (!walk_regs) {
    hipFuncAttributes fa;
    walk_regs = hipFuncGetAttributes(&fa, (const void*) k_pip_walk2) == hipSuccess && fa.numRegs > 0 ? (fa.numRegs + 7) / 8 * 8 : 64;
    lsi_regs = hipFuncGetAttributes(&fa, (const void*) k_lsi2) == hipSuccess && fa.numRegs > 0 ? (fa.numRegs + 7) / 8 * 8 : 80;
  }
  const int by_vgpr = (512 - lsi_blocks_per_cu * lsi_regs) / walk_regs;
  if (n > by_vgpr) n = by_vgpr;
  if (n > pip_walk2_blocks_per_cu(top)) n = pip_walk2_blocks_per_cu(top);
  return n < 1 ? 1 : n;
}

hipError_t launch_pip_walk2(hipStream_t st, const PipArgs& a_in, int max_blocks, int cus, bool stats) {
  PipArgs a = a_in;
  const size_t lds = 4 * walk2_wave_lds(a.bvh.top);
  const int res = cus * pip_walk2_blocks_per_cu(a.bvh.top);
  a.group_lanes = 64;
  const uint64_t ngroups = (a.n + 127) / 128;
  a.chunk_groups = a.chunk_groups ? a.chunk_groups : 3;
  const uint64_t nchunks = (ngroups + a.chunk_groups - 1) / a.chunk_groups;
  const int grid = grid_for(nchunks, 4, res < max_blocks ? res : max_blocks);
  note("k_pip_walk2", grid, 2);
  if (stats)
    hipLaunchKernelGGL(k_pip_walk2_stats, dim3(grid), dim3(256), lds, st, a);
  else if (a.qpts)
    hipLaunchKernelGGL(k_pip_walk2_prepared, dim3(grid), dim3(256), lds, st, a);
  else
    hipLaunchKernelGGL(k_pip_walk2, dim3(grid), dim3(256), lds, st, a);
  return hipGetLastError();
}

hipError_t launch_pip_exact(hipStream_t st, const PipArgs& a, int blocks, const PipRestArgs& r) {
  hipLaunchKernelGGL(k_pip_exact, dim3((blocks < 1 ? 1 : blocks) + r.blocks), dim3(256), 0, st, a, r);
  return hipGetLastError();
}

hipError_t launch_pip(hipStream_t st, const PipArgs& a_in, bool stats, int max_blocks) {
  PipArgs a = a_in;
  const void* k = stats ? (const void*) k_pip<true> : (const void*) k_pip<false>;
  static int res[2] = {0, 0};
  if (!res[stats]) res[stats] = resident_blocks(k, 1 << 20, 64 * kPipWaves);
  if (!a.group_lanes) a.group_lanes = pick_group_lanes(a.n, res[stats], kPipWaves);
  uint64_t ngroups = (a.n + a.group_lanes - 1) / a.group_lanes;
  a.chunk_groups = pick_chunk_groups(a.chunk_groups, 6);
  uint64_t nchunks = (ngroups + a.chunk_groups - 1) / a.chunk_groups;
  int grid = grid_for(nchunks, kPipWaves, res[stats] < max_blocks ? res[stats] : max_blocks);
  if (stats)
    { note("k_pip (instrumented)", grid, 1); hipLaunchKernelGGL(k_pip<true>, dim3(grid), dim3(64 * kPipWaves), 0, st, a); }
  else
    { note("k_pip", grid, 1); hipLaunchKernelGGL(k_pip<false>, dim3(grid), dim3(64 * kPipWaves), 0, st, a); }
  return hipGetLastError();
}

}
```

Baseline: 39890 M query segments/s.

## Add three-points-per-lane PIP walk variant when paired with LSI

Adds k_pip_walk3_prepared, which handles three query points per lane instead of two. It keeps the same LDS footprint by shrinking the per-point candidate list to five slots and capping the traversal stack at 76 entries, and it uses lean lane addressing to stay within 28 VGPRs. The variant is used automatically for prepared points when the walk shares the chip with the LSI kernel. A heuristic turns it off for the current epoch if it leaves noticeably more points to the exact-kernel rest list than the two-set walk did. The aim is more traversal work amortised per wave and per BVH node visit, at the cost of more overflow into the slower exact pass.

```diff
diff --git a/rayjoin_amd/csrc/rj_api.hip b/rayjoin_amd/csrc/rj_api.hip
--- a/rayjoin_amd/csrc/rj_api.hip
+++ b/rayjoin_amd/csrc/rj_api.hip
@@ -146,6 +146,12 @@
   int flip_lsi = 0, flip_pip[2] = {0, 0};
   int pip_walk = 1;
   int last_walk_points = 1;
+  int walk_sets = 0;
+  int last_walk_sets = 2;
+  static constexpr int kRest3Word = 5;
+  uint64_t walk_n3 = 0;
+  int rest_sets_aux = 2;
+  uint64_t walk3_off_epoch = ~0ull;
   int last_prepared = 0;
   int last_passes = 0;
   int flip_walk[2] = {0, 0};
@@ -288,6 +294,7 @@
       LaunchNote first = {"", 0, 0};
       int passes = 0, order = 0, exact_blocks = 0, locate_blocks = 0;
       int prepared = 0;
+      int sets = 0;
       const char* why = "";
     } pip;
   } plan;
@@ -604,13 +611,14 @@
     {"pip_schedule_us", 3, RJ_READ(h->co_best[k] < 1e29f ? (int64_t) (h->co_best[k] * 1000.0f) : -1)},
     {"lsi_last_segments", 0, RJ_READ(h->last_lsi_segments)},
     {"pip_last_walk_points", 0, RJ_READ(h->last_walk_points)},
+    {"pip_last_walk_sets", 0, RJ_READ(h->last_walk_sets)},
     {"pip_last_prepared", 0, RJ_READ(h->last_prepared)},
     {"lsi_points_last_split", 0, RJ_READ(h->last_points_split)},
     {"lsi_points_gcd_pairs", 0, read_gcd_pairs},
     {"pip_last_passes", 0, RJ_READ(h->last_passes)},
     {"pip_last_columns", 0, RJ_READ(h->last_columns)},
     {"pip_rest", 0, RJ_READ(h->h_rest[0])},
-    {"pip_rest_aux", 0, RJ_READ(h->h_rest[1])},
+    {"pip_rest_aux", 0, RJ_READ(h->h_rest[h->rest_sets_aux == 3 ? rj_handle_s::kRest3Word : 1])},
     {"leaf_order_used", 2, RJ_READ(h->bvh[k].leaf_order)},
     {"leaf_slots", 2, RJ_READ(h->bvh[k].n0p)},
     {"leaf_runs", 2, RJ_READ(h->map[k].runs_cut ? (int64_t) h->map[k].nruns : -1)},
@@ -732,6 +740,7 @@
   for (const Option& o : kOptions)
     if (const char* e = o.env ? getenv(o.env) : nullptr)
       if (o.accepts(atoi(e))) h->*o.field = atoi(e);
+  if (const char* e = getenv("RJ_WALK_SETS")) { const int v = atoi(e); h->walk_sets = v == 2 || v == 3 ? v : 0; }
   {
     hipDeviceProp_t prop;
     if (hipGetDeviceProperties(&prop, device_id) == hipSuccess && prop.multiProcessorCount > 0) h->cus = prop.multiProcessorCount;
@@ -759,6 +768,7 @@
     h->h_fault[0] = h->h_fault[1] = h->h_fault[kFaultNearestStack] = h->h_fault[kFaultWithinStack] = 0;
     h->h_rest[0] = h->h_rest[1] = ~0ull;
     h->h_rest[2] = ~0ull;
+    h->h_rest[rj_handle_s::kRest3Word] = ~0ull;
     for (int k = 0; k < rj_handle_s::kCallerSets; k++) h->h_est[k] = 0;
     ok = hipMemset(h->d_counter, 0, kCounterBytes) == hipSuccess;
     for (size_t blk : {kSchedLsi, kSchedLsi + kSchedBlockWords, kSchedPipMain, kSchedPipMain + kSchedBlockWords, kSchedPipAux,
@@ -910,10 +920,10 @@
   }
   if (P.pip.ran) {
     add(", \"pip\": {\"epoch\": %llu, \"current\": %s, \"points\": %llu, \"points_from\": \"%s\", \"stream\": \"%s\", \"on_shared_grid\": %s, \"order\": \"%s\", "
-        "\"passes\": %d, \"first_pass\": {\"kernel\": \"%s\", \"blocks\": %d, \"points_per_lane\": %d}, \"prepared_points\": %d",
+        "\"passes\": %d, \"first_pass\": {\"kernel\": \"%s\", \"blocks\": %d, \"points_per_lane\": %d, \"sets\": %d}, \"prepared_points\": %d",
         (unsigned long long) P.pip.epoch, P.pip.epoch == P.epoch ? "true" : "false", (unsigned long long) P.pip.n, P.pip.caller ? "a caller-owned array" : "the query map's vertices",
         P.pip.aux ? "second (beside the LSI query)" : "main", P.pip.shared ? "true" : "false", kOrder[P.pip.order], P.pip.passes, P.pip.first.kernel, P.pip.first.grid,
-        P.pip.first.per_lane, P.pip.prepared);
+        P.pip.first.per_lane, P.pip.sets, P.pip.prepared);
     if (P.pip.passes == 3)
       add(", \"second_pass\": {\"kernel\": \"k_pip_exact\", \"blocks\": %d, \"locate_blocks\": %d}, \"left_over_by_last_query_of_this_size\": %lld", P.pip.exact_blocks,
           P.pip.locate_blocks, P.pip.rest_hint == ~0ull ? -1ll : (long long) P.pip.rest_hint);
@@ -951,7 +961,7 @@
   RJ_HIP(h, join_aux(h));
   co_reset(h);
   h->h_rest[0] = h->h_rest[1] = ~0ull;
-  h->walk_n[0] = h->walk_n[1] = 0;
+  h->walk_n[0] = h->walk_n[1] = 0; h->h_rest[rj_handle_s::kRest3Word] = ~0ull; h->walk_n3 = 0;
   return RJ_OK;
 }
 
@@ -1432,7 +1442,7 @@
   b.built = true;
   co_reset(h);
   h->h_rest[0] = h->h_rest[1] = ~0ull;
-  h->walk_n[0] = h->walk_n[1] = 0;
+  h->walk_n[0] = h->walk_n[1] = 0; h->h_rest[rj_handle_s::kRest3Word] = ~0ull; h->walk_n3 = 0;
   return RJ_OK;
 }
 
@@ -1801,7 +1811,7 @@
         co_reset(h);
         h->plan.epoch++;
         h->h_rest[0] = h->h_rest[1] = ~0ull;
-        h->walk_n[0] = h->walk_n[1] = 0;
+        h->walk_n[0] = h->walk_n[1] = 0; h->h_rest[rj_handle_s::kRest3Word] = ~0ull; h->walk_n3 = 0;
         h->last_ordered = false; h->order_fresh = false; h->cur_caller = -1; h->cur_order = nullptr;
       } else if (int r = maybe_order_queries(h, true, pts, nullptr, 0, n, &order, pts_dev ? -1 : query_map_id, coh_begin)) {
         return r;
@@ -1867,6 +1877,10 @@
     if (seen == ~0ull && h->walk_n[k] == n && h->h_rest[k] != ~0ull) {
       seen = h->h_rest[k];
     }
+  const uint64_t seen3 = h->walk_n3 == n ? (uint64_t) h->h_rest[rj_handle_s::kRest3Word] : ~0ull;
+  constexpr uint64_t kWalk3RestSlack = 2048;
+  if (seen3 != ~0ull && h->walk_sets == 0 && h->walk3_off_epoch != h->plan.epoch && seen3 > (seen != ~0ull ? seen : 0) + kWalk3RestSlack)
+    h->walk3_off_epoch = h->plan.epoch;
   const char* why = !h->pip_walk ? "\"pip_walk\" 0: the exact kernel alone" : (walk ? "" : "instrumented (\"stats\"), no points, or more than 2^32 of them: the exact kernel alone");
   if (walk && h->pip_walk == 1 && seen != ~0ull && (seen * 10 > n * 3 || seen > 16384)) {
     walk = false;
@@ -1894,6 +1908,7 @@
   h->last_passes = walk ? 3 : 1;
   h->last_walk_points = 1;
   h->last_prepared = 0;
+  int walk_sets_now = 2;
   tic(h, RJ_T_PIP_KERNEL, st);
   if (n && walk) {
     const int wflip = h->flip_walk[si];
@@ -1931,8 +1946,16 @@
         h->last_prepared = 1;
         if (pt_begin % 64 == 0) { w.qext = q.qext + pt_begin / 64; h->last_prepared = 2; }
       }
-      RJ_HIP(h, launch_pip_walk2(st, w, walk_blocks, h->cus, h->stats_on));
+      const bool in_pair = aux && h->lsi_inflight && (h->lsi_shared || h->co_mode == 2);
+      const int grid_cap = walk_blocks < h->cus * pip_walk2_blocks_per_cu(w.bvh.top, 3) ? walk_blocks : h->cus * pip_walk2_blocks_per_cu(w.bvh.top, 3);
+      const bool three = h->walk_sets != 2 && w.qpts && in_pair && (h->walk_sets == 3 || h->walk3_off_epoch != h->plan.epoch) &&
+                         n >= (uint64_t) 192 * 4 * 4 * (uint64_t) (grid_cap > 0 ? grid_cap : 1);
+      RJ_HIP(h, launch_pip_walk2(st, w, walk_blocks, h->cus, h->stats_on, three ? 3 : 2));
       h->last_walk_points = 2;
+      h->last_walk_sets = three ? 3 : 2;
+      walk_sets_now = h->last_walk_sets;
+      if (!three && w.qpts && in_pair && h->walk_sets == 0 && h->walk3_off_epoch == h->plan.epoch)
+        why = "two sets per wave: three left far more points to the rest list than two on this pair (five list slots, a stack of 76)";
     } else {
       RJ_HIP(h, launch_pip_walk(st, w, h->stats_on, walk_blocks));
     }
@@ -1940,23 +1963,25 @@
     h->plan.pip.first = columns ? last_strip_launch() : last_launch();
     toc(h, RJ_T_PIP_WALK, st);
     h->flip_walk[si] = 1 - wflip;
-    const uint64_t left = seen != ~0ull ? seen : 8192;
+    const uint64_t hint = walk_sets_now == 3 && seen3 != ~0ull ? seen3 : seen;
+    const uint64_t left = hint != ~0ull ? hint : 8192;
     PipRestArgs r;
     r.order = h->rest[li];
     r.n_dev = w.rest_count;
-    r.rest_count = h->d_rest + si;
+    r.rest_count = h->d_rest + (walk_sets_now == 3 ? rj_handle_s::kRest3Word : si);
     r.work_counter = a.work_counter;
     r.next_work_counter = a.next_work_counter;
     r.group_lanes = left < 8192 ? 1 : (left * 100 < n ? 4 : (left * 10 < n ? 8 : 16));
     r.chunk_groups = 1;
     int rest_blocks = h->cus * 4;
-    if (seen != ~0ull) {
-      const uint64_t want = seen / (r.group_lanes * 4 * 2) + 1;
+    if (hint != ~0ull) {
+      const uint64_t want = hint / (r.group_lanes * 4 * 2) + 1;
       const uint64_t lo = (uint64_t) h->cus / 4, hi = (uint64_t) h->cus * 4;
       rest_blocks = (int) (want < lo ? lo : (want > hi ? hi : want));
     }
     r.blocks = (uint32_t) rest_blocks;
-    h->walk_n[si] = n;
+    if (walk_sets_now == 3) h->walk_n3 = n; else h->walk_n[si] = n;
+    if (si) h->rest_sets_aux = walk_sets_now;
     if (own) {
       RJ_HIP(h, hipEventRecord(h->ev_walk_done, st));
       RJ_HIP(h, hipStreamWaitEvent(h->exact_stream, h->ev_walk_done, 0));
@@ -1984,9 +2009,10 @@
   {
     rj_handle_s::PlanRec::Pip& pp = h->plan.pip;
     pp.ran = n > 0; pp.epoch = h->plan.epoch; pp.n = n; pp.aux = aux; pp.caller = pts_dev != nullptr;
-    pp.shared = aux && h->lsi_shared; pp.passes = h->last_passes; pp.rest_hint = seen; pp.why = why;
+    pp.shared = aux && h->lsi_shared; pp.passes = h->last_passes; pp.rest_hint = walk_sets_now == 3 && seen3 != ~0ull ? seen3 : seen; pp.why = why;
     pp.order = order ? (h->order_fresh ? 2 : 1) : 0;
     pp.prepared = h->last_prepared;
+    pp.sets = walk && h->last_walk_points == 2 ? h->last_walk_sets : 0;
   }
   toc(h, RJ_T_PIP_KERNEL, own ? h->exact_stream : st);
   if (h->cur_caller >= 0 && n) {
diff --git a/rayjoin_amd/csrc/rj_kernels.h b/rayjoin_amd/csrc/rj_kernels.h
--- a/rayjoin_amd/csrc/rj_kernels.h
+++ b/rayjoin_amd/csrc/rj_kernels.h
@@ -161,9 +161,9 @@
                              unsigned long long* count_hint);
 hipError_t launch_pip(hipStream_t st, const PipArgs& a, bool stats, int max_blocks);
 hipError_t launch_pip_walk(hipStream_t st, const PipArgs& a, bool stats, int max_blocks);
-hipError_t launch_pip_walk2(hipStream_t st, const PipArgs& a, int max_blocks, int cus, bool stats = false);
-int pip_walk2_blocks_per_cu(int top);
-int pip_walk2_blocks_beside(int top, int lsi_blocks_per_cu);
+hipError_t launch_pip_walk2(hipStream_t st, const PipArgs& a, int max_blocks, int cus, bool stats = false, int sets = 2);
+int pip_walk2_blocks_per_cu(int top, int sets = 2);
+int pip_walk2_blocks_beside(int top, int lsi_blocks_per_cu, int sets = 2);
 hipError_t launch_pip_exact(hipStream_t st, const PipArgs& a, int blocks, const PipRestArgs& r);
 int pip_walk_list_slots();
 uint32_t pip_walk_group_lanes(uint64_t n, int top, int cus);
diff --git a/rayjoin_amd/csrc/rj_kernels.hip b/rayjoin_amd/csrc/rj_kernels.hip
--- a/rayjoin_amd/csrc/rj_kernels.hip
+++ b/rayjoin_amd/csrc/rj_kernels.hip
@@ -1716,19 +1716,35 @@
 }
 
 
-__host__ __device__ __forceinline__ size_t walk2_wave_lds(int top, int P = 2) { return (size_t) 16 * walk_stack_entries(top) + (size_t) kWalkList * 256 * P; }
+constexpr int kWalk3List = 5;
+constexpr int kWalk3Stack = 76;
+static_assert(3 * kWalk3List * 256 + 16 * kWalk3Stack == 2 * kWalkList * 256 + 16 * kWalkStack, "k_pip_walk3_prepared: the LDS of k_pip_walk2, to the byte");
+static_assert(kWalk3List <= kWalkList, "a todo record has kWalkList slots");
+__host__ __device__ __forceinline__ int walk2_stack_entries(int top, int stack_max = kWalkStack) {
+  const int e = walk_stack_entries(top);
+  return e < stack_max ? e : stack_max;
+}
+__host__ __device__ __forceinline__ size_t walk2_wave_lds(int top, int P = 2, int list = kWalkList, int stack_max = kWalkStack) {
+  return (size_t) 16 * walk2_stack_entries(top, stack_max) + (size_t) list * 256 * P;
+}
 
 constexpr int kWalkCycleStamps = 7777;
-template <bool STATS, int P, bool PREP = false>
+template <bool STATS, int P, bool PREP = false, int LIST = kWalkList, int STACKMAX = kWalkStack>
 __device__ __forceinline__ void pip_walk_many(const PipArgs& A) {
   extern __shared__ uint4 walk_smem[];
   const int lane = lane_id();
-  const int wib = threadIdx.x >> 6;
+  constexpr bool LEAN = P >= 3;
+  const int wib = LEAN ? (int) __builtin_amdgcn_readfirstlane(threadIdx.x >> 6) : (int) (threadIdx.x >> 6);
+  auto here = [&]() -> uint32_t {
+    uint32_t l = (uint32_t) lane;
+    if (LEAN) asm volatile("" : "+v"(l));
+    return l;
+  };
   const DeviceBvh& T = A.bvh;
   const uint32_t* const sky = (T.sky && T.sky[kSkyBuckets] == 0u) ? T.sky : nullptr;
-  const int stack_entries = walk_stack_entries(T.top);
+  const int stack_entries = walk2_stack_entries(T.top, STACKMAX);
   const int stack_cap = A.walk_stack > 0 && A.walk_stack < stack_entries ? A.walk_stack : stack_entries;
-  uint4* const stack = walk_smem + (size_t) wib * (walk2_wave_lds(T.top, P) / 16);
+  uint4* const stack = walk_smem + (size_t) wib * (walk2_wave_lds(T.top, P, LIST, STACKMAX) / 16);
   uint32_t* const cand = reinterpret_cast<uint32_t*>(stack + stack_entries);
   const uint32_t stack_lds = (uint32_t) (uintptr_t) stack;
   constexpr uint32_t GP = 64u * P;
@@ -1755,6 +1771,8 @@
     int32_t qx[P], qy[P], qbest[P], sure_y0[P];
     uint32_t cand_base[P], cand_at[P];
     bool valid[P];
+    auto base_of = [&](int p) -> uint32_t { return LEAN ? (uint32_t) p * (LIST * 64) : cand_base[p]; };
+    auto slot_of = [&](uint32_t at) -> uint32_t { return LEAN ? at + here() : at; };
     typedef int i2_t __attribute__((ext_vector_type(2)));
     typedef int i4_t __attribute__((ext_vector_type(4)));
     typedef const __attribute__((address_space(4))) i4_t* ext_ptr_t;
@@ -1775,15 +1793,22 @@
         ipl[p] = !prep && A.order ? A.order[ipc] : (uint32_t) ipc;
       }
     }
-    i4_t ext0 = {0, 0, 0, 0}, ext1 = {0, 0, 0, 0};
+    i4_t extp[P];
+#pragma unroll
+    for (int p = 0; p < P; p++) extp[p] = i4_t{0, 0, 0, 0};
     if (ext) {
       const ext_ptr_t E = (ext_ptr_t) (uintptr_t) A.qext + (uint64_t) gu * P;
-      ext0 = E[0];
-      ext1 = E[1];
+#pragma unroll
+      for (int p = 0; p < P; p++) extp[p] = E[p];
     }
     ll2_t ptl[P];
     i2_t qpl[P];
-    if (full) {
+    if (full && LEAN) {
+      const i2_t* const q = reinterpret_cast<const i2_t*>(A.qpts) + (uint64_t) gu * GP;
+      const uint32_t l = here();
+#pragma unroll
+      for (int p = 0; p < P; p++) qpl[p] = __builtin_nontemporal_load(q + (l + 64u * p));
+    } else if (full) {
       const i2_t* const q = reinterpret_cast<const i2_t*>(A.qpts) + (uint64_t) gu * GP + lane;
 #pragma unroll
       for (int p = 0; p < P; p++) qpl[p] = __builtin_nontemporal_load(q + 64 * p);
@@ -1812,8 +1837,8 @@
         qy[p] = valid[p] ? quant(ptl[p].y) : 0;
         qbest[p] = valid[p] ? 0x7FFFFFFF : -1;
       }
-      cand_base[p] = (uint32_t) lane + (uint32_t) p * (kWalkList * 64);
-      cand_at[p] = cand_base[p];
+      cand_base[p] = (uint32_t) lane + (uint32_t) p * (LIST * 64);
+      cand_at[p] = base_of(p);
       sure_y0[p] = INT32_MIN;
     }
     if (sky) {
@@ -1830,9 +1855,13 @@
       ext_ok = !__ballot(gone);
     }
     if (ext_ok) {
-      gx0 = ext0.x < ext1.x ? ext0.x : ext1.x;
-      gx1 = ext0.y > ext1.y ? ext0.y : ext1.y;
-      gy0 = ext0.z < ext1.z ? ext0.z : ext1.z;
+      gx0 = extp[0].x; gx1 = extp[0].y; gy0 = extp[0].z;
+#pragma unroll
+      for (int p = 1; p < P; p++) {
+        gx0 = gx0 < extp[p].x ? gx0 : extp[p].x;
+        gx1 = gx1 > extp[p].y ? gx1 : extp[p].y;
+        gy0 = gy0 < extp[p].z ? gy0 : extp[p].z;
+      }
     } else {
       const bool l0 = qbest[0] >= 0, l1 = qbest[1] >= 0;
       const int32_t a0 = l0 ? qx[0] : kEmptyMin, a1 = l1 ? qx[1] : kEmptyMin;
@@ -1872,8 +1901,8 @@
       const uint64_t higher = root_higher;
       uint64_t m = refine_if_many(b, __ballot(b.x0 <= gx1 && gx0 <= b.x1 && b.y1 >= gy0 - 1));
       if (__popcll(m) > stack_cap) { m = 0; ovf = true; }
-      if ((m >> lane) & 1)
-        stack[__popcll(m & higher)] = make_uint4(((uint32_t) T.top << 28) | (uint32_t) lane, (uint32_t) b.y0, (uint32_t) b.x0, (uint32_t) b.x1);
+      if ((m >> here()) & 1)
+        stack[__popcll(m & higher)] = make_uint4(((uint32_t) T.top << 28) | here(), (uint32_t) b.y0, (uint32_t) b.x0, (uint32_t) b.x1);
       sp = __popcll(m);
       wave_lds_fence();
       if (STATS) { st_groups++; st_pushed += (unsigned long long) sp; }
@@ -1917,9 +1946,9 @@
         }
         uint64_t m = refine_if_many(b, __ballot(b.x0 <= gx1 && gx0 <= b.x1 && b.y1 >= gy0 - 1 && b.y0 <= gbest));
         if (sp + __popcll(m) > stack_cap) { ovf = true; break; }
-        if ((m >> lane) & 1)
+        if ((m >> here()) & 1)
           stack[sp + __popcll(m & higher)] =
-              make_uint4(((uint32_t) (lvl - 1) << 28) | (idx * 64 + lane), (uint32_t) b.y0, (uint32_t) b.x0, (uint32_t) b.x1);
+              make_uint4(((uint32_t) (lvl - 1) << 28) | (idx * 64 + here()), (uint32_t) b.y0, (uint32_t) b.x0, (uint32_t) b.x1);
         sp += __popcll(m);
         wave_lds_fence();
         if (STATS) { st_nodes++; st_pushed += (unsigned long long) __popcll(m); }
@@ -1961,10 +1990,10 @@
             if ((sx0 <= qx[p]) & (qx[p] <= sx1) & (sy1 >= qy[p] - 1) & (qbest[p] >= sy0) & (j >= jlo)) {
               const bool certain = sx0 < qx[p] && qx[p] < sx1 && sy0 > qy[p];
               const bool replace = certain && sy1 < sure_y0[p];
-              const bool first = cand_at[p] == cand_base[p];
-              const bool over = !replace && cand_at[p] == cand_base[p] + kWalkList * 64;
+              const bool first = cand_at[p] == base_of(p);
+              const bool over = !replace && cand_at[p] == base_of(p) + LIST * 64;
               if (STATS && lane == __builtin_ctzll(__ballot(true))) st_hits++;
-              cand[(replace || over) ? cand_base[p] : cand_at[p]] = slot0 + (uint32_t) jj;
+              cand[slot_of((replace || over) ? base_of(p) : cand_at[p])] = slot0 + (uint32_t) jj;
               sure_y0[p] = (replace || (first && certain)) ? sy0 : INT32_MIN;
               cand_at[p] += replace ? 0u : 64u;
               const int32_t top = certain ? sy1 + 1 : 0x7FFFFFFF;
@@ -1991,7 +2020,7 @@
             int kept = 0;
             if (STATS) st_sweeps++;
             for (int base = 0; base < sp; base += 64) {
-              const int i = base + lane;
+              const int i = base + (int) here();
               const bool have = i < sp;
               uint4 en = make_uint4(0, 0, 0, 0);
               if (have) en = stack[i];
@@ -2017,9 +2046,9 @@
     for (int p = 0; p < P; p++) {
       const uint64_t ipos = (uint64_t) g32 * GP + (uint64_t) p * 64 + lane;
       ipv[p] = !PREP && A.order ? A.order[valid[p] ? ipos : A.n - 1] : (uint32_t) ipos;
-      donev[p] = valid[p] && !ovf && (cand_at[p] == cand_base[p] || sure_y0[p] != INT32_MIN);
-      const bool hit = donev[p] && cand_at[p] != cand_base[p];
-      const uint32_t slot = hit ? cand[cand_base[p]] : 0u;
+      donev[p] = valid[p] && !ovf && (cand_at[p] == base_of(p) || sure_y0[p] != INT32_MIN);
+      const bool hit = donev[p] && cand_at[p] != base_of(p);
+      const uint32_t slot = hit ? cand[slot_of(base_of(p))] : 0u;
       const uint32_t e = T.seid[slot];
       const int32_t f = A.face ? T.sface[slot] : 0;
       out_e[p] = hit ? e : 0xFFFFFFFFu;
@@ -2027,15 +2056,15 @@
     }
 #pragma unroll
     for (int p = 0; p < P; p++) {
-      const uint32_t fill = (cand_at[p] - cand_base[p]) >> 6;
-      const bool listed = valid[p] && !donev[p] && !ovf && fill <= (uint32_t) kWalkList;
+      const uint32_t fill = (cand_at[p] - base_of(p)) >> 6;
+      const bool listed = valid[p] && !donev[p] && !ovf && fill <= (uint32_t) LIST;
       const bool rest = valid[p] && !donev[p] && !listed;
       const uint64_t lm = __ballot(listed);
       const uint64_t g64 = (uint64_t) g32 * P + p;
       if (listed) {
         const uint64_t rec = g64 * 64 + rank_below(lm);
 #pragma unroll
-        for (int k = 0; k < kWalkList; k++) A.todo[rec * kWalkList + k] = (uint32_t) k < fill ? cand[cand_base[p] + 64 * k] : 0xFFFFFFFFu;
+        for (int k = 0; k < kWalkList; k++) A.todo[rec * kWalkList + k] = k < LIST && (uint32_t) k < fill ? cand[slot_of(base_of(p)) + 64 * k] : 0xFFFFFFFFu;
       }
       if (lane == 0 && g64 * 64 < A.n) A.todo_mask[g64] = lm;
       const uint64_t rm = __ballot(rest);
@@ -2101,6 +2130,7 @@
 __global__ __launch_bounds__(256, 8) __attribute__((amdgpu_num_sgpr(96))) __attribute__((amdgpu_num_vgpr(28))) void k_pip_walk2(PipArgs A) { pip_walk_many<false, 2>(A); }
 __global__ __launch_bounds__(256, 4) __attribute__((amdgpu_num_sgpr(96))) void k_pip_walk2_stats(PipArgs A) { pip_walk_many<true, 2>(A); }
 __global__ __launch_bounds__(256, 8) __attribute__((amdgpu_num_sgpr(96))) __attribute__((amdgpu_num_vgpr(28))) void k_pip_walk2_prepared(PipArgs A) { pip_walk_many<false, 2, true>(A); }
+__global__ __launch_bounds__(256, 8) __attribute__((amdgpu_num_sgpr(96))) __attribute__((amdgpu_num_vgpr(28))) void k_pip_walk3_prepared(PipArgs A) { pip_walk_many<false, 3, true, kWalk3List, kWalk3Stack>(A); }
 
 
 #ifndef RJ_EXACT_WAVES
@@ -2468,14 +2498,18 @@
   return hipGetLastError();
 }
 
-int pip_walk2_blocks_per_cu(int top) {
-  const size_t block = 4 * walk2_wave_lds(top) + 64;
+static size_t walk2_block_lds(int top, int sets) {
+  return 4 * (sets == 3 ? walk2_wave_lds(top, 3, kWalk3List, kWalk3Stack) : walk2_wave_lds(top));
+}
+
+int pip_walk2_blocks_per_cu(int top, int sets) {
+  const size_t block = walk2_block_lds(top, sets) + 64;
   const size_t by_lds = (size_t) 160 * 1024 / block;
   return (int) (by_lds < 8 ? by_lds : 8);
 }
 
-int pip_walk2_blocks_beside(int top, int lsi_blocks_per_cu) {
-  const size_t block = 4 * walk2_wave_lds(top) + 64;
+int pip_walk2_blocks_beside(int top, int lsi_blocks_per_cu, int sets) {
+  const size_t block = walk2_block_lds(top, sets) + 64;
   const size_t left = (size_t) 160 * 1024 > (size_t) lsi_blocks_per_cu * 17920 ? (size_t) 160 * 1024 - (size_t) lsi_blocks_per_cu * 17920 : 0;
   int n = (int) (left / block);
   if (n > 8 - lsi_blocks_per_cu) n = 8 - lsi_blocks_per_cu;
@@ -2487,22 +2521,26 @@
   }
   const int by_vgpr = (512 - lsi_blocks_per_cu * lsi_regs) / walk_regs;
   if (n > by_vgpr) n = by_vgpr;
-  if (n > pip_walk2_blocks_per_cu(top)) n = pip_walk2_blocks_per_cu(top);
+  if (n > pip_walk2_blocks_per_cu(top, sets)) n = pip_walk2_blocks_per_cu(top, sets);
   return n < 1 ? 1 : n;
 }
 
-hipError_t launch_pip_walk2(hipStream_t st, const PipArgs& a_in, int max_blocks, int cus, bool stats) {
+hipError_t launch_pip_walk2(hipStream_t st, const PipArgs& a_in, int max_blocks, int cus, bool stats, int sets) {
   PipArgs a = a_in;
-  const size_t lds = 4 * walk2_wave_lds(a.bvh.top);
-  const int res = cus * pip_walk2_blocks_per_cu(a.bvh.top);
+  if (sets != 3 || stats || !a.qpts) sets = 2;
+  const size_t lds = walk2_block_lds(a.bvh.top, sets);
+  const int res = cus * pip_walk2_blocks_per_cu(a.bvh.top, sets);
   a.group_lanes = 64;
-  const uint64_t ngroups = (a.n + 127) / 128;
-  a.chunk_groups = a.chunk_groups ? a.chunk_groups : 3;
+  const uint64_t gp = 64u * (uint64_t) sets;
+  const uint64_t ngroups = (a.n + gp - 1) / gp;
+  a.chunk_groups = a.chunk_groups ? a.chunk_groups : (sets == 3 ? 2 : 3);
   const uint64_t nchunks = (ngroups + a.chunk_groups - 1) / a.chunk_groups;
   const int grid = grid_for(nchunks, 4, res < max_blocks ? res : max_blocks);
   note("k_pip_walk2", grid, 2);
   if (stats)
     hipLaunchKernelGGL(k_pip_walk2_stats, dim3(grid), dim3(256), lds, st, a);
+  else if (sets == 3)
+    hipLaunchKernelGGL(k_pip_walk3_prepared, dim3(grid), dim3(256), lds, st, a);
   else if (a.qpts)
     hipLaunchKernelGGL(k_pip_walk2_prepared, dim3(grid), dim3(256), lds, st, a);
   else
```

Result: faster. 41000 M query segments/s, median of 6 (+2.8%).
